# Algolzw/image-restoration-sde

Measured on AMD Instinct MI355X. Metric: restored images/sec at 256x256, 100-step IR-SDE reverse sampler, higher is better.
Workload: dtype f32; 1 GPU; IR-SDE deraining ConditionalUNet nf=64 depth=4, reverse_sde, batch=16/GPU 256x256, T=100 (BASELINE.json configs[1]); compute_dtype=fp32, global_batch=16

## Files before the change

### image_restoration_sde_amd/_lib.py

```python
import ctypes
import os
import subprocess
import threading

_HERE = os.path.dirname(os.path.abspath(__file__))
LIB_PATH = os.environ.get("IRSDE_LIB_PATH") or os.path.join(_HERE, "libirsde_hip.so")
CSRC = os.path.join(_HERE, "csrc")

MODE = {"sde": 0, "ode": 1, "posterior": 2, "dsde_sde": 3, "dsde_ode": 4}
COEF_STRIDE = 12
FLAG_KEEP_ACTIVATIONS = 1
FLAG_NAIVE_CONV = 2
FLAG_NO_WINOGRAD = 4
FLAG_NO_WINOGRAD_F43 = 8
FLAG_UNCOND_FULLATTN = 16
FLAG_BF16 = 32
FLAG_NAF_INTRO_SKIP = 64
FLAG_BF16_ACT = 128
FLAG_NO_FUSED_LN = 256
FLAG_NAF_LENS = 512
FLAG_FP16 = 1024
FLAG_NO_WINOGRAD_FUSED = 2048
FLAG_NO_FUSED_ATTN = 4096
FLAG_NO_NAF_CHAIN = 8192
FLAG_SPLIT_BF16X2 = 16384
FLAG_SPLIT_F16X2 = 32768
FLAG_NAF_STEREO = 65536
FLAG_NAF_UNCOND = 131072
FLAG_UNET_STEREO = 262144
FLAG_F16_ACT = 524288
FLAG_NO_WINO_POLY = 1048576
FLAG_SCAM_STREAM = 2097152
FLAG_NO_SPLIT3 = 4194304
SAMPLE_GRAPH = 1
SAMPLE_PROFILE = 2

SYMBOLS = [
    "irsde_last_error", "irsde_version", "irsde_create", "irsde_create_nafnet", "irsde_destroy", "irsde_num_weights",
    "irsde_weight_name", "irsde_weight_shape", "irsde_load_weight", "irsde_finalize_weights",
    "irsde_set_schedule", "irsde_unet_forward", "irsde_sample", "irsde_sde_step", "irsde_philox_normal",
    "irsde_get_profile", "irsde_debug_tap", "irsde_work_model", "irsde_debug_conv", "irsde_debug_conv_choice", "irsde_debug_conv_halo_choice", "irsde_debug_conv_features", "irsde_plan_describe", "irsde_bench_conv", "irsde_op_profile", "irsde_debug_split_gemm", "irsde_bench_naf_chain", "irsde_debug_force_subbatches", "irsde_debug_force_chain_groups", "irsde_debug_force_wino_poly", "irsde_debug_force_split3", "irsde_debug_force_split3_blocks", "irsde_debug_scam", "irsde_debug_scam_full",
    "irsde_debug_scam_stream", "irsde_debug_scam_full_stream", "irsde_debug_force_scam_stream",
    "irsde_debug_naf_gate_sca", "irsde_debug_tlsc", "irsde_debug_ln_film", "irsde_debug_naf_lnconv", "irsde_debug_naf_chain", "irsde_debug_naf_chain_split_order",
    "irsde_debug_full_attention16",
    "irsde_eval_metrics", "irsde_tensor2img", "irsde_upscale_bicubic", "irsde_mask_to", "irsde_imresize",
    "irsde_set_lens_info", "irsde_nafnet_set_local_pool", "irsde_create_latent_unet", "irsde_latent_shapes", "irsde_latent_encode", "irsde_latent_decode", "irsde_latent_hidden",
]


class IrsdeLibraryError(RuntimeError):
    pass


class IrsdeError(RuntimeError):
    pass


class Config(ctypes.Structure):
    _fields_ = [("in_nc", ctypes.c_int32), ("out_nc", ctypes.c_int32), ("nf", ctypes.c_int32),
                ("depth", ctypes.c_int32), ("device", ctypes.c_int32), ("flags", ctypes.c_int32)]


class NafConfig(ctypes.Structure):
    _fields_ = [("img_channel", ctypes.c_int32), ("width", ctypes.c_int32), ("middle_blk_num", ctypes.c_int32),
                ("n_enc", ctypes.c_int32), ("enc_blk_nums", ctypes.c_int32 * 8), ("n_dec", ctypes.c_int32),
                ("dec_blk_nums", ctypes.c_int32 * 8), ("device", ctypes.c_int32), ("flags", ctypes.c_int32)]


class LatentConfig(ctypes.Structure):
    _fields_ = [("in_ch", ctypes.c_int32), ("out_ch", ctypes.c_int32), ("ch", ctypes.c_int32), ("n_mult", ctypes.c_int32),
                ("ch_mult", ctypes.c_int32 * 8), ("embed_dim", ctypes.c_int32), ("device", ctypes.c_int32),
                ("flags", ctypes.c_int32)]


_lib = None
_lock = threading.Lock()


PROBES_LIB_PATH = os.path.join(_HERE, "libirsde_hip_probes.so")


def build_library(force=False, verbose=False, probes=True):
    if force:
        subprocess.run(["make", "-C", CSRC, "clean"], check=True, capture_output=not verbose)
    for extra in ([], ["PROBES=1"]) if probes else ([],):
        r = subprocess.run(["make", "-j8", "-C", CSRC] + extra, capture_output=True, text=True)
        if r.returncode != 0:
            raise IrsdeLibraryError("building libirsde_hip%s.so failed:\n" % ("_probes" if extra else "") + r.stdout + r.stderr)
        if verbose:
            print(r.stdout)
    return LIB_PATH


def _declare(lib):
    c = ctypes
    P = c.c_void_p
    lib.irsde_last_error.restype = c.c_char_p
    lib.irsde_last_error.argtypes = []
    lib.irsde_version.restype = c.c_int
    lib.irsde_create.argtypes = [c.POINTER(Config), c.POINTER(P)]
    lib.irsde_create_nafnet.argtypes = [c.POINTER(NafConfig), c.POINTER(P)]
    lib.irsde_destroy.argtypes = [P]
    lib.irsde_destroy.restype = None
    lib.irsde_num_weights.argtypes = [P]
    lib.irsde_weight_name.argtypes = [P, c.c_int]
    lib.irsde_weight_name.restype = c.c_char_p
    lib.irsde_weight_shape.argtypes = [P, c.c_int, c.POINTER(c.c_int64), c.POINTER(c.c_int)]
    lib.irsde_load_weight.argtypes = [P, c.c_char_p, P, c.POINTER(c.c_int64), c.c_int]
    lib.irsde_finalize_weights.argtypes = [P]
    lib.irsde_set_schedule.argtypes = [P, c.c_int, P]
    lib.irsde_unet_forward.argtypes = [P, P, P, c.POINTER(c.c_int64), c.c_int, c.c_int, c.c_int, c.c_int, P, P]
    lib.irsde_sample.argtypes = [P, c.c_int, P, P, P, c.c_uint64, c.c_uint64, c.c_int, c.c_int, c.c_int,
                                 c.c_int, c.c_int, P, P, c.c_int]
    lib.irsde_sde_step.argtypes = [c.c_int, c.c_int, P, P, P, P, P, c.c_uint64, c.c_uint64, c.c_int, c.c_int,
                                   c.c_int, c.c_int, P]
    lib.irsde_philox_normal.argtypes = [P, c.c_int, c.c_int, c.c_int, c.c_uint64, c.c_uint64, P]
    lib.irsde_get_profile.argtypes = [P, c.POINTER(c.c_double)]
    lib.irsde_debug_tap.argtypes = [P, c.c_char_p, P, c.POINTER(c.c_int64)]
    lib.irsde_work_model.argtypes = [P, c.c_int, c.c_int, c.c_int, c.POINTER(c.c_double)]
    lib.irsde_debug_conv.argtypes = [P, c.c_int, P, c.c_int, c.c_int, c.c_int, c.c_int, c.c_int, P, c.c_int, c.c_int,
                                     c.c_int, c.c_int, c.c_int, P, P, c.c_int, c.c_int, P, P, c.c_int, c.c_int, P]
    lib.irsde_debug_conv_choice.argtypes = [c.c_int] * 13 + [c.c_uint] + [c.c_int] * 4 + [c.POINTER(c.c_int), c.c_char_p, c.c_int]
    lib.irsde_debug_conv_halo_choice.argtypes = [c.c_int] * 13 + [c.c_uint] + [c.c_int] * 5 + [c.c_char_p, c.c_int]
    lib.irsde_debug_conv_features.argtypes = ([P, c.c_int, P, c.c_int] + [c.c_int] * 4 + [P] + [c.c_int] * 7 + [P] * 3 + [P, c.c_int, P, P, P, c.c_int] + [c.c_int] * 6 +
                                              [c.POINTER(c.c_int), P, c.c_char_p, c.c_int, P])
    lib.irsde_plan_describe.argtypes = [P, c.c_int, c.c_int, c.c_int, c.c_char_p, c.c_int]
    lib.irsde_op_profile.argtypes = [P, c.c_char_p, c.c_int]
    lib.irsde_bench_conv.argtypes = [c.c_int] * 11 + [c.POINTER(c.c_double)]
    lib.irsde_bench_naf_chain.argtypes = [c.c_int] * 4 + [c.POINTER(c.c_double)]
    lib.irsde_debug_force_subbatches.argtypes = [c.c_int]
    lib.irsde_debug_force_chain_groups.argtypes = [c.c_int]
    lib.irsde_debug_force_wino_poly.argtypes = [c.c_int]
    lib.irsde_debug_force_split3.argtypes = [c.c_int]
    lib.irsde_debug_force_split3_blocks.argtypes = [c.c_int]
    lib.irsde_debug_scam.argtypes = [P, c.c_int, c.c_int, c.c_int, c.c_int] + [P] * 12 + [P, P]
    lib.irsde_debug_scam_full.argtypes = [P, c.c_int, c.c_int, c.c_int, c.c_int] + [P] * 12 + [P, P]
    lib.irsde_debug_scam_stream.argtypes = [P, c.c_int, c.c_int, c.c_int, c.c_int] + [P] * 12 + [c.c_int, P, P]
    lib.irsde_debug_scam_full_stream.argtypes = [P, c.c_int, c.c_int, c.c_int, c.c_int] + [P] * 12 + [c.c_int, P, P]
    lib.irsde_debug_force_scam_stream.argtypes = [c.c_int]
    lib.irsde_debug_naf_gate_sca.argtypes = [P, c.c_int, c.c_int, c.c_int, c.c_int] + [P] * 8
    lib.irsde_debug_tlsc.argtypes = [P] + [c.c_int] * 6 + [P] * 4
    lib.irsde_debug_ln_film.argtypes = [P, c.c_int64, c.c_int, c.c_int64, P, P, P, c.c_int, P, P]
    lib.irsde_debug_naf_lnconv.argtypes = [c.c_int, P, c.c_int64, c.c_int, c.c_int, c.c_int64, P, P, P, c.c_int, P, P, P, c.c_int, P, P, P, P, P]
    lib.irsde_debug_naf_chain.argtypes = [P, P, c.c_int, c.c_int] + [P] * 16 + [P, c.c_int, c.c_int, P, c.c_int, c.c_int, c.c_int, P]
    lib.irsde_debug_naf_chain_split_order.argtypes = [c.c_int, c.c_int, c.POINTER(c.c_int), c.c_int64]
    lib.irsde_debug_full_attention16.argtypes = [P, c.c_int, c.c_int, P, P]
    lib.irsde_debug_split_gemm.argtypes = [P, P, P, c.c_int, c.c_int, c.c_int, c.c_int, c.c_int, P]
    lib.irsde_eval_metrics.argtypes = [P, P, c.c_int, c.c_int, c.c_int, c.c_int, c.c_int, c.POINTER(c.c_double), P]
    lib.irsde_tensor2img.argtypes = [P, P, c.c_int, c.c_int, c.c_int, c.c_int, P]
    lib.irsde_upscale_bicubic.argtypes = [P, P, c.c_int, c.c_int, c.c_int, c.c_int, c.c_int, P]
    lib.irsde_mask_to.argtypes = [P, P, c.c_int, c.c_int, c.c_int, c.c_int, P, c.c_int, c.c_int, c.c_int, c.c_int, P]
    lib.irsde_imresize.argtypes = [P, P] + [c.c_int] * 6 + [P, P, c.c_int, P, P, c.c_int, P]
    lib.irsde_set_lens_info.argtypes =[P, c.POINTER(c.c_float), c.c_int]
    lib.irsde_nafnet_set_local_pool.argtypes = [P, c.c_int, c.c_int, c.c_int, c.c_int]
    lib.irsde_create_latent_unet.argtypes = [c.POINTER(LatentConfig), c.POINTER(P)]
    lib.irsde_latent_shapes.argtypes = [P, c.c_int, c.c_int, c.POINTER(c.c_int64), c.POINTER(c.c_int64), c.POINTER(c.c_int)]
    lib.irsde_latent_encode.argtypes = [P, P, c.c_int, c.c_int, c.c_int, P, c.POINTER(P), P]
    lib.irsde_latent_decode.argtypes = [P, P, c.POINTER(P), c.c_int, c.c_int, c.c_int, P, P]
    lib.irsde_latent_hidden.argtypes = [P, c.c_int, c.c_int, c.c_int, c.c_int, P, P]
    for name in SYMBOLS:
        getattr(lib, name)
    return lib


def lib():
    global _lib
    with _lock:
        if _lib is None:
            if not os.path.exists(LIB_PATH):
                raise IrsdeLibraryError(
                    "libirsde_hip.so not found at %s — build it with `python -c 'import __graft_entry__ as g; "
                    "g.build()'` or `make -C %s`. There is no CPU/PyTorch fallback for this path." % (LIB_PATH, CSRC))
            try:
                _lib = _declare(ctypes.CDLL(LIB_PATH))
            except OSError as ex:
                raise IrsdeLibraryError("failed to load %s: %s" % (LIB_PATH, ex)) from ex
        return _lib


_probes = None


def probes_lib():
    global _probes
    with _lock:
        if _probes is None:
            if not os.path.exists(PROBES_LIB_PATH):
                raise IrsdeLibraryError("libirsde_hip_probes.so not found at %s — build it with `make -C %s PROBES=1`" % (PROBES_LIB_PATH, CSRC))
            try:
                _probes = _declare(ctypes.CDLL(PROBES_LIB_PATH))
            except OSError as ex:
                raise IrsdeLibraryError("failed to load %s: %s" % (PROBES_LIB_PATH, ex)) from ex
        return _probes


def check(rc, L=None):
    if rc != 0:
        msg = (L or lib()).irsde_last_error()
        raise IrsdeError("libirsde_hip error %d: %s" % (rc, msg.decode() if msg else "?"))


def stream_ptr(torch_stream=None):
    import torch
    s = torch_stream if torch_stream is not None else torch.cuda.current_stream()
    return ctypes.c_void_p(s.cuda_stream)
```

### image_restoration_sde_amd/csrc/common.h

```cpp
#pragma once
#include <hip/hip_runtime.h>
#include <cstdint>
#include <cstdio>
#include <cstdlib>
#include <stdexcept>
#include <string>
#include <vector>
#include "split3_layout.h"

namespace irsde {

struct HipError : std::runtime_error {
    using std::runtime_error::runtime_error;
};
struct HipOutOfMemory : HipError {
    using HipError::HipError;
};

inline int tuning_env_int(const char* name, int dflt) {
    static const bool on = [] { const char* t = getenv("IRSDE_TUNING"); return t && atoi(t) == 1; }();
    if (!on) return dflt;
    const char* v = getenv(name);
    return v ? atoi(v) : dflt;
}
// ... 185 lines not shown
    int tiles_x = 0, tiles_y = 0, nblk_n = 0;
    int n_slow = 0;
    unsigned grid = 0;
    int lds = 0;
    int instance = -1;
};
constexpr int kHaloInstances = 9;
struct ConvChoice {
    enum Family { PAIR, NARROW3, ZLOOP_BATCH, ZLOOP_1X1, HALO, IGEMM };
    enum Operand { OP_F32, OP_F32_BUF, OP_BF16, OP_F16 };
    enum Storage { ACT_F32, ACT_BF16, ACT_F16 };
    Family family = IGEMM;
    int BM = 0, BN = 0;
    Operand op = OP_F32;
    Storage act = ACT_F32;
    bool inscale = false;
    int zbatch = 0, zrows = 0;
    unsigned gx = 0, gy = 1, gz = 1;
    HaloChoice halo;
    int threads = 0, lds = 0;
    int row = -1;
    std::string name() const;
    long long blocks() const { return (long long)gx * gy * gz; }
};
int conv_base_bn(int Cout);
void conv_validate(const ConvParams& p);
ConvChoice conv_choose(const ConvParams& p, const ConvTune& t, const ConvKnobs& k, int cu_count);
int conv_instance_count();
void launch_conv(const ConvParams& p, hipStream_t s, const ConvTune& t = {}, const ConvKnobs* knobs = nullptr, ConvChoice* chosen = nullptr);
void conv_global_init();
void conv_halo_global_init();
bool conv_halo_eligible(const ConvParams& p);
HaloChoice conv_halo_choose(const ConvParams& p, const ConvTune& t, int halo2, int nslow);
bool conv_halo2_wanted(const ConvParams& p);
HaloChoice launch_conv_halo(const ConvParams& p, hipStream_t s, const ConvTune& t = {});
void launch_fill_random(float* p, size_t n, unsigned seed, float scale, hipStream_t s);
__device__ __forceinline__ float silu_hw(const float v) {
    return v * __builtin_amdgcn_rcpf(1.0f + __builtin_amdgcn_exp2f(v * -1.44269504088896341f));
}

void launch_f32_to_bf16(const float* in, unsigned short* out, size_t n, hipStream_t s);
void launch_f32_to_f16(const float* in, unsigned short* out, size_t n, hipStream_t s);
void launch_bf16_to_f32(const unsigned short* in, float* out, size_t n, hipStream_t s);
void launch_f16_to_f32(const unsigned short* in, float* out, size_t n, hipStream_t s);
void launch_conv_naive(const ConvParams& p, hipStream_t s);

void launch_layernorm(const float* x, const float* g, const float* res, float* out, int64_t M, int C,
                      float eps, hipStream_t s, bool bf16 = false);
void launch_layernorm_film(const float* x, const float* g, const float* scale, const float* shift, int film_bstride,
                           int64_t pixels_per_image, float* out, int64_t M, int C, float eps, hipStream_t s,
                           bool f16 = false);
int dwgate_tiles(int H, int W, int c);
bool naf_lnconv_ok(int c, int Cout, long long M);
void launch_naf_pwconv(const float* x, const float* in_scale, int64_t pixels_per_image, const unsigned short* w16, const float* bias, const float* ch_scale,
                       const float* res, float* out, int64_t M, int c, int Cout, hipStream_t s, bool f16 = false);
void naf_lnconv_global_init();
void launch_naf_lnconv(const float* x, const float* g, const float* fscale, const float* fshift, int film_bstride, int64_t pixels_per_image,
                       const unsigned short* w16, const float* bias, float* out, int64_t M, int c, int Cout, int gate, const float* gate_film,
                       int gate_film_bstride, hipStream_t s, bool f16 = false);
void launch_dwconv_gate(const float* u, const float* w, const float* bias, float* out, float* partial, int B, int H, int W,
                        int c, hipStream_t s, bool f16 = false);
void launch_sca(const float* partial, int ntiles, const float* W, const float* bias, float* mean, float* s_out, int B,
                int c, int HW, hipStream_t s);
void launch_sca_mean(const float* partial, int ntiles, float* mean, int B, int c, int HW, hipStream_t s);
void tlsc_check_shape(int B, int h, int w, int c, int k1, int k2);
void launch_tlsc_pool(const float* gated, float* rowsum, float* pooled, int B, int h, int w, int c, int k1, int k2, hipStream_t s);
void launch_tlsc_scale(float* gated, const float* scale, int B, int h, int w, int c, int k1, int k2, hipStream_t s);
void launch_row_gate(const float* in, float* out, int rows, int h, hipStream_t s);

struct AttnWorkspace {
    float* pmax = nullptr;
    float* pctx = nullptr;
    float* psum = nullptr;
    float* ctx = nullptr;
    int nch = 0;
};
int attn_num_chunks(int N, int B);
void launch_linear_attention(const float* qkv, float* out, int B, int N, const AttnWorkspace& ws, hipStream_t s,
                             bool bf16 = false);

void launch_attention_kv_context(const float* xn, const float* wkv, int B, int N, int C, const AttnWorkspace& ws, hipStream_t s,
                                 const float* ln_g = nullptr, float ln_eps = 1e-5f, const unsigned short* wkv_pair = nullptr,
                                 float w_inv_scale = 1.f, int op16 = 0, bool act_bf16 = false);
void launch_attention_q_out(const float* q, float* out, int B, int N, const AttnWorkspace& ws, hipStream_t s);
void launch_attention_q_out_fused(const float* xn, const float* x, const float* wq, const float* wout, const float* bias,
                                  const float* g2, float* y, int B, int N, int C, float eps, const AttnWorkspace& ws, hipStream_t s,
                                  const float* ln_g = nullptr, const unsigned short* wq_pair = nullptr, const unsigned short* wout_pair = nullptr,
                                  float wq_inv = 1.f, float wout_inv = 1.f, int op16 = 0, bool act_bf16 = false);

void scam_check_shape(int H, int W, int c, bool any_width = false);
void launch_scam_prologue(const float* x, const float* g_l, const float* g_r, float* xs2, int B, int H, int W, int c, hipStream_t s);
void launch_scam_core(const float* qv, float* F, int B, int H, int W, int c, hipStream_t s);
void launch_scam_epilogue(const float* x, const float* F, const float* beta, const float* gamma, float* out, int B, int H, int W, int c, hipStream_t s);
void scam_pack_proj(const float* w1, const float* b1, const float* w2, const float* b2, int c, std::vector<float>& w, std::vector<float>& bias);
constexpr int kScamFullMaxW = 1024;
constexpr int kScamFullMaxC = 2048;
void scam_full_check_shape(int H, int W, int c, bool any_width = false);
void launch_scam_full_prologue(const float* x, const float* g_l, const float* g_r, float* x2, int B, int H, int W, int c, hipStream_t s);
void launch_scam_full_core(const float* qv, float* F, int B, int H, int W, int c, hipStream_t s);
void launch_scam_full_epilogue(float* x, const float* F, const float* beta, const float* gamma, int B, int H, int W, int c, hipStream_t s);
constexpr int kScamMaxWs = 512;
constexpr int kScamStreamMaxBlockW = 512;
bool scam_stream_block_ok(int block_w);
void launch_scam_stream_core(const float* qv, float* F, int B, int Hs, int Ws, int c, int block_w, hipStream_t s);
void launch_stereo_prep(const float* xt, const float* cond, float* x0, int B, int ic, int P, int H, int W, int Hp, int Wp, hipStream_t s);
void launch_stereo_pack_pred(const float* in, float* out, int B, int ic, int Hp, int Wp, int in_stride, int out_stride, hipStream_t s);
void launch_stereo_unet_prep(const float* xt, const float* cond, float* x0, int B, int ic, int P, int H, int W, int Hp, int Wp, hipStream_t s);
void launch_stereo_unet_pack_pred(const float* in, const float* xt, float* out, int B, int ic, int H, int W, int Hp, int Wp, int in_stride, int out_stride,
                                  hipStream_t s);

void launch_full_attention(const float* qkv, float* out, int B, int N, hipStream_t s);
void launch_full_attention16(const unsigned short* qkv, unsigned short* out, int B, int N, hipStream_t s);

void launch_prep_input(const float* xt, const float* cond, float* x0, int B, int in_nc, int H, int W, int Hp, int Wp,
                       hipStream_t s, int reflect = 1);

enum Act { ACT_NONE = 0, ACT_SILU = 1, ACT_GELU = 2 };
void launch_sinusoid(const float* tvals, const float* freqs, float* out, int rows, int half, hipStream_t s);
void launch_row_linear(const float* in, int in_stride, const float* W, const float* b, float* out, int out_stride,
                       int rows, int in_dim, int out_dim, int act_in, int act_out, hipStream_t s);

struct StepState {
    int t;
    int t_next;
    int pad0, pad1;
    float coef[12];
};
void launch_step_begin(StepState* st, const float* film_table, int film_row, float* film_cur,
                       const float* coef_table, hipStream_t s);
void launch_set_step(StepState* st, int t_next, hipStream_t s);

struct SampleCtl {
    int mode;
    int pad;
    const float* noise;
    long long noise_tstride;
    unsigned long long seed;
    unsigned long long image_offset;
};
void launch_set_ctl(SampleCtl* ctl, int mode, const float* noise, long long noise_tstride, unsigned long long seed,
                    unsigned long long image_offset, hipStream_t s);

void launch_unpack_pred(const float* pred, float* out, int B, int C, int H, int W, int Hp, int Wp, int stride, hipStream_t s);
void launch_add(const float* a, const float* b, float* out, size_t n, hipStream_t s);
void launch_nchw_to_nhwc_pad(const float* in, float* out, int B, int C, int H, int W, int Hp, int Wp, int Cp, int reflect,
                             hipStream_t s);
void launch_nhwc_to_nchw(const float* in, float* out, int B, int C, int H, int W, hipStream_t s, bool bf16 = false, bool f16 = false);

struct UpdateParams {
    float* x;
    const float* mu;
    const float* pred;
    int64_t sb, sc, sy, sx;
    const float* noise;
    int64_t noise_tstride;
    const StepState* st;
    const SampleCtl* ctl;
    int t_imm;
    float coef_imm[12];
    int mode;
    int B, C, H, W;
    uint64_t seed;
    uint64_t image_offset;
    int batch0;
};
void launch_sde_update(const UpdateParams& p, hipStream_t s);
// ... 12 lines not shown
```

### image_restoration_sde_amd/csrc/engine.h

```cpp
#pragma once
#include <algorithm>
#include <cmath>
#include <cstring>
#include <functional>
#include <map>
#include <memory>
#include <mutex>
#include <string>
#include <vector>

#include "../../include/irsde_hip.h"
#include "common.h"

namespace irsde {

constexpr int kWinoFusedMaxCin = 256, kWinoFusedMaxCout = 256;
inline long long wino_fused_min_tiles() { return tuning_env_int("IRSDE_WINO_FUSED_MINT", 4096); }
inline bool wino_fused64_enabled() { return tuning_env_int("IRSDE_WINO_FUSED64", 1) != 0; }
inline bool wino_fused64_pair_enabled() { return tuning_env_int("IRSDE_WINO_FUSED64_PAIR", 1) != 0; }
inline int wino_fused64_max_cin() { return tuning_env_int("IRSDE_WINO_FUSED64_MAXCIN", 512); }
inline int wino_fused64_max_cout() { return tuning_env_int("IRSDE_WINO_FUSED64_MAXCOUT", 512); }
inline long long wino_fused64_min_tiles() { return tuning_env_int("IRSDE_WINO_FUSED64_MINT", 1024); }
inline int wino_fused64t_mode() { return tuning_env_int("IRSDE_WINO_FUSED64T", 1); }
inline bool naf_lnconv_enabled() { return tuning_env_int("IRSDE_NAF_LNCONV", 1) != 0; }
inline int naf_chain_split_mode() { return tuning_env_int("IRSDE_NAF_CHAIN_SPLIT", 0); }

int wino_poly_mode();
void set_force_wino_poly(int mode);
constexpr int kWinoPolyUpMinCin = 512;
inline bool wino_poly_wants_weights(int mode, bool up, int Cin) { return mode >= 2 || (mode == 1 && (!up || Cin >= kWinoPolyUpMinCin)); }

int split3_mode();
void set_force_split3(int mode);
constexpr int kSplit3WinoMinCin = 512;
inline int split3_wino_min_cin() { return tuning_env_int("IRSDE_SPLIT3_MINCIN", kSplit3WinoMinCin); }
inline bool split3_wino_wants_weights(int mode, int Cin, int Cout) { return mode >= 2 || Cin > 512 || (Cin >= split3_wino_min_cin() && Cout >= 512); }
inline long long split3_fused_min_tiles() { return tuning_env_int("IRSDE_SPLIT3_FUSED_MINT", 4096); }
constexpr int kSplit3NotExactF32 = IRSDE_FLAG_NO_WINOGRAD | IRSDE_FLAG_NAIVE_CONV | IRSDE_FLAG_BF16 | IRSDE_FLAG_BF16_ACT | IRSDE_FLAG_FP16 | IRSDE_FLAG_F16_ACT |
                                   IRSDE_FLAG_SPLIT_BF16X2 | IRSDE_FLAG_SPLIT_F16X2 | IRSDE_FLAG_NO_SPLIT3;
inline bool split3_wants_weights(int flags) { return !(flags & kSplit3NotExactF32) && split3_mode() > 0; }

inline int wino_min_c(int tile) {
    return tuning_env_int(tile == 4 ? "IRSDE_WINO4_MINC" : "IRSDE_WINO2_MINC", tile == 4 ? 64 : 256);
}

struct DeviceScope {
    int prev = -1;
    explicit DeviceScope(int dev) {
        if (hipGetDevice(&prev) != hipSuccess) prev = -1;
        if (prev != dev) IRSDE_HIP_CHECK(hipSetDevice(dev));
        else prev = -1;
    }
    ~DeviceScope() {
        if (prev >= 0) (void)hipSetDevice(prev);
    }
    DeviceScope(const DeviceScope&) = delete;
    DeviceScope& operator=(const DeviceScope&) = delete;
};

struct HostTensor {
    std::vector<int64_t> shape;
    std::vector<float> data;
    bool loaded = false;
};

struct ConvW {
    float* w = nullptr;
    float* bias = nullptr;
    int Cout = 0, Cin = 0, KH = 1, KW = 1;
    float* wino_u2 = nullptr;
    float* wino_u4 = nullptr;
    float* wino_uf = nullptr;
    float* wino_uf64 = nullptr;
    unsigned short* wino_uf64p = nullptr;
    float wino_uf64p_scale = 1.f;
    unsigned short* wino_up = nullptr;
    float wino_up_scale = 1.f;
    unsigned short* wino_u4t = nullptr;
    unsigned short* wino_polyt = nullptr;
    float* wino_poly = nullptr;
};
struct ResW {
    ConvW b1, b2, res;
    bool has_res = false;
    float* mlp_w = nullptr;
    float* mlp_b = nullptr;
    int film_off = 0;
    int Cout = 0;
};
struct ScamW {
    int c = 0;
    float *gl = nullptr, *gr = nullptr;
    ConvW l, r;
    float *beta = nullptr, *gamma = nullptr;
};
struct AttnW {
    float* g1 = nullptr;
    ConvW qkv, out;
    float* g2 = nullptr;
    int C = 0;
};

struct NafBlockW {
    int c = 0;
    float *g1 = nullptr, *g2 = nullptr;
    ConvW conv1, conv3, conv4, conv5;
    float *dw_w = nullptr, *dw_b = nullptr;
    float *sca_w = nullptr, *sca_b = nullptr;
    float *beta = nullptr, *gamma = nullptr;
    float *mlp_w = nullptr, *mlp_b = nullptr;
    int film_off = 0;
    float *cam_w = nullptr, *cam_b = nullptr;
    int cam_off = 0;
    ScamW fusion;
};

struct NafChainW {
    unsigned short* w = nullptr;
    float* vecs = nullptr;
    int nblocks = 0, film_off = 0, cam_off = 0;
    unsigned short* wsplit[5] = {nullptr, nullptr, nullptr, nullptr, nullptr};
};

// ... 226 lines not shown
    ScamW mid_scam;
    std::vector<ResW> up_res;
    std::vector<AttnW> up_attn;
    std::vector<ConvW> up_conv;
    ResW final_res;
    std::vector<ResW*> all_res;
    int film_row = 0;

    int arch = 0;
    int naf_ic = 0;
    std::vector<int> naf_enc_nums, naf_dec_nums;
    int naf_mid_num = 0;
    std::vector<std::vector<NafBlockW>> naf_enc, naf_dec;
    std::vector<NafBlockW> naf_mid;
    std::vector<ConvW> naf_downs, naf_ups;
    ConvW naf_intro, naf_ending;
    std::vector<NafBlockW*> naf_all;
    std::vector<NafChainW> naf_chain_enc, naf_chain_dec;
    NafChainW naf_chain_mid;
    float *cm_w1 = nullptr, *cm_b1 = nullptr, *cm_w3 = nullptr, *cm_b3 = nullptr;
    int cam_row = 0;
    float* cam_cur = nullptr;
    int cam_rows = 0;
    int cam_set = 0;

    int tlsc_base_h = 0, tlsc_base_w = 0, tlsc_train_h = 0, tlsc_train_w = 0;

    int lat_in = 0, lat_out = 0, lat_ch = 0, lat_embed = 0;
    std::vector<int> lat_mult;
    ConvW lat_init, lat_latent, lat_post, lat_final;
    std::vector<ResW> lat_enc_res, lat_dec_res;
    AttnW lat_enc_attn, lat_dec_attn;
    std::vector<ConvW> lat_down, lat_up;
    std::vector<std::unique_ptr<LatentPlan>> lat_plans;

    int T = 0;
    float* coef_table = nullptr;
    float* film_table = nullptr;
    float* film_cur = nullptr;
    int film_cur_rows = 0;
    StepState* step = nullptr;
    SampleCtl* ctl = nullptr;

    float* zeros = nullptr;
    hipStream_t stream = nullptr;
    hipEvent_t ev_in = nullptr, ev_out = nullptr;
    static constexpr int kMaxSub = 4;
    hipStream_t sub_stream[kMaxSub - 1] = {nullptr, nullptr, nullptr};
    hipEvent_t ev_fork = nullptr, ev_join[kMaxSub - 1] = {nullptr, nullptr, nullptr};
    std::vector<std::unique_ptr<Plan>> plans;
    uint64_t use_counter = 0;
    double profile[12] = {0};
    std::vector<double> op_ms;
    std::vector<std::string> op_desc;
    int op_steps = 0;
    int plan_parts = 1;
    int op_split = 1;
    std::vector<hipEvent_t> ev_pool;
    std::mutex mu;

    float* dmalloc(size_t n) {
        float* p = nullptr;
        IRSDE_HIP_CHECK(hipMalloc(&p, std::max<size_t>(n, 16) * sizeof(float)));
        dev_allocs.push_back(p);
        return p;
    }
    std::map<const float*, unsigned short*> bf16_copies;
    const unsigned short* bf16_copy(const float* w, size_t n) {
        auto it = bf16_copies.find(w);
        if (it != bf16_copies.end()) return it->second;
        unsigned short* d = nullptr;
        IRSDE_HIP_CHECK(hipMalloc(&d, n * sizeof(unsigned short)));
        if (cfg.flags & IRSDE_FLAG_FP16) launch_f32_to_f16(w, d, n, stream);
        else launch_f32_to_bf16(w, d, n, stream);
        IRSDE_HIP_CHECK(hipStreamSynchronize(stream));
        bf16_copies[w] = d;
        return d;
    }
    struct PairCopy { unsigned short* p; float inv_scale; };
    std::map<const float*, PairCopy> pair_copies;
    PairCopy pair_copy(const float* w, size_t n) {
        return make_pair_copy(pair_copies, w, n, [&](unsigned short* d, bool f16, float sc) { launch_split_planes(w, d, n, n, 2, stream, f16, sc); });
    }
    std::map<const float*, PairCopy> pair_copies_il;
    PairCopy pair_copy_il(const float* w, size_t rows, int K) {
        return make_pair_copy(pair_copies_il, w, rows * (size_t)K, [&](unsigned short* d, bool f16, float sc) { launch_split_pairs(w, d, rows, K, stream, f16, sc); });
    }
    template <class Split>
    PairCopy make_pair_copy(std::map<const float*, PairCopy>& cache, const float* w, size_t n, Split split) {
        auto it = cache.find(w);
        if (it != cache.end()) return it->second;
        const bool f16 = (cfg.flags & IRSDE_FLAG_SPLIT_F16X2) != 0;
        float sc = 1.f;
        if (f16) {
            std::vector<float> h(n);
            IRSDE_HIP_CHECK(hipMemcpy(h.data(), w, n * sizeof(float), hipMemcpyDeviceToHost));
            sc = pow2_scale_into_512(h.data(), n);
        }
        unsigned short* d = nullptr;
        IRSDE_HIP_CHECK(hipMalloc(&d, 2 * n * sizeof(unsigned short)));
        dev_allocs.push_back(reinterpret_cast<float*>(d));
        split(d, f16, sc);
        IRSDE_HIP_CHECK(hipStreamSynchronize(stream));
        const PairCopy pc{d, 1.0f / sc};
        cache[w] = pc;
        return pc;
    }
    float* upload(const std::vector<float>& v) {
        float* p = dmalloc(v.size());
        IRSDE_HIP_CHECK(hipMemcpy(p, v.data(), v.size() * sizeof(float), hipMemcpyHostToDevice));
        return p;
    }
};

namespace irsde {

inline bool naf_lens(const irsde_engine* e) { return (e->cfg.flags & IRSDE_FLAG_NAF_LENS) != 0; }
inline bool naf_stereo(const irsde_engine* e) { return e->arch == 1 && (e->cfg.flags & IRSDE_FLAG_NAF_STEREO) != 0; }
inline bool unet_stereo(const irsde_engine* e) { return e->arch == 0 && (e->cfg.flags & IRSDE_FLAG_UNET_STEREO) != 0; }
inline bool stereo_engine(const irsde_engine* e) { return naf_stereo(e) || unet_stereo(e); }
inline bool uncond_engine(const irsde_engine* e) {
    return (e->arch == 0 && (e->cfg.flags & IRSDE_FLAG_UNCOND_FULLATTN) != 0) || (e->arch == 1 && (e->cfg.flags & IRSDE_FLAG_NAF_UNCOND) != 0);
}
inline int rup32(int c) { return (c + 31) & ~31; }
inline bool tlsc_window(const irsde_engine* e, int level, int* K0, int* K1) {
    if (e->tlsc_train_h <= 0) return false;
    const int P = 1 << e->cfg.depth;
    const int Hp = (e->tlsc_train_h + P - 1) / P * P, Wp = (e->tlsc_train_w + P - 1) / P * P;
    *K0 = (int)((long long)(Hp >> level) * e->tlsc_base_h / e->tlsc_train_h);
    *K1 = (int)((long long)(Wp >> level) * e->tlsc_base_w / e->tlsc_train_w);
    return true;
}
inline StepState* step_of(const irsde_engine* e, const Plan* pl) { return pl->own_step ? pl->own_step : e->step; }
inline float* film_of(const irsde_engine* e, const Plan* pl) { return pl->own_film ? pl->own_film : e->film_cur; }

void build_inventory(irsde_engine* e);
void build_inventory_naf(irsde_engine* e);
void build_inventory_latent(irsde_engine* e);
void finalize(irsde_engine* e);
void compute_film_rows(irsde_engine* e, const float* tvals, int rows, float* dst, hipStream_t s);
void ensure_film_cur(irsde_engine* e, int rows);
void pack_conv_rows(const float* w_oihw, const float* bias, int O, int I, int KH, int KW, const std::vector<int>& perm, std::vector<float>& pw,
                    std::vector<float>& pb);
std::vector<int> naf_gate_perm(int c);
std::vector<int> naf_shuffle_perm(int Cout);
std::vector<float> pack_dwconv_taps(const float* w, int c2);
void pack_naf_chain_host(const std::vector<NafChainHostW>& blocks, std::vector<unsigned short>& w, std::vector<float>& vecs);

Plan* get_plan(irsde_engine* e, int B, int H, int W, bool per_sample_film, int slot = 0, int b0 = 0);
int naf_subbatches(const irsde_engine* e, int B, int H, int W);
void set_force_chain_groups(int g);
void set_force_scam_stream(int block_w);
int forced_chain_groups();
int forced_scam_stream();
void set_force_subbatches(int n);
LatentPlan* get_latent_plan(irsde_engine* e, int B, int H, int W, bool decode);

int guard(const std::function<void()>& f);

}
```

### image_restoration_sde_amd/csrc/engine_debug.hip

```cpp
#include "engine.h"
#include "../../include/irsde_hip_debug.h"

using namespace irsde;

namespace irsde {
namespace {

struct Scratch {
    hipStream_t s;
    std::vector<void*> bufs;
    explicit Scratch(hipStream_t s_) : s(s_) {}
    ~Scratch() {
        (void)hipStreamSynchronize(s);
        for (void* p : bufs) (void)hipFree(p);
    }
    Scratch(const Scratch&) = delete;
    Scratch& operator=(const Scratch&) = delete;
    template <class T> T* alloc(size_t n) {
        void* p = nullptr;
        IRSDE_HIP_CHECK(hipMalloc(&p, n * sizeof(T)));
        bufs.push_back(p);
        return static_cast<T*>(p);
    }
    float* upload(const float* host, size_t n) {
// ... 838 lines not shown
        const bool f16 = operand == 2;
        unsigned short *w16 = nullptr, *a0 = nullptr, *a1 = nullptr, *ar = nullptr, *ao = nullptr;
        float wsc = 1.f;
        if (pair) {
            wsc = f16 ? pow2_scale_into_512(pk.data(), pk.size()) : 1.f;
            w16 = mem.alloc<unsigned short>(2 * pk.size());
            p.w_pair = w16; p.pair_scale = 1.0f / wsc;
        } else if (operand) {
            w16 = mem.alloc<unsigned short>(pk.size());
            p.w_bf = w16;
        }
        p.f16 = f16 ? 1 : 0;
        if (storage) {
            a0 = mem.alloc<unsigned short>(npix_in * C0);
            p.in0 = reinterpret_cast<const float*>(a0);
            if (in1) { a1 = mem.alloc<unsigned short>(npix_in * C1); p.in1 = reinterpret_cast<const float*>(a1); }
            if (res) { ar = mem.alloc<unsigned short>(nout); p.res = reinterpret_cast<const float*>(ar); }
            ao = mem.alloc<unsigned short>(nout);
            p.out = reinterpret_cast<float*>(ao);
            p.in_bf16 = p.out_bf16 = storage == 1;
            p.in_f16 = p.out_f16 = storage == 2;
        }
        ConvKnobs k;
        static_assert(sizeof(ConvKnobs) == 11 * sizeof(int), "the hook's knob array is ConvKnobs, field by field");
        if (knobs) memcpy(&k, knobs, sizeof k);
        conv_validate(p);
        auto narrow = [&](const float* src, unsigned short* dst, size_t n) {
            if (storage == 2) launch_f32_to_f16(src, dst, n, s);
            else launch_f32_to_bf16(src, dst, n, s);
        };
        if (pair) launch_split_pairs(dw, w16, (size_t)Cout * nz, K * K * Cin, s, f16, wsc);
        else if (operand == 2) launch_f32_to_f16(dw, w16, pk.size(), s);
        else if (operand == 1) launch_f32_to_bf16(dw, w16, pk.size(), s);
        if (storage) {
            narrow(in0, a0, npix_in * C0);
            if (in1) narrow(in1, a1, npix_in * C1);
            if (res) narrow(res, ar, nout);
            IRSDE_HIP_CHECK(hipMemsetAsync(ao, 0xFF, nout * 2, s));
        }
        ConvChoice c;
        launch_conv(p, s, conv_tune_from_code(tune), knobs ? &k : nullptr, &c);
        if (storage == 2) launch_f16_to_f32(ao, out, nout, s);
        else if (storage == 1) launch_bf16_to_f32(ao, out, nout, s);
        IRSDE_HIP_CHECK(hipStreamSynchronize(s));
        write_choice_line(c, choice, choice_len);
        if (c.family == ConvChoice::HALO) {
            const size_t n = strlen(choice);
            if (n + 2 < (size_t)choice_len) {
                choice[n] = ' ';
                write_halo_line(c.halo, choice + n + 1, choice_len - (int)n - 1);
            }
        }
    });
}

int irsde_debug_split_gemm(const float* A, const float* Bm, float* C, int M, int N, int K, int ncomp, int nplanes, void* stream) {
    return guard([&] {
        const int twin3 = nplanes == 43 ? 0 : nplanes == 45 ? 1 : nplanes == 47 ? 2 : -1;
        if (twin3 < 0 && nplanes != 42 && nplanes != 44) throw HipError("debug_split_gemm: nplanes must be 42, 43, 44, 45 or 47");
        hipStream_t s = reinterpret_cast<hipStream_t>(stream);
        conv_global_init();
        Scratch mem(s);
        if (twin3 >= 0) {
            if (!gemm_split_triples_fits(M, N, K, N)) throw HipError("debug_split_gemm: shape not eligible for the three-piece GEMM");
            launch_gemm_split_triples(split_triples(mem, A, Bm, C, M, N, K, ncomp, s), ncomp, s, split3_launch_twin(twin3));
        } else {
            const bool f16 = nplanes == 44;
            launch_gemm_split_pairs(split_pairs(mem, A, Bm, C, M, N, K, ncomp, s, f16, f16 ? 1.0f / 16.0f : 1.f, f16 ? 64.0f : 1.f), ncomp, s, 0, f16);
        }
        IRSDE_HIP_CHECK(hipStreamSynchronize(s));
    });
}

int irsde_debug_force_chain_groups(int g) {
    set_force_chain_groups(g == 1 || g == 2 || g == 4 ? g : 0);
    return IRSDE_OK;
}

int irsde_debug_force_split3(int mode) {
    set_force_split3(mode >= 0 && mode <= 2 ? mode : -1);
    return IRSDE_OK;
}

int irsde_debug_force_split3_blocks(int n) {
    if (n >= 0 && n < 8) return guard([&] { throw HipError("debug_force_split3_blocks: n must be at least 8 (one block per XCD), or negative for the default"); });
    set_force_split3_blocks(n);
    return IRSDE_OK;
}

int irsde_debug_force_wino_poly(int mode) {
    set_force_wino_poly(mode >= 0 && mode <= 2 ? mode : -1);
    return IRSDE_OK;
}

int irsde_debug_force_subbatches(int n) {
    set_force_subbatches(n < 0 ? 0 : n);
    return IRSDE_OK;
}

int irsde_bench_naf_chain(int variant, int nblocks, int B, int iters, double* ms_out) {
    return guard([&] {
        if (!ms_out || nblocks < 1 || nblocks > 64 || B < 1 || iters < 1) throw HipError("bench_naf_chain: bad argument");
        const int G = variant == 22 ? 2 : (variant == 24 || variant == 25 || variant == 26) ? 4 : 1;
#ifdef IRSDE_PROBES
        if (variant != 0 && variant != 1 && variant != 11 && G == 1) throw HipError("bench_naf_chain: bad variant");
#else
        if (variant != 0 && variant != 1 && G == 1) throw HipError("bench_naf_chain: variant 11 is a measurement twin (make PROBES=1)");
#endif
        conv_global_init();
        OwnedStream stream(hipStreamDefault);
        hipStream_t s = stream.s;
        Scratch mem(s);
        const size_t nx = (size_t)B * 64 * 512, nw = naf_chain_weight_halves(nblocks), nv = naf_chain_vec_floats(nblocks);
        float *dx = mem.alloc<float>(nx), *dout = mem.alloc<float>(nx), *dvec = mem.alloc<float>(nv), *dfilm = mem.alloc<float>((size_t)nblocks * 2048);
        unsigned short* dw = mem.alloc<unsigned short>(nw);
        const size_t chunk = (size_t)64 << 20;
        float* dwf = mem.alloc<float>(chunk);
        launch_fill_random(dx, nx, 1, 1.0f, s);
        launch_fill_random(dvec, nv, 2, 0.1f, s);
        launch_fill_random(dfilm, (size_t)nblocks * 2048, 3, 0.1f, s);
        for (size_t o = 0; o < nw; o += chunk) {
            const size_t n = std::min(chunk, nw - o);
            launch_fill_random(dwf, n, 4 + (unsigned)(o / chunk), 0.04f, s);
            launch_f32_to_f16(dwf, dw + o, n, s);
        }
        unsigned short* dwg = nullptr;
        void* dscratch = nullptr;
        if (G > 1) {
            IRSDE_HIP_CHECK(hipStreamSynchronize(s));
            dwg = mem.alloc<unsigned short>(nw);
            naf_chain_build_split_weights(dw, dwg, nblocks, G, s);
            dscratch = mem.alloc<char>(naf_chain_split_scratch_bytes(B));
            IRSDE_HIP_CHECK(hipMemset(dscratch, 0, naf_chain_split_scratch_bytes(B)));
        }
        auto run = [&]() {
            if (G > 1) launch_naf_chain_split(dx, dout, dwg, dvec, nblocks, B, dfilm, 0, 0, nullptr, 0, 0, G, dscratch, s);
            else launch_naf_chain(dx, dout, dw, dvec, nblocks, B, dfilm, 0, 0, nullptr, 0, 0, s, variant == 11 ? 1 : variant);
        };
        if (variant == 26) {
#ifdef IRSDE_PROBES
            naf_chain_set_sabotage(1);
#else
            throw HipError("bench_naf_chain: variant 26 is a PROBES-build test");
#endif
        }
        struct SabotageOff { ~SabotageOff() { naf_chain_set_sabotage(0); } } sabotage_off;
        run();
        if (variant == 25) {
#ifdef IRSDE_PROBES
            const int ng = naf_chain_split_groups(B, 4);
            unsigned long long* dd = mem.alloc<unsigned long long>((size_t)ng * 8 * 16);
            IRSDE_HIP_CHECK(hipMemsetAsync(dd, 0, (size_t)ng * 8 * 16 * 8, s));
            naf_chain_set_debug(dd);
            run();
            IRSDE_HIP_CHECK(hipStreamSynchronize(s));
            naf_chain_set_debug(nullptr);
            std::vector<unsigned long long> hd((size_t)ng * 8 * 16);
            IRSDE_HIP_CHECK(hipMemcpy(hd.data(), dd, hd.size() * 8, hipMemcpyDeviceToHost));
            double acc[16] = {0};
            double nwv = 0;
            for (size_t w = 0; w < (size_t)ng * 8; ++w) {
                if (!hd[w * 16 + 15]) continue;
                for (int k = 0; k < 16; ++k) acc[k] += (double)hd[w * 16 + k];
                nwv += 1;
            }
            static const char* names[12] = {"norm1 (incl. residual-stream fetch)", "conv1 GEMM passes", "depthwise 3x3 + gate + pool", "gated fetch behind barrier (pool)", "sca.1 GEMM", "conv3 GEMM + residual", "norm2 (incl. residual-stream fetch)", "conv4 GEMM + gate", "conv5 GEMM + residual", "scale-vector / gated fetch (sca, conv4)", "group barriers (6 per block)", "publishing (gated slice, residual slice)"};
// ... 244 lines not shown
```

### image_restoration_sde_amd/csrc/engine_plan.hip

```cpp
#include "engine.h"
#include <atomic>

using namespace irsde;

namespace irsde {

struct Builder {
    irsde_engine* e;
    Plan* pl;
    bool reuse;
    bool naive;
    int film_bstride;
    int b0 = 0;
    const float* film_base() const { return film_of(e, pl) + (size_t)b0 * film_bstride; }
    const float* cam_base() const { return e->cam_cur + (size_t)b0 * e->cam_row; }
    const float* fused_ln_g = nullptr;

    bool act_bf16() const { return (e->cfg.flags & IRSDE_FLAG_BF16_ACT) != 0; }
    bool act_f16() const { return (e->cfg.flags & IRSDE_FLAG_F16_ACT) != 0; }
    Tensor talloc(int B, int H, int W, int C, int force_f32 = 0) {
        Tensor t;
        t.B = B; t.H = H; t.W = W; t.C = C;
        t.bf16 = act_bf16() && !force_f32;
        t.f16 = act_f16() && !force_f32;
// ... 96 lines not shown
            if (w.wino_uf64p && push_wino_fused(p, reinterpret_cast<const float*>(w.wino_uf64p), true, w.wino_uf64p_scale)) return out;
            if (w.wino_uf64 && push_wino_fused(p, w.wino_uf64, true)) return out;
            if (w.wino_uf && push_wino_fused(p, w.wino_uf, false)) return out;
            if (w.wino_u4 && wino_shape_ok(p, 4) && push_wino(p, w.wino_u4, 4, nullptr, 1.f, w.wino_u4t)) return out;
            if (w.wino_u2 && wino_shape_ok(p, 2) && push_wino(p, w.wino_u2, 2)) return out;
        }
        push_conv(p);
        return out;
    }

    bool push_wino_fused(const ConvParams& d, const float* Uf, bool k64, float pair_uscale = 0.f) {
        ConvParams dd = d;
        dd.zeros = e->zeros;
        if (pair_uscale != 0.f) dd.pair_scale = 1.0f / (kWinoFused64PairVScale * pair_uscale);
        auto eligible = [&](const ConvParams& q) { return k64 ? wino_fused64_eligible(q) : wino_fused_eligible(q); };
        int parts = 1;
        if (!eligible(dd)) {
            for (parts = 2; parts <= 4; parts *= 2) {
                if (d.B % parts) continue;
                ConvParams q = dd;
                q.B = d.B / parts;
                if (eligible(q)) break;
            }
            if (parts > 4) return false;
            dd.B = d.B / parts;
        }
        const int Ctot = d.C0 + d.C1;
        const long long T = (long long)dd.B * (d.Ho / 4) * (d.Wo / 4);
        const long long blocks = k64 ? wino_fused64_num_blocks(dd) : (long long)dd.B * ((d.Ho / 4 + 3) / 4) * ((d.Wo / 4 + 7) / 8) * (d.Cout / 32);
        if (T < (k64 ? wino_fused64_min_tiles() : wino_fused_min_tiles()) || blocks < 256) return false;
        bool use_t = false;
        if (k64 && pair_uscale == 0.f && wino_fused64t_mode() && wino_fused64t_eligible(dd)) {
            const double per_block = (double)wino_fused64t_num_items(dd) / std::max(1, device_cu_count());
            const double work = per_block * (Ctot / 16);
            use_t = wino_fused64t_mode() >= 2 || (!d.in_shift && (work >= 64.0 || (work >= 32.0 && per_block >= 8.0 && !d.res)));
        }
        Op op;
        op.kind = OP_CONV;
        op.flops = conv_flops(d);
        op.exec_flops = 36 * 2.0 * (double)T * parts * Ctot * d.Cout;
        op.bytes = 4.0 * (double)d.B * d.Hin * d.Win * Ctot + 4.0 * (double)d.B * d.Ho * d.Wo * d.Cout + 4.0 * 9.0 * (double)d.Cout * Ctot;
        char buf[256];
        const bool pair = pair_uscale != 0.f;
        snprintf(buf, sizeof buf, "conv(%swinograd F4 fused) %s T=%lld Cout=%d Cin=%d up=%d blocks=%lld flops=%.4g exec=%.4g%s", pair ? "split f16x2 " : "",
                 use_t ? "32x64" : k64 ? "16x64" : "32x32", T * parts, d.Cout, Ctot, d.in_shift, blocks * parts, op.flops, op.exec_flops,
                 parts > 1 ? (parts == 2 ? " (2 batch slices)" : " (4 batch slices)") : "");
        op.desc = buf;
        std::vector<ConvParams> slices;
        for (int i = 0; i < parts; ++i) {
            ConvParams q = dd;
            const size_t b0 = (size_t)i * dd.B;
            q.in0 = dd.in0 + b0 * dd.Hin * dd.Win * dd.pix0;
            if (dd.in1) q.in1 = dd.in1 + b0 * dd.Hin * dd.Win * dd.pix1;
            q.out = dd.out + b0 * dd.Ho * dd.Wo * dd.out_stride;
            if (dd.res) q.res = dd.res + b0 * dd.Ho * dd.Wo * dd.res_stride;
            if (dd.film && dd.film_bstride) q.film = dd.film + b0 * dd.film_bstride;
            slices.push_back(q);
        }
        if (use_t)
            op.fn = [slices, Uf](hipStream_t s) { for (const auto& q : slices) launch_wino_fused64t(q, Uf, s, 0); };
        else if (k64)
            op.fn = [slices, Uf, pair](hipStream_t s) { for (const auto& q : slices) launch_wino_fused64(q, Uf, s, pair ? 4 : 0); };
        else
            op.fn = [slices, Uf](hipStream_t s) { for (const auto& q : slices) launch_wino_fused(q, Uf, s); };
        push_op(std::move(op));
        return true;
    }

    static constexpr long long kSplit3MinRows = 256;
    static constexpr int kSplit3MinCout = 512, kSplit3MinCoutPoly = 256;
    static constexpr double kSplit3MinFlop = 9e9;
    bool split3_rule(long long T, int K, int Cout, int ncomp, int min_cout = kSplit3MinCout) const {
        return T >= kSplit3MinRows && Cout >= min_cout && ncomp * 2.0 * (double)T * K * Cout >= kSplit3MinFlop;
    }
    bool split3_adopts(const unsigned short* Ut, long long T, int K, int Cout, int ncomp, int min_cout = kSplit3MinCout) const {
        const int mode = split3_mode();
        if (!Ut || mode <= 0 || naive || (e->cfg.flags & kSplit3NotExactF32) || !gemm_split_triples_fits(T, Cout, K, Cout)) return false;
        return mode >= 2 || split3_rule(T, K, Cout, ncomp, min_cout);
    }
    bool split3_over_fused(const ConvW& w, const ConvParams& p) const {
        if (!w.wino_u4t || p.C0 + p.C1 > 512 || !wino_shape_ok(p, 4)) return false;
        const long long T = (long long)p.B * (p.Ho / 4) * (p.Wo / 4);
        return T >= split3_fused_min_tiles() && split3_rule(T, p.C0 + p.C1, p.Cout, 36) && split3_adopts(w.wino_u4t, T, p.C0 + p.C1, p.Cout, 36);
    }
    float* alloc_triples(int ncomp, long long rows, int K) { return pl->alloc(((size_t)ncomp * split3_comp_elems((size_t)rows, (size_t)K) + 1) / 2, true); }

    bool push_wino_poly(const ConvParams& d, const float* U, const unsigned short* Ut = nullptr) {
        const int mode = wino_poly_mode();
        if (mode <= 0 || !wino_poly_eligible(d)) return false;
        ConvParams dd = d;
        dd.zeros = e->zeros;
        WinoPolyPlan wp = make_wino_poly(dd, U, nullptr, nullptr);
        const long long T = wp.T;
        const long long gemm_blocks = wp.ncomp * ((T + 127) / 128) * ((d.Cout + 127) / 128);
        const double exec_flops = wp.ncomp * 2.0 * (double)T * wp.K * d.Cout;
        if (mode == 1 && (gemm_blocks < 2ll * device_cu_count() || exec_flops < 2e10)) return false;
        if ((unsigned long long)T * std::max(wp.K, d.Cout) * 4ull >= 0x7fffffffull) return false;
        static const int poly_min_cout = tuning_env_int("IRSDE_SPLIT3_POLY_MINCOUT", kSplit3MinCoutPoly);
        const bool tri = split3_adopts(Ut, T, wp.K, d.Cout, wp.ncomp, poly_min_cout);
        float* V = tri ? alloc_triples(wp.ncomp, T, wp.K) : pl->alloc((size_t)wp.ncomp * T * wp.K, true);
        float* Mb = pl->alloc((size_t)wp.ncomp * T * d.Cout, true);
        wp = make_wino_poly(dd, U, V, Mb);
        SplitGemmArgs sg;
        if (tri) sg = make_wino_poly_triples(wp, d.Cout, Ut, reinterpret_cast<unsigned short*>(V), Mb);
        const char* what = wp.in.up ? "up" : "down";
        {
            Op op;
            op.kind = OP_WINO;
            op.desc = std::string("wino_poly_input(") + what + ") T=" + std::to_string(T) + " C=" + std::to_string(d.C0);
            const WinoPolyParams ip = wp.in;
            op.fn = [ip](hipStream_t s) { launch_wino_poly_input(ip, s); };
            pl->net_ops.push_back(std::move(op));
        }
        {
            Op op;
            op.kind = OP_CONV;
            op.flops = conv_flops(d);
            op.exec_flops = exec_flops;
            op.bytes = 4.0 * (double)d.B * d.Hin * d.Win * d.C0 + 4.0 * (double)d.B * d.Ho * d.Wo * d.Cout + 4.0 * (double)d.KH * d.KW * d.Cout * d.C0;
            char buf[256];
            snprintf(buf, sizeof buf, "conv(winograd F4x2 poly %s gemm x%d) T=%lld Cout=%d Cin=%d K=%d flops=%.4g exec=%.4g%s", what, wp.ncomp, T, d.Cout, d.C0, wp.K,
                     op.flops, op.exec_flops, tri ? " bf16x3" : "");
            op.desc = buf;
            const ConvParams g = wp.gemm;
            const int ncomp = wp.ncomp;
            if (tri) op.fn = [sg, ncomp](hipStream_t s) { launch_gemm_split_triples(sg, ncomp, s); };
            else op.fn = [g](hipStream_t s) { launch_conv(g, s); };
            push_op(std::move(op));
        }
        {
            Op op;
            op.kind = OP_WINO;
            op.desc = std::string("wino_poly_output(") + what + ") T=" + std::to_string(T) + " Cout=" + std::to_string(d.Cout);
            const WinoPolyParams oparm = wp.out;
            op.fn = [oparm](hipStream_t s) { launch_wino_poly_output(oparm, s); };
            pl->net_ops.push_back(std::move(op));
        }
        pl->release(V);
        pl->release(Mb);
        return true;
    }

    bool push_wino(const ConvParams& d, const float* U, int tile, const unsigned short* Up = nullptr, float up_scale = 1.f, const unsigned short* Ut = nullptr) {
        const int Ctot = d.C0 + d.C1;
        const int ncomp = (tile + 2) * (tile + 2);
        const long long T = (long long)d.B * (d.Ho / tile) * (d.Wo / tile);
        const long long gemm_blocks = ncomp * ((T + 127) / 128) * ((d.Cout + 127) / 128);
        if (gemm_blocks < 256) return false;
        ConvParams dd = d;
        dd.zeros = e->zeros;
        if (Up && (T < 256 || d.Cout < 256 || (unsigned long long)T * Ctot * 4ull >= 0xffffffffull)) return false;
        const bool tri = !Up && tile == 4 && split3_adopts(Ut, T, Ctot, d.Cout, ncomp);
        float* V = tri ? alloc_triples(ncomp, T, Ctot) : pl->alloc((size_t)ncomp * T * Ctot, true);
        float* Mb = pl->alloc((size_t)ncomp * T * d.Cout, true);
        WinoPlan wp = make_wino(dd, U, V, Mb, tile);
        WinoSplitPlan sp;
        if (Up) {
            sp = make_wino_pairs(dd, Up, reinterpret_cast<unsigned short*>(V), Mb, (e->cfg.flags & IRSDE_FLAG_SPLIT_F16X2) != 0, up_scale);
            wp.in = sp.in;
        } else if (tri) {
            sp = make_wino_triples(dd, Ut, reinterpret_cast<unsigned short*>(V), Mb);
            wp.in = sp.in;
        }
        const double direct = conv_flops(d);
        {
            Op op;
// ... 380 lines not shown
            pl->net_ops.back().desc = buf;
        }
        Tensor out = x;
        if (!reuse) {
            out = talloc(x.B, H, W, c);
            const float* src = x.p;
            float* dst = out.p;
            const size_t bytes = x.numel() * sizeof(float);
            push_other(OP_OTHER, [=](hipStream_t s) { IRSDE_HIP_CHECK(hipMemcpyAsync(dst, src, bytes, hipMemcpyDeviceToDevice, s)); });
            name("copy(kept activations)");
        }
        {
            const float *be = w.beta, *ga = w.gamma;
            float* op = out.p;
            push_other(OP_OTHER, [=](hipStream_t s) { launch_scam_full_epilogue(op, F, be, ga, Bp, H, W, c, s); });
            name("epilogue(scale + residual, in place)");
        }
        return out;
    }

    Tensor resblock(const ResW& w, const Tensor& in0, const Tensor* in1) {
        Tensor R;
        if (w.has_res)
            R = conv(w.res, in0, in1, 1, 0, 0, nullptr, 0, nullptr);
        else
            R = in0;
        Tensor h1 = conv(w.b1, in0, in1, 1, 1, 0, w.mlp_w ? film_base() + w.film_off : nullptr, 1, nullptr);
        Tensor out = conv(w.b2, h1, nullptr, 1, 1, 0, nullptr, 1, &R);
        tfree(h1);
        if (w.has_res) tfree(R);
        return out;
    }

    AttnWorkspace attn_workspace(int B, int N) {
        AttnWorkspace ws;
        ws.nch = attn_num_chunks(N, B);
        ws.pmax = pl->alloc((size_t)B * ws.nch * 128, false);
        ws.pctx = pl->alloc((size_t)B * 4 * ws.nch * 1024, false);
        ws.psum = pl->alloc((size_t)B * 4 * ws.nch * 32, false);
        ws.ctx = pl->alloc((size_t)B * 4 * 1024, false);
        return ws;
    }

    Tensor attn(const AttnW& w, const Tensor& x) {
        const int64_t M = (int64_t)x.B * x.H * x.W;
        const int N = x.H * x.W;
        const bool fused_kv = w.g2 && !naive && !x.bf16 && !(e->cfg.flags & (IRSDE_FLAG_BF16 | IRSDE_FLAG_NO_FUSED_ATTN)) &&
                              x.C % 32 == 0 && x.C <= 256;
        const bool fused_all = fused_kv && (x.C == 64 || x.C == 128 || x.C == 256) && !(e->cfg.flags & IRSDE_FLAG_NO_FUSED_LN);
        const bool fused_16 = w.g2 && !naive && (e->cfg.flags & IRSDE_FLAG_BF16) && !(e->cfg.flags & (IRSDE_FLAG_NO_FUSED_ATTN | IRSDE_FLAG_NO_FUSED_LN)) &&
                              (x.C == 64 || x.C == 128 || x.C == 256) && x.bf16 == act_bf16();
        if (fused_16) {
            const AttnWorkspace ws = attn_workspace(x.B, N);
            Tensor y = talloc(x.B, x.H, x.W, x.C);
            if (y.bf16 != x.bf16) throw HipError("attention: mixed activation storage types");
            const float *xp = x.p, *wqkv = w.qkv.w, *wo = w.out.w, *bo = w.out.bias, *g1 = w.g1, *g2 = w.g2;
            float* yp = y.p;
            const int B = x.B, C = x.C;
            if (!bo) throw HipError("attention: to_out.0.bias missing");
            const unsigned short* wqkv16 = e->bf16_copy(wqkv, (size_t)384 * C);
            const unsigned short* wo16 = e->bf16_copy(wo, (size_t)C * 128);
            const unsigned short* wkv16 = wqkv16 + (size_t)128 * C;
            const int op16 = (e->cfg.flags & IRSDE_FLAG_FP16) ? 3 : 2;
            const bool abf = x.bf16;
            const char* tag = op16 == 3 ? " (fp16 operands)" : abf ? " (bf16 operands + storage)" : " (bf16 operands)";
            push_other(OP_ATTN, [=](hipStream_t s) {
                launch_attention_kv_context(xp, wqkv + (size_t)128 * C, B, N, C, ws, s, g1, 1e-5f, wkv16, 1.f, op16, abf);
            });
            pl->net_ops.back().desc = std::string("linear_attention LayerNorm + k,v projection") + tag + " + context (fused) C=" + std::to_string(C);
            push_other(OP_ATTN, [=](hipStream_t s) {
                launch_attention_q_out_fused(xp, xp, wqkv, wo, bo, g2, yp, B, N, C, 1e-5f, ws, s, g1, wqkv16, wo16, 1.f, 1.f, op16, abf);
            });
            pl->net_ops.back().desc = std::string("linear_attention LayerNorm + q projection") + tag +
                                      " + softmax + context + to_out + LayerNorm + residual (fused) C=" + std::to_string(C);
            return y;
        }
        if (fused_all) {
            const AttnWorkspace ws = attn_workspace(x.B, N);
            Tensor y = talloc(x.B, x.H, x.W, x.C);
            const float *xp = x.p, *wq = w.qkv.w, *wkv = w.qkv.w + (size_t)128 * x.C, *wo = w.out.w, *bo = w.out.bias, *g1 = w.g1, *g2 = w.g2;
            float* yp = y.p;
            const int B = x.B, C = x.C;
            if (!bo) throw HipError("attention: to_out.0.bias missing");
            const unsigned short* wkv_pair = nullptr;
            float kv_inv = 1.f;
            if (e->cfg.flags & IRSDE_FLAG_SPLIT_F16X2) {
                const auto pc = e->pair_copy(wkv, (size_t)256 * C);
                wkv_pair = pc.p; kv_inv = pc.inv_scale;
            }
            push_other(OP_ATTN, [=](hipStream_t s) { launch_attention_kv_context(xp, wkv, B, N, C, ws, s, g1, 1e-5f, wkv_pair, kv_inv); });
            pl->net_ops.back().desc = std::string("linear_attention LayerNorm + k,v projection") + (wkv_pair ? " (split f16x2)" : "") + " + context (fused) C=" + std::to_string(C);
            const unsigned short *wq_pair = nullptr, *wo_pair = nullptr;
            float wq_inv = 1.f, wo_inv = 1.f;
            if (e->cfg.flags & IRSDE_FLAG_SPLIT_F16X2) {
                const auto pq = e->pair_copy(wq, (size_t)128 * C), po = e->pair_copy(wo, (size_t)C * 128);
                wq_pair = pq.p; wq_inv = pq.inv_scale; wo_pair = po.p; wo_inv = po.inv_scale;
            }
            push_other(OP_ATTN, [=](hipStream_t s) {
                launch_attention_q_out_fused(xp, xp, wq, wo, bo, g2, yp, B, N, C, 1e-5f, ws, s, g1, wq_pair, wo_pair, wq_inv, wo_inv);
            });
            pl->net_ops.back().desc = std::string("linear_attention LayerNorm + q projection") + (wq_pair ? " (split f16x2)" : "") +
                                      " + softmax + context + to_out + LayerNorm + residual (fused) C=" + std::to_string(C);
            return y;
        }
        Tensor xn = talloc(x.B, x.H, x.W, x.C);
        {
            const float *xp = x.p, *g = w.g1;
            float* o = xn.p;
            const int C = x.C;
            const bool bf = x.bf16;
            push_other(OP_LN, [=](hipStream_t s) { launch_layernorm(xp, g, nullptr, o, M, C, 1e-5f, s, bf); });
        }
        Tensor a = talloc(x.B, x.H, x.W, 128);
        if (fused_kv) {
            const AttnWorkspace ws = attn_workspace(x.B, N);
            {
                const float *xp = xn.p, *wkv = w.qkv.w + (size_t)128 * x.C;
                const int B = x.B, C = x.C;
                push_other(OP_ATTN, [=](hipStream_t s) { launch_attention_kv_context(xp, wkv, B, N, C, ws, s); });
                pl->net_ops.back().desc = "linear_attention k,v projection + context (fused) C=" + std::to_string(C);
            }
            ConvW wq = w.qkv;
            wq.Cout = 128;
            Tensor q = conv(wq, xn, nullptr, 1, 0, 0, nullptr, 0, nullptr);
            tfree(xn);
            {
                const float* qp = q.p;
                float* o = a.p;
                const int B = x.B;
                push_other(OP_ATTN, [=](hipStream_t s) { launch_attention_q_out(qp, o, B, N, ws, s); });
                pl->net_ops.back().desc = "linear_attention softmax(q) . context";
            }
            tfree(q);
            return attn_tail(w, x, a, M);
        }
        Tensor qkv = conv(w.qkv, xn, nullptr, 1, 0, 0, nullptr, 0, nullptr);
        tfree(xn);
        if (!w.g2) {
            const float* q = qkv.p;
            float* o = a.p;
            const int B = x.B;
            if (x.bf16) {
                if (!qkv.bf16 || !a.bf16) throw HipError("attention: mixed activation storage types");
                push_other(OP_ATTN, [=](hipStream_t s) {
                    launch_full_attention16(reinterpret_cast<const unsigned short*>(q), reinterpret_cast<unsigned short*>(o), B, N, s);
                });
                pl->net_ops.back().desc = "full_attention (bf16 operands + storage)";
            } else {
                push_other(OP_ATTN, [=](hipStream_t s) { launch_full_attention(q, o, B, N, s); });
            }
            tfree(qkv);
            Tensor y = conv(w.out, a, nullptr, 1, 0, 0, nullptr, 0, &x);
            tfree(a);
            return y;
        }
        {
            const AttnWorkspace ws = attn_workspace(x.B, N);
            const float* q = qkv.p;
            float* o = a.p;
            const int B = x.B;
            const bool bf = x.bf16;
            push_other(OP_ATTN, [=](hipStream_t s) { launch_linear_attention(q, o, B, N, ws, s, bf); });
        }
        tfree(qkv);
        return attn_tail(w, x, a, M);
    }
// ... 52 lines not shown
        x = b.talloc(B, pl->Hp, pl->Wp, p.Cout);
        p.out = x.p; p.out_stride = p.Cout; p.out_f16 = x.f16;
        b.push_conv(p);
        const double real = 2.0 * (double)B * pl->Hp * pl->Wp * p.Cout * 9.0 * ((uncond_engine(e) ? 1.0 : 2.0) * e->naf_ic);
        pl->conv_flops += real - pl->net_ops.back().flops;
        pl->net_ops.back().flops = real;
    }
    b.tap("intro", x);
    const bool intro_skip = (e->cfg.flags & IRSDE_FLAG_NAF_INTRO_SKIP) != 0;
    const Tensor intro = x;
    auto run_level = [&](NafChainW& chain, const std::vector<NafBlockW>& blks, const std::string& path, int level) {
        auto advance = [&](const Tensor& y) {
            if (!(intro_skip && x.p == intro.p)) b.tfree(x);
            x = y;
        };
        if (!b.tlsc_local(x, level) && b.naf_chain_ok(chain, x))
            advance(b.nafchain(chain, x));
        else
            for (size_t j = 0; j < blks.size(); ++j) advance(block(blks[j], x, path + std::to_string(j), level));
    };
    std::vector<Tensor> encs;
    for (size_t i = 0; i < e->naf_enc.size(); ++i) {
        run_level(e->naf_chain_enc[i], e->naf_enc[i], "encoders." + std::to_string(i) + ".", (int)i);
        b.tap("encoders." + std::to_string(i), x);
        encs.push_back(x);
        Builder::ConvOpts od;
        od.stride = 2;
        x = b.conv_naf(e->naf_downs[i], x, od);
        b.tap("downs." + std::to_string(i), x);
    }
    const int nlev = (int)e->naf_enc.size();
    run_level(e->naf_chain_mid, e->naf_mid, "middle_blks.", nlev);
    b.tap("middle", x);
    for (size_t i = 0; i < e->naf_dec.size(); ++i) {
        Tensor skip = encs[encs.size() - 1 - i];
        Builder::ConvOpts ou;
        ou.shuffle = 1; ou.res = &skip;
        Tensor y = b.conv_naf(e->naf_ups[i], x, ou);
        b.tfree(x);
        b.tfree(skip);
        x = y;
        b.tap("ups." + std::to_string(i), x);
        run_level(e->naf_chain_dec[i], e->naf_dec[i], "decoders." + std::to_string(i) + ".", nlev - 1 - (int)i);
        b.tap("decoders." + std::to_string(i), x);
    }
    if (intro_skip) {
        Tensor y = b.talloc(x.B, x.H, x.W, x.C);
        const float *xa = x.p, *xb = intro.p;
        float* yo = y.p;
        const size_t n = x.numel();
        b.push_other(OP_OTHER, [=](hipStream_t s) { launch_add(xa, xb, yo, n, s); });
        b.tfree(x);
        b.tfree(intro);
        x = y;
    }
    Builder::ConvOpts oe;
    oe.pad = 1; oe.out_stride = stereo ? (e->naf_ic + 3) & ~3 : pl->pred_stride;
    Tensor pr = b.conv_naf(e->naf_ending, x, oe);
    b.tfree(x);
    if (stereo) {
        float* pred = pl->alloc((size_t)pl->B * pl->Hp * pl->Wp * pl->pred_stride, false);
        const float* src = pr.p;
        const int Bp = pl->B, ic = e->naf_ic, Hp = pl->Hp, Wp = pl->Wp, is = oe.out_stride, os = pl->pred_stride;
        b.push_other(OP_OTHER, [=](hipStream_t s) { launch_stereo_pack_pred(src, pred, Bp, ic, Hp, Wp, is, os, s); });
        pl->net_ops.back().desc = "stereo_pack_pred";
        pl->pred = pred;
        return;
    }
    pl->pred = pr.p;
}

static std::atomic<int> g_force_chain_groups{0};
void set_force_chain_groups(int g) { g_force_chain_groups.store(g, std::memory_order_relaxed); }
int forced_chain_groups() { return g_force_chain_groups.load(std::memory_order_relaxed); }
static std::atomic<int> g_force_scam_stream{0};
void set_force_scam_stream(int block_w) { g_force_scam_stream.store(block_w, std::memory_order_relaxed); }
int forced_scam_stream() { return g_force_scam_stream.load(std::memory_order_relaxed); }
static std::atomic<int> g_force_split3{-1};
void set_force_split3(int mode) { g_force_split3.store(mode, std::memory_order_relaxed); }
int split3_mode() {
    const int f = g_force_split3.load(std::memory_order_relaxed);
    return f >= 0 ? f : tuning_env_int("IRSDE_SPLIT3", 1);
}
static std::atomic<int> g_force_wino_poly{-1};
void set_force_wino_poly(int mode) { g_force_wino_poly.store(mode, std::memory_order_relaxed); }
int wino_poly_mode() {
    const int f = g_force_wino_poly.load(std::memory_order_relaxed);
    return f >= 0 ? f : tuning_env_int("IRSDE_WINO_POLY", 1);
}
static std::atomic<int> g_force_subbatches{0};
void set_force_subbatches(int n) { g_force_subbatches.store(n, std::memory_order_relaxed); }
int naf_subbatches(const irsde_engine* e, int B, int H, int W) {
    if (e->arch == 2 || stereo_engine(e) || (e->cfg.flags & (IRSDE_FLAG_NAIVE_CONV | IRSDE_FLAG_KEEP_ACTIVATIONS))) return 1;
    int n = g_force_subbatches.load(std::memory_order_relaxed);
    if (n <= 0) {
        static const int env = tuning_env_int("IRSDE_SUBBATCHES", 0);
        n = env;
    }
    if (n <= 0 && e->arch != 1) n = 1;
    if (n <= 0) {
        bool chain = false;
        const int nlev = (int)e->naf_enc.size(), ps = 1 << nlev;
        const int Hp = (H + ps - 1) / ps * ps, Wp = (W + ps - 1) / ps * ps;
        if ((e->cfg.flags & IRSDE_FLAG_FP16) && !(e->cfg.flags & (IRSDE_FLAG_NO_NAF_CHAIN | IRSDE_FLAG_F16_ACT)))
            for (int i = 0; i < nlev; ++i)
                if (e->naf_chain_enc[i].nblocks > 0 && naf_chain_shape_ok(Hp >> i, Wp >> i, e->naf_intro.Cout << i)) {
                    int K0 = 0, K1 = 0;
                    if (!tlsc_window(e, i, &K0, &K1) || (K0 >= (Hp >> i) && K1 >= (Wp >> i))) chain = true;
                }
        n = chain && B >= 8 ? 2 : 1;
    }
    n = std::min(n, (int)irsde_engine::kMaxSub);
    while (n > 1 && B % n) --n;
    return std::max(n, 1);
}

static bool evict_lru_plan(irsde_engine* e) {
    if (e->plans.empty()) return false;
    size_t lru = 0;
    for (size_t i = 1; i < e->plans.size(); ++i)
        if (e->plans[i]->last_use < e->plans[lru]->last_use) lru = i;
    IRSDE_HIP_CHECK(hipDeviceSynchronize());
    const int vb = e->plans[lru]->B, vh = e->plans[lru]->H, vw = e->plans[lru]->W;
    const bool split = e->plans[lru]->slot > 0;
    for (size_t i = e->plans.size(); i-- > 0;)
        if (i == lru || (split && e->plans[i]->slot > 0 && e->plans[i]->B == vb && e->plans[i]->H == vh && e->plans[i]->W == vw))
            e->plans.erase(e->plans.begin() + i);
    return true;
}

static Plan* build_plan(irsde_engine* e, int B, int H, int W, bool per_sample_film, int slot, int b0);

static void init_plan_geometry(irsde_engine* e, Plan* pl, int B, int H, int W, int sdiv) {
    pl->B = B; pl->H = H; pl->W = W;
    pl->Hp = (H + sdiv - 1) / sdiv * sdiv;
    pl->Wp = (W + sdiv - 1) / sdiv * sdiv;
    pl->last_use = ++e->use_counter;
    if (e->arch != 1 && (pl->Hp - H >= H || pl->Wp - W >= W)) throw HipError("image too small for reflect padding");
}

Plan* get_plan(irsde_engine* e, int B, int H, int W, bool per_sample_film, int slot, int b0) {
    for (auto& p : e->plans)
        if (p->B == B && p->H == H && p->W == W && p->per_sample_film == per_sample_film && p->slot == slot && p->b0 == b0) {
            p->last_use = ++e->use_counter;
            return p.get();
        }
    if (e->plans.size() >= 8) evict_lru_plan(e);
    for (;;) {
        try {
            return build_plan(e, B, H, W, per_sample_film, slot, b0);
        } catch (const HipOutOfMemory&) {
            if (!evict_lru_plan(e)) throw;
        }
    }
}

static Plan* build_plan(irsde_engine* e, int B, int H, int W, bool per_sample_film, int slot, int b0) {
    const bool stereo = stereo_engine(e), ustereo = unet_stereo(e);
    if (stereo && slot > 0) throw HipError("internal: a stereo batch is never split into sub-batches");
    ensure_film_cur(e, per_sample_film ? (stereo ? 2 : 1) * (b0 + B) : 1);
    if (naf_lens(e)) {
        if (e->cam_set < b0 + B) throw HipError("latent-bokeh ConditionalNAFNet: irsde_set_lens_info must cover the batch first");
        if (e->cam_rows < b0 + B) throw HipError("internal: lens table smaller than the batch");
    }

    const int depth = e->cfg.depth, nf = e->cfg.nf, in_nc = e->cfg.in_nc;
// ... 236 lines not shown
```

### image_restoration_sde_amd/csrc/gemm_split.hip

```cpp
#include "common.h"
#include <algorithm>
#include <atomic>
#include <type_traits>

namespace irsde {

typedef float floatx16 __attribute__((ext_vector_type(16)));
typedef __bf16 bf16x8 __attribute__((ext_vector_type(8)));
typedef _Float16 f16x8 __attribute__((ext_vector_type(8)));
typedef unsigned uintx4 __attribute__((ext_vector_type(4)));

namespace {

constexpr int SG_BK = 32;

#define IRSDE_GLDS16(GPTR, LPTR) \
    __builtin_amdgcn_global_load_lds((const __attribute__((address_space(1))) void*)(GPTR), (__attribute__((address_space(3))) void*)(LPTR), 16, 0, 0)

template <int ABL = 0, bool F16 = false>
__global__ __launch_bounds__(512, 2) void gemm_split2i_kernel(const SplitGemmArgs g) {
    using frag_t = typename std::conditional<F16, f16x8, bf16x8>::type;
    constexpr int TM = 4, TN = 2, WN = 4, BM = 256, BN = 256;
    constexpr int A_STAGE = BM * 128, STAGE = (BM + BN) * 128;
    extern __shared__ __attribute__((aligned(16))) char lds[];
// ... 323 lines not shown
                    for (int r = 0; r < 16; ++r) {
                        const float v = acc[i][j][r];
                        const unsigned voff = (unsigned)((i * 32 + (r & 3) + 8 * (r >> 2) + 4 * h) * g.ldc + colu + l31) * 4u;
                        __builtin_amdgcn_raw_buffer_store_b32(__builtin_bit_cast(unsigned, v), ro, (int)voff, 0, 0);
                    }
                }
            }
        if (!next) break;
#pragma unroll
        for (int i = 0; i < TM; ++i)
#pragma unroll
            for (int j = 0; j < TN; ++j)
#pragma unroll
                for (int r = 0; r < 16; ++r) acc[i][j][r] = 0.f;
    }
}
#undef IRSDE_PHASE_BARRIER
#undef IRSDE_WAIT_VM
#undef IRSDE_GLDS16

__global__ __launch_bounds__(256) void split_triples_kernel(const float* __restrict__ in, unsigned short* __restrict__ out, const size_t n, const size_t rows,
                                                            const int K) {
    const size_t i = (size_t)blockIdx.x * blockDim.x + threadIdx.x;
    if (i >= n) return;
    const size_t rk = rows * (size_t)K;
    const size_t z = i / rk, rem = i - z * rk;
    const size_t row = rem / K;
    const int k = (int)(rem - row * K);
    float r = in[i];
    unsigned short* o = out + z * split3_comp_elems(rows, K);
#pragma unroll
    for (int p = 0; p < 3; ++p) {
        const __bf16 hb = (__bf16)r;
        o[split3_index(row, k, p, K / 32)] = __builtin_bit_cast(unsigned short, hb);
        r -= (float)hb;
    }
}

template <bool F16>
__global__ __launch_bounds__(256) void split_pairs_kernel(const float* __restrict__ in, unsigned short* __restrict__ out, const size_t n, const int K,
                                                          const float scale) {
    const size_t i = (size_t)blockIdx.x * blockDim.x + threadIdx.x;
    if (i >= n) return;
    const size_t row = i / K;
    const int k = (int)(i - row * K);
    float r = in[i];
    const size_t base = (row * (size_t)(K / 32) + k / 32) * 64 + (k & 31);
    if constexpr (F16) {
        r *= scale;
        const _Float16 hb = (_Float16)r;
        out[base] = __builtin_bit_cast(unsigned short, hb);
        r -= (float)hb;
        const _Float16 lb = (_Float16)r;
        out[base + 32] = __builtin_bit_cast(unsigned short, lb);
    } else {
        const __bf16 hb = (__bf16)r;
        out[base] = __builtin_bit_cast(unsigned short, hb);
        r -= (float)hb;
        const __bf16 lb = (__bf16)r;
        out[base + 32] = __builtin_bit_cast(unsigned short, lb);
    }
}

template <int NPL, bool F16 = false>
__global__ __launch_bounds__(256) void split_planes_kernel(const float* __restrict__ in, unsigned short* __restrict__ out, const size_t n,
                                                           const size_t plane, const float scale) {
    const size_t i = (size_t)blockIdx.x * blockDim.x + threadIdx.x;
    if (i >= n) return;
    float r = F16 ? in[i] * scale : in[i];
#pragma unroll
    for (int p = 0; p < NPL; ++p) {
        if constexpr (F16) {
            const _Float16 hb = (_Float16)r;
            out[p * plane + i] = __builtin_bit_cast(unsigned short, hb);
            r -= (float)hb;
        } else {
            const __bf16 hb = (__bf16)r;
            out[p * plane + i] = __builtin_bit_cast(unsigned short, hb);
            r -= (float)hb;
        }
    }
}

}

void gemm_split_global_init() {
    IRSDE_HIP_CHECK(hipFuncSetAttribute(reinterpret_cast<const void*>(gemm_split2i_kernel<0>), hipFuncAttributeMaxDynamicSharedMemorySize, 160 * 1024));
    IRSDE_HIP_CHECK(hipFuncSetAttribute(reinterpret_cast<const void*>(gemm_split2i_kernel<0, true>), hipFuncAttributeMaxDynamicSharedMemorySize, 160 * 1024));
    IRSDE_HIP_CHECK(hipFuncSetAttribute(reinterpret_cast<const void*>(gemm_split2i_kernel<5, true>), hipFuncAttributeMaxDynamicSharedMemorySize, 160 * 1024));
    IRSDE_HIP_CHECK(hipFuncSetAttribute(reinterpret_cast<const void*>(gemm_split2i_kernel<1>), hipFuncAttributeMaxDynamicSharedMemorySize, 160 * 1024));
    IRSDE_HIP_CHECK(hipFuncSetAttribute(reinterpret_cast<const void*>(gemm_split2i_kernel<3>), hipFuncAttributeMaxDynamicSharedMemorySize, 160 * 1024));
    IRSDE_HIP_CHECK(hipFuncSetAttribute(reinterpret_cast<const void*>(gemm_split2i_kernel<4>), hipFuncAttributeMaxDynamicSharedMemorySize, 160 * 1024));
    IRSDE_HIP_CHECK(hipFuncSetAttribute(reinterpret_cast<const void*>(gemm_split3i_kernel<0, true>), hipFuncAttributeMaxDynamicSharedMemorySize, 160 * 1024));
    IRSDE_HIP_CHECK(hipFuncSetAttribute(reinterpret_cast<const void*>(gemm_split3i_kernel<0, false>), hipFuncAttributeMaxDynamicSharedMemorySize, 160 * 1024));
    IRSDE_HIP_CHECK(hipFuncSetAttribute(reinterpret_cast<const void*>(gemm_split3i_kernel<0, true, true>), hipFuncAttributeMaxDynamicSharedMemorySize, 160 * 1024));
#ifdef IRSDE_PROBES
    IRSDE_HIP_CHECK(hipFuncSetAttribute(reinterpret_cast<const void*>(gemm_split3i_kernel<1, true>), hipFuncAttributeMaxDynamicSharedMemorySize, 160 * 1024));
    IRSDE_HIP_CHECK(hipFuncSetAttribute(reinterpret_cast<const void*>(gemm_split3i_kernel<3, true>), hipFuncAttributeMaxDynamicSharedMemorySize, 160 * 1024));
    IRSDE_HIP_CHECK(hipFuncSetAttribute(reinterpret_cast<const void*>(gemm_split3i_kernel<4, true>), hipFuncAttributeMaxDynamicSharedMemorySize, 160 * 1024));
    IRSDE_HIP_CHECK(hipFuncSetAttribute(reinterpret_cast<const void*>(gemm_split3i_kernel<1, false>), hipFuncAttributeMaxDynamicSharedMemorySize, 160 * 1024));
    IRSDE_HIP_CHECK(hipFuncSetAttribute(reinterpret_cast<const void*>(gemm_split3i_kernel<3, false>), hipFuncAttributeMaxDynamicSharedMemorySize, 160 * 1024));
    IRSDE_HIP_CHECK(hipFuncSetAttribute(reinterpret_cast<const void*>(gemm_split3i_kernel<4, false>), hipFuncAttributeMaxDynamicSharedMemorySize, 160 * 1024));
    IRSDE_HIP_CHECK(hipFuncSetAttribute(reinterpret_cast<const void*>(gemm_split3i_kernel<1, true, true>), hipFuncAttributeMaxDynamicSharedMemorySize, 160 * 1024));
    IRSDE_HIP_CHECK(hipFuncSetAttribute(reinterpret_cast<const void*>(gemm_split3i_kernel<3, true, true>), hipFuncAttributeMaxDynamicSharedMemorySize, 160 * 1024));
    IRSDE_HIP_CHECK(hipFuncSetAttribute(reinterpret_cast<const void*>(gemm_split3i_kernel<4, true, true>), hipFuncAttributeMaxDynamicSharedMemorySize, 160 * 1024));
#endif
}

void launch_gemm_split_pairs(const SplitGemmArgs& a, int ncomp, hipStream_t s, int abl, bool f16) {
    if (a.K % SG_BK) throw HipError("gemm_split_pairs: K must be a multiple of 32");
    if ((unsigned long long)a.M * a.K * 4ull >= 0xffffffffull || (unsigned long long)a.N * a.K * 4ull >= 0xffffffffull ||
        (size_t)a.M * a.ldc * 4 >= 0xffffffffull)
        throw HipError("gemm_split_pairs: a component exceeds the 32-bit offset range");
    SplitGemmArgs g = a;
    g.nblk_n = (a.N + 255) / 256;
    g.n_inner = ncomp;
    const int units = ((a.M + 255) / 256) * ncomp;
    int per_xcd = 0;
    for (int x = 0; x < 8; ++x) per_xcd = std::max(per_xcd, (int)((long long)(x + 1) * units / 8) - (int)((long long)x * units / 8));
    const dim3 grid((unsigned)(8 * per_xcd * g.nblk_n));
    const size_t lds = (size_t)2 * 512 * 128;
    if (f16) {
        if (abl != 0) throw HipError("gemm_split_pairs: the ablation twins exist for the bf16 kernel only");
        static const bool nt = tuning_env_int("IRSDE_SPLIT_NT", 0) != 0;
        if (nt) hipLaunchKernelGGL((gemm_split2i_kernel<5, true>), grid, dim3(512), lds, s, g);
        else hipLaunchKernelGGL((gemm_split2i_kernel<0, true>), grid, dim3(512), lds, s, g);
        IRSDE_HIP_CHECK(hipGetLastError());
        return;
    }
    switch (abl) {
        case 0: hipLaunchKernelGGL(gemm_split2i_kernel<0>, grid, dim3(512), lds, s, g); break;
        case 1: hipLaunchKernelGGL(gemm_split2i_kernel<1>, grid, dim3(512), lds, s, g); break;
        case 3: hipLaunchKernelGGL(gemm_split2i_kernel<3>, grid, dim3(512), lds, s, g); break;
        case 4: hipLaunchKernelGGL(gemm_split2i_kernel<4>, grid, dim3(512), lds, s, g); break;
        default: throw HipError("gemm_split_pairs: bad ablation variant");
    }
    IRSDE_HIP_CHECK(hipGetLastError());
}

bool gemm_split_triples_fits(long long M, long long N, long long K, long long ldc) {
    if (M < 1 || N < 1 || K < 32 || K % SG_BK) return false;
    return (unsigned long long)split3_comp_elems((size_t)M, (size_t)K) * 2ull < 0xffffffffull && (unsigned long long)split3_comp_elems((size_t)N, (size_t)K) * 2ull < 0xffffffffull &&
           (unsigned long long)M * ldc * 4ull < 0xffffffffull;
}

static std::atomic<int> g_force_split3_blocks{-1};
void set_force_split3_blocks(int n) { g_force_split3_blocks.store(n >= 8 ? n : -1, std::memory_order_relaxed); }

template <int ABL>
static void launch_split3_abl(bool walk, bool drain, dim3 grid, size_t lds, hipStream_t s, const SplitGemmArgs& g) {
    if (drain) hipLaunchKernelGGL((gemm_split3i_kernel<ABL, true, true>), grid, dim3(512), lds, s, g);
    else if (walk) hipLaunchKernelGGL((gemm_split3i_kernel<ABL, true>), grid, dim3(512), lds, s, g);
    else hipLaunchKernelGGL((gemm_split3i_kernel<ABL, false>), grid, dim3(512), lds, s, g);
}
void launch_gemm_split_triples(const SplitGemmArgs& a, int ncomp, hipStream_t s, const Split3Launch& o) {
    if (a.K % SG_BK) throw HipError("gemm_split_triples: K must be a multiple of 32");
    if (!gemm_split_triples_fits(a.M, a.N, a.K, a.ldc)) throw HipError("gemm_split_triples: a component exceeds the 32-bit offset range");
    if (ncomp < 1 || a.ldc < a.N) throw HipError("gemm_split_triples: bad component count or output stride");
    static const bool walk_knob = tuning_env_int("IRSDE_SPLIT3_WALK", 1) != 0, drain_knob = tuning_env_int("IRSDE_SPLIT3_DRAIN", 0) != 0;
    const bool walk = o.walk == Split3Launch::RULE ? walk_knob : o.walk == Split3Launch::ON;
    const bool drain = o.drain == Split3Launch::RULE ? drain_knob : o.drain == Split3Launch::ON;
    if (drain && !walk) throw HipError("gemm_split_triples: the drain twin exists on the walk only");
    SplitGemmArgs g = a;
    g.nblk_n = (a.N + 127) / 128;
    g.n_inner = ncomp;
    const long long units = (long long)((a.M + 255) / 256) * ncomp;
// ... 48 lines not shown
```

### image_restoration_sde_amd/csrc/kernels_misc.hip

```cpp
#include "common.h"
#include <algorithm>
#include <type_traits>

namespace irsde {

typedef float floatx16 __attribute__((ext_vector_type(16)));
typedef float floatx4 __attribute__((ext_vector_type(4)));
typedef __bf16 bf16_t;
typedef _Float16 f16_t;
typedef __bf16 bf16x4 __attribute__((ext_vector_type(4)));
typedef _Float16 f16x4 __attribute__((ext_vector_type(4)));
typedef _Float16 f16x8 __attribute__((ext_vector_type(8)));
typedef __bf16 bf16x8 __attribute__((ext_vector_type(8)));
typedef float floatx8 __attribute__((ext_vector_type(8)));

namespace {

template <bool F16OP>
struct Mf16 {
    using x8 = bf16x8;
    using x4 = bf16x4;
    static __device__ __forceinline__ floatx16 mfma(x8 a, x8 b, floatx16 c) { return __builtin_amdgcn_mfma_f32_32x32x16_bf16(a, b, c, 0, 0, 0); }
};
template <>
// ... 205 lines not shown
    ssum += __shfl_xor(ssum, 32, 64);
    if (h == 0) red[wave][1024 + 32 + l31] = mrun;
    __syncthreads();
    float mblk = fmaxf(fmaxf(red[0][1024 + 32 + l31], red[1][1024 + 32 + l31]),
                       fmaxf(red[2][1024 + 32 + l31], red[3][1024 + 32 + l31]));
    const float wscale = mrun == -INFINITY ? 0.f : expf(mrun - mblk);
#pragma unroll
    for (int r = 0; r < 16; ++r) {
        const int d = (r & 3) + 8 * (r >> 2) + 4 * h;
        red[wave][d * 32 + l31] = acc[r] * __shfl(wscale, d, 64);
    }
    if (h == 0) red[wave][1024 + l31] = ssum * wscale;
    __syncthreads();
    float* oc = pctx + ((size_t)bh * nch + ch) * 1024;
    for (int i = threadIdx.x; i < 1024; i += 256) oc[i] = (red[0][i] + red[1][i]) + (red[2][i] + red[3][i]);
    if (threadIdx.x < 32) {
        const int i = 1024 + threadIdx.x;
        psum[((size_t)bh * nch + ch) * 32 + threadIdx.x] = (red[0][i] + red[1][i]) + (red[2][i] + red[3][i]);
        pmax[((size_t)b * nch + ch) * kHid + head * kDh + threadIdx.x] = mblk;
    }
}

struct SwapPair { float a, b; };
__device__ __forceinline__ SwapPair swap16(const float v) {
    SwapPair r{v, v};
    asm volatile("s_nop 1\n\tv_permlane16_swap_b32 %0, %1" : "+v"(r.a), "+v"(r.b));
    return r;
}
__device__ __forceinline__ SwapPair swap32(const float v) {
    SwapPair r{v, v};
    asm volatile("s_nop 1\n\tv_permlane32_swap_b32 %0, %1" : "+v"(r.a), "+v"(r.b));
    return r;
}
template <int W>
__device__ __forceinline__ float group_sum(float v) {
    static_assert(W >= 1 && W <= 64 && (W & (W - 1)) == 0, "group width must be a power of two <= 64");
    if constexpr (W >= 2) v += __builtin_bit_cast(float, __builtin_amdgcn_mov_dpp(__builtin_bit_cast(int, v), 0xB1, 0xF, 0xF, true));
    if constexpr (W >= 4) v += __builtin_bit_cast(float, __builtin_amdgcn_mov_dpp(__builtin_bit_cast(int, v), 0x4E, 0xF, 0xF, true));
    if constexpr (W >= 8) v += __builtin_bit_cast(float, __builtin_amdgcn_mov_dpp(__builtin_bit_cast(int, v), 0x141, 0xF, 0xF, true));
    if constexpr (W >= 16) v += __builtin_bit_cast(float, __builtin_amdgcn_mov_dpp(__builtin_bit_cast(int, v), 0x140, 0xF, 0xF, true));
    if constexpr (W >= 32) {
        const SwapPair r = swap16(v);
        v = r.a + r.b;
    }
    if constexpr (W >= 64) {
        const SwapPair r = swap32(v);
        v = r.a + r.b;
    }
    return v;
}

__device__ __forceinline__ float half_sum(const float v) {
    const SwapPair r = swap32(v);
    return r.a + r.b;
}
__device__ __forceinline__ float half_max(const float v) {
    const SwapPair r = swap32(v);
    return fmaxf(r.a, r.b);
}

template <int C4>
__device__ __forceinline__ floatx4 ln_piece(floatx4 v, const floatx4 g, const float eps) {
    const float s = group_sum<C4>((v.x + v.y) + (v.z + v.w));
    const float mean = s * (1.0f / (float)(4 * C4));
    v -= mean;
    const float q = group_sum<C4>((v.x * v.x + v.y * v.y) + (v.z * v.z + v.w * v.w));
    const float rstd = __builtin_amdgcn_rsqf(q * (1.0f / (float)(4 * C4)) + eps);
    return v * rstd * g;
}

template <int C8>
__device__ __forceinline__ floatx8 ln_piece8(floatx8 v, const float* __restrict__ g8, const float eps) {
    const float s = group_sum<C8>(((v[0] + v[1]) + (v[2] + v[3])) + ((v[4] + v[5]) + (v[6] + v[7])));
    const float mean = s * (1.0f / (float)(8 * C8));
    v -= mean;
    const float q = group_sum<C8>(((v[0] * v[0] + v[1] * v[1]) + (v[2] * v[2] + v[3] * v[3])) + ((v[4] * v[4] + v[5] * v[5]) + (v[6] * v[6] + v[7] * v[7])));
    const float rstd = __builtin_amdgcn_rsqf(q * (1.0f / (float)(8 * C8)) + eps);
    const floatx4 ga = *reinterpret_cast<const floatx4*>(g8), gb = *reinterpret_cast<const floatx4*>(g8 + 4);
    const floatx8 g = {ga.x, ga.y, ga.z, ga.w, gb.x, gb.y, gb.z, gb.w};
    return v * rstd * g;
}

constexpr int kKvTile = 128;
template <int C, int MODE = 0, bool ABF = false>
__global__ __launch_bounds__(256, 2) void attn_kv_ctx_kernel(const float* __restrict__ xn, const float* __restrict__ wkv,
                                                             float* __restrict__ pmax, float* __restrict__ pctx,
                                                             float* __restrict__ psum, const int N, const int chunk_len,
                                                             const int nch, const float* __restrict__ ln_g, const float ln_eps,
                                                             const unsigned short* __restrict__ wkv_pair = nullptr, const float w_inv_scale = 1.f) {
    extern __shared__ __attribute__((aligned(16))) float kv_smem[];
    constexpr bool PAIR = MODE == 1, P16 = MODE != 0;
    using M16 = Mf16<MODE == 1 || MODE == 3>;
    static_assert(!ABF || MODE == 2, "bf16 activation storage goes with the bf16 operand mode");
    constexpr int RB = 2 * C + 16;
    const int ch = blockIdx.x, b = blockIdx.y;
    const int tid = threadIdx.x, lane = tid & 63, head = tid >> 6;
    const int l31 = lane & 31, h = lane >> 5;
    constexpr int LDA = C + 4;
    const int n0 = ch * chunk_len;
    const int n1 = min(N, n0 + chunk_len);
    const float* wk = wkv + (size_t)(head * kDh + l31) * C + 4 * h;
    const float* wv = wkv + (size_t)(kHid + head * kDh + l31) * C + 4 * h;
    constexpr int c4n = C >> 2;
    floatx16 ctx;
#pragma unroll
    for (int r = 0; r < 16; ++r) ctx[r] = 0.f;
    float ssum = 0.f, mrun = -INFINITY;
    for (int t0 = n0; t0 < n1; t0 += kKvTile) {
        auto stage_tile = [&](auto full_tag) {
            constexpr bool FULL = decltype(full_tag)::value;
            const float* tile = xn + ((size_t)b * N + t0) * C;
            constexpr int NP = kKvTile * c4n / 256;
            constexpr int NB = NP % 8 == 0 ? 8 : 4;
#pragma unroll
            for (int j0 = 0; j0 < NP; j0 += NB) {
                floatx4 st[NB];
#pragma unroll
                for (int j = 0; j < NB; ++j) {
                    int i = tid + 256 * (j0 + j), row, c4;
                    if constexpr (256 % c4n == 0) { row = tid / c4n + (256 / c4n) * (j0 + j); c4 = tid % c4n; }
                    else { row = i / c4n; c4 = i - row * c4n; }
                    if constexpr (FULL) st[j] = *reinterpret_cast<const floatx4*>(tile + 4 * i);
                    else st[j] = *reinterpret_cast<const floatx4*>(xn + ((size_t)b * N + min(t0 + row, n1 - 1)) * C + 4 * c4);
                }
#pragma unroll
                for (int j = 0; j < NB; ++j) {
                    int i = tid + 256 * (j0 + j), row, c4;
                    if constexpr (256 % c4n == 0) { row = tid / c4n + (256 / c4n) * (j0 + j); c4 = tid % c4n; }
                    else { row = i / c4n; c4 = i - row * c4n; }
                    if constexpr ((c4n & (c4n - 1)) == 0)
                        if (ln_g) st[j] = ln_piece<c4n>(st[j], *reinterpret_cast<const floatx4*>(ln_g + 4 * c4), ln_eps);
                    if constexpr (PAIR) {
                        const f16x4 hi = __builtin_convertvector(st[j], f16x4);
                        const f16x4 lo = __builtin_convertvector(st[j] - __builtin_convertvector(hi, floatx4), f16x4);
                        char* dst = reinterpret_cast<char*>(kv_smem) + row * RB + 8 * c4;
                        *reinterpret_cast<f16x4*>(dst) = hi;
                        *reinterpret_cast<f16x4*>(dst + kKvTile * RB) = lo;
                    } else if constexpr (P16) {
                        *reinterpret_cast<typename M16::x4*>(reinterpret_cast<char*>(kv_smem) + row * RB + 8 * c4) = __builtin_convertvector(st[j], typename M16::x4);
                    } else {
                        *reinterpret_cast<floatx4*>(kv_smem + row * LDA + 4 * c4) = st[j];
                    }
                }
            }
        };
        auto stage_tile_bf = [&](auto full_tag) {
            constexpr bool FULL = decltype(full_tag)::value;
            constexpr int c8n = C >> 3;
            const char* xb = reinterpret_cast<const char*>(xn);
            const char* tile = xb + ((size_t)b * N + t0) * C * 2;
            constexpr int NP = kKvTile * c8n / 256;
            constexpr int NB = NP % 8 == 0 ? 8 : 4;
            static_assert(256 % c8n == 0 && NP % NB == 0, "piece / thread mapping");
#pragma unroll
            for (int j0 = 0; j0 < NP; j0 += NB) {
                bf16x8 st[NB];
#pragma unroll
                for (int j = 0; j < NB; ++j) {
                    const int i = tid + 256 * (j0 + j), row = tid / c8n + (256 / c8n) * (j0 + j), c8 = tid % c8n;
                    if constexpr (FULL) st[j] = *reinterpret_cast<const bf16x8*>(tile + 16 * (size_t)i);
                    else st[j] = *reinterpret_cast<const bf16x8*>(xb + (((size_t)b * N + min(t0 + row, n1 - 1)) * C + 8 * c8) * 2);
                }
#pragma unroll
                for (int j = 0; j < NB; ++j) {
                    const int row = tid / c8n + (256 / c8n) * (j0 + j), c8 = tid % c8n;
                    if (ln_g) st[j] = __builtin_convertvector(ln_piece8<c8n>(__builtin_convertvector(st[j], floatx8), ln_g + 8 * c8, ln_eps), bf16x8);
                    *reinterpret_cast<bf16x8*>(reinterpret_cast<char*>(kv_smem) + row * RB + 16 * c8) = st[j];
                }
            }
        };
        if constexpr (ABF) {
            if (t0 + kKvTile <= n1) stage_tile_bf(std::true_type{}); else stage_tile_bf(std::false_type{});
        } else {
            if (t0 + kKvTile <= n1) stage_tile(std::true_type{}); else stage_tile(std::false_type{});
        }
        __syncthreads();
        floatx16 ak[4], av[4];
#pragma unroll
        for (int rt = 0; rt < 4; ++rt)
#pragma unroll
            for (int r = 0; r < 16; ++r) { ak[rt][r] = 0.f; av[rt][r] = 0.f; }
        if constexpr (PAIR) {
            const char* arow = reinterpret_cast<const char*>(kv_smem) + l31 * RB + 16 * h;
            const char* wkp = reinterpret_cast<const char*>(wkv_pair) + ((size_t)(head * kDh + l31) * C + 8 * h) * 2;
            const char* wvp = reinterpret_cast<const char*>(wkv_pair) + ((size_t)(kHid + head * kDh + l31) * C + 8 * h) * 2;
            constexpr size_t WPL = (size_t)2 * kHid * C * 2;
            constexpr int NK16 = C / 16;
            f16x8 wk2[2][2], wv2[2][2];
            wk2[0][0] = *reinterpret_cast<const f16x8*>(wkp);
            wk2[0][1] = *reinterpret_cast<const f16x8*>(wkp + WPL);
            wv2[0][0] = *reinterpret_cast<const f16x8*>(wvp);
            wv2[0][1] = *reinterpret_cast<const f16x8*>(wvp + WPL);
            auto kstep = [&](const int ks) {
                const int cur = ks & 1, nxt = cur ^ 1;
                const int kp = (ks + 1 < NK16 ? ks + 1 : ks) * 32;
                wk2[nxt][0] = *reinterpret_cast<const f16x8*>(wkp + kp);
                wk2[nxt][1] = *reinterpret_cast<const f16x8*>(wkp + WPL + kp);
                wv2[nxt][0] = *reinterpret_cast<const f16x8*>(wvp + kp);
                wv2[nxt][1] = *reinterpret_cast<const f16x8*>(wvp + WPL + kp);
#pragma unroll
                for (int rt = 0; rt < 4; ++rt) {
                    const f16x8 ah = *reinterpret_cast<const f16x8*>(arow + rt * 32 * RB + 32 * ks);
                    const f16x8 al = *reinterpret_cast<const f16x8*>(arow + kKvTile * RB + rt * 32 * RB + 32 * ks);
                    ak[rt] = __builtin_amdgcn_mfma_f32_32x32x16_f16(ah, wk2[cur][1], ak[rt], 0, 0, 0);
                    av[rt] = __builtin_amdgcn_mfma_f32_32x32x16_f16(ah, wv2[cur][1], av[rt], 0, 0, 0);
                    ak[rt] = __builtin_amdgcn_mfma_f32_32x32x16_f16(al, wk2[cur][0], ak[rt], 0, 0, 0);
                    av[rt] = __builtin_amdgcn_mfma_f32_32x32x16_f16(al, wv2[cur][0], av[rt], 0, 0, 0);
                    ak[rt] = __builtin_amdgcn_mfma_f32_32x32x16_f16(ah, wk2[cur][0], ak[rt], 0, 0, 0);
                    av[rt] = __builtin_amdgcn_mfma_f32_32x32x16_f16(ah, wv2[cur][0], av[rt], 0, 0, 0);
                }
            };
            if constexpr (C > 64) {
#pragma unroll 2
                for (int ks = 0; ks < NK16; ++ks) kstep(ks);
            } else {
#pragma unroll
                for (int ks = 0; ks < NK16; ++ks) kstep(ks);
            }
#pragma unroll
            for (int rt = 0; rt < 4; ++rt)
#pragma unroll
                for (int r = 0; r < 16; ++r) { ak[rt][r] *= w_inv_scale; av[rt][r] *= w_inv_scale; }
        } else if constexpr (P16) {
            using x8 = typename M16::x8;
            const char* arow = reinterpret_cast<const char*>(kv_smem) + l31 * RB + 16 * h;
            const char* wkp = reinterpret_cast<const char*>(wkv_pair) + ((size_t)(head * kDh + l31) * C + 8 * h) * 2;
            const char* wvp = reinterpret_cast<const char*>(wkv_pair) + ((size_t)(kHid + head * kDh + l31) * C + 8 * h) * 2;
            constexpr int NK16 = C / 16;
            x8 wk1[2], wv1[2];
            wk1[0] = *reinterpret_cast<const x8*>(wkp);
            wv1[0] = *reinterpret_cast<const x8*>(wvp);
#pragma unroll
            for (int ks = 0; ks < NK16; ++ks) {
                const int cur = ks & 1, nxt = cur ^ 1;
                const int kp = (ks + 1 < NK16 ? ks + 1 : ks) * 32;
                wk1[nxt] = *reinterpret_cast<const x8*>(wkp + kp);
                wv1[nxt] = *reinterpret_cast<const x8*>(wvp + kp);
#pragma unroll
                for (int rt = 0; rt < 4; ++rt) {
                    const x8 a = *reinterpret_cast<const x8*>(arow + rt * 32 * RB + 32 * ks);
                    ak[rt] = M16::mfma(a, wk1[cur], ak[rt]);
                    av[rt] = M16::mfma(a, wv1[cur], av[rt]);
                }
            }
        } else {
            const float* arow = kv_smem + l31 * LDA + 4 * h;
            constexpr int NK = C / 8;
            static_assert(NK % 2 == 0, "C must be a multiple of 16");
            floatx4 wkr[2], wvr[2];
            wkr[0] = *reinterpret_cast<const floatx4*>(wk);
            wvr[0] = *reinterpret_cast<const floatx4*>(wv);
#pragma unroll 1
            for (int ks0 = 0; ks0 < NK; ks0 += 2)
#pragma unroll
            for (int u = 0; u < 2; ++u) {
                const int ks = ks0 + u;
                const int k8 = 8 * ks;
                {
                    const int kp = ks + 1 < NK ? k8 + 8 : k8;
                    wkr[u ^ 1] = *reinterpret_cast<const floatx4*>(wk + kp);
                    wvr[u ^ 1] = *reinterpret_cast<const floatx4*>(wv + kp);
                }
                __builtin_amdgcn_sched_barrier(0);
                const floatx4 bk = wkr[u], bv = wvr[u];
#pragma unroll
                for (int rt = 0; rt < 4; ++rt) {
                    const floatx4 a = *reinterpret_cast<const floatx4*>(arow + rt * 32 * LDA + k8);
                    ak[rt] = __builtin_amdgcn_mfma_f32_32x32x2f32(a.x, bk.x, ak[rt], 0, 0, 0);
                    av[rt] = __builtin_amdgcn_mfma_f32_32x32x2f32(a.x, bv.x, av[rt], 0, 0, 0);
                    ak[rt] = __builtin_amdgcn_mfma_f32_32x32x2f32(a.y, bk.y, ak[rt], 0, 0, 0);
                    av[rt] = __builtin_amdgcn_mfma_f32_32x32x2f32(a.y, bv.y, av[rt], 0, 0, 0);
                    ak[rt] = __builtin_amdgcn_mfma_f32_32x32x2f32(a.z, bk.z, ak[rt], 0, 0, 0);
                    av[rt] = __builtin_amdgcn_mfma_f32_32x32x2f32(a.z, bv.z, av[rt], 0, 0, 0);
                    ak[rt] = __builtin_amdgcn_mfma_f32_32x32x2f32(a.w, bk.w, ak[rt], 0, 0, 0);
                    av[rt] = __builtin_amdgcn_mfma_f32_32x32x2f32(a.w, bv.w, av[rt], 0, 0, 0);
                }
            }
        }
        float mit = -INFINITY;
        if (t0 + kKvTile > n1) {
#pragma unroll
            for (int rt = 0; rt < 4; ++rt)
#pragma unroll
                for (int r = 0; r < 16; ++r) {
                    const int n = t0 + 32 * rt + (r & 3) + 8 * (r >> 2) + 4 * h;
                    if (n >= n1) { ak[rt][r] = -INFINITY; av[rt][r] = 0.f; }
                }
        }
#pragma unroll
        for (int rt = 0; rt < 4; ++rt)
#pragma unroll
            for (int r = 0; r < 16; ++r) mit = fmaxf(mit, ak[rt][r]);
        mit = half_max(mit);
        if (__any(mit > mrun)) {
            const float mnew = fmaxf(mrun, mit);
            const float alpha = expf(mrun - mnew);
            mrun = mnew;
            ssum *= alpha;
#pragma unroll
            for (int r = 0; r < 16; ++r) ctx[r] *= __shfl(alpha, (r & 3) + 8 * (r >> 2) + 4 * h, 64);
        }
        {
            const float ml = mrun * 1.44269504088896341f;
#pragma unroll
            for (int rt = 0; rt < 4; ++rt)
#pragma unroll
                for (int r = 0; r < 16; ++r) {
                    ak[rt][r] = __builtin_amdgcn_exp2f(__builtin_fmaf(ak[rt][r], 1.44269504088896341f, -ml));
                    ssum += ak[rt][r];
                }
        }
        __builtin_amdgcn_sched_barrier(0);
        if constexpr (MODE >= 2) {
            using x8 = typename M16::x8;
#pragma unroll
            for (int rt = 0; rt < 4; ++rt)
#pragma unroll
                for (int sh = 0; sh < 2; ++sh) {
                    const floatx8 ka = {ak[rt][8 * sh], ak[rt][8 * sh + 1], ak[rt][8 * sh + 2], ak[rt][8 * sh + 3],
                                        ak[rt][8 * sh + 4], ak[rt][8 * sh + 5], ak[rt][8 * sh + 6], ak[rt][8 * sh + 7]};
                    const floatx8 va = {av[rt][8 * sh], av[rt][8 * sh + 1], av[rt][8 * sh + 2], av[rt][8 * sh + 3],
                                        av[rt][8 * sh + 4], av[rt][8 * sh + 5], av[rt][8 * sh + 6], av[rt][8 * sh + 7]};
                    ctx = M16::mfma(__builtin_convertvector(ka, x8), __builtin_convertvector(va, x8), ctx);
                }
        } else {
#pragma unroll
            for (int rt = 0; rt < 4; ++rt)
#pragma unroll
                for (int r = 0; r < 16; ++r) ctx = __builtin_amdgcn_mfma_f32_32x32x2f32(ak[rt][r], av[rt][r], ctx, 0, 0, 0);
        }
        __syncthreads();
    }
    ssum = half_sum(ssum);
    const int bh = b * kHeads + head;
    float* oc = pctx + ((size_t)bh * nch + ch) * 1024;
#pragma unroll
    for (int r = 0; r < 16; ++r) oc[((r & 3) + 8 * (r >> 2) + 4 * h) * 32 + l31] = ctx[r];
    if (h == 0) {
        psum[((size_t)bh * nch + ch) * 32 + l31] = ssum;
        pmax[((size_t)b * nch + ch) * kHid + head * kDh + l31] = mrun;
    }
}

__global__ __launch_bounds__(1024) void attn_ctx_finalize_kernel(const float* __restrict__ pctx,
                                                                 const float* __restrict__ psum,
                                                                 const float* __restrict__ pmax,
                                                                 float* __restrict__ ctx, const int nch,
                                                                 const float inv_n, const float scale) {
    __shared__ float sm[4][8];
    __shared__ float ss[4][256];
    __shared__ float sz[4][8];
    const int bh = blockIdx.x, dq = blockIdx.y;
    const int b = bh >> 2, head = bh & 3;
    const int el = threadIdx.x & 255, sl = threadIdx.x >> 8;
    const int dl = el >> 5, e = el & 31, d = 8 * dq + dl;
    const float* pm = pmax + (size_t)b * nch * kHid + head * kDh + d;
    float mx = -INFINITY;
    for (int c = sl; c < nch; c += 4) mx = fmaxf(mx, pm[(size_t)c * kHid]);
    if (e == 0) sm[sl][dl] = mx;
    __syncthreads();
    mx = fmaxf(fmaxf(sm[0][dl], sm[1][dl]), fmaxf(sm[2][dl], sm[3][dl]));
    const float* pc = pctx + (size_t)bh * nch * 1024 + d * 32 + e;
    const float* ps = psum + (size_t)bh * nch * 32 + d;
    float s = 0.f, z = 0.f;
#pragma unroll 4
    for (int c = sl; c < nch; c += 4) {
        const float w = expf(pm[(size_t)c * kHid] - mx);
        s += pc[(size_t)c * 1024] * w;
        z += ps[(size_t)c * 32] * w;
    }
    ss[sl][el] = s;
    if (e == 0) sz[sl][dl] = z;
    __syncthreads();
    if (sl == 0) {
        const float st = (ss[0][el] + ss[1][el]) + (ss[2][el] + ss[3][el]);
        const float zt = (sz[0][dl] + sz[1][dl]) + (sz[2][dl] + sz[3][dl]);
        ctx[(size_t)bh * 1024 + d * 32 + e] = st / zt * inv_n * scale;
    }
}

constexpr int kOutTilesPerBlock = 8;

template <typename T>
__global__ __launch_bounds__(256) void attn_out_kernel(const T* __restrict__ qkv, const float* __restrict__ ctx,
                                                       T* __restrict__ out, const int N, const int qstride) {
    const int b = blockIdx.y;
    const int lane = threadIdx.x & 63, head = threadIdx.x >> 6;
    const int l31 = lane & 31, h = lane >> 5;
    float cb[16];
    const float* cp = ctx + ((size_t)(b * kHeads + head)) * 1024 + (16 * h) * 32 + l31;
#pragma unroll
    for (int s = 0; s < 16; ++s) cb[s] = cp[s * 32];

    auto load_q = [&](int t, float* dst) {
        const int nb = (blockIdx.x * kOutTilesPerBlock + t) * 32;
        const int nn = nb + l31;
        const T* qp = qkv + ((size_t)b * N + (nn < N ? nn : (nb < N ? nb : 0))) * qstride + head * kDh + 16 * h;
#pragma unroll
        for (int v = 0; v < 4; ++v) {
            const float4 t4 = ld4(qp + 4 * v);
            dst[4 * v + 0] = t4.x; dst[4 * v + 1] = t4.y; dst[4 * v + 2] = t4.z; dst[4 * v + 3] = t4.w;
        }
    };
    float qn[16];
    load_q(0, qn);
    for (int t = 0; t < kOutTilesPerBlock; ++t) {
        const int nbase = (blockIdx.x * kOutTilesPerBlock + t) * 32;
        if (nbase >= N) break;
        float q[16];
#pragma unroll
        for (int s = 0; s < 16; ++s) q[s] = qn[s];
        if (t + 1 < kOutTilesPerBlock) load_q(t + 1, qn);
        float m = q[0];
#pragma unroll
        for (int s = 1; s < 16; ++s) m = fmaxf(m, q[s]);
        m = fmaxf(m, __shfl_xor(m, 32, 64));
        float z = 0.f;
#pragma unroll
        for (int s = 0; s < 16; ++s) {
            q[s] = expf(q[s] - m);
            z += q[s];
        }
        z += __shfl_xor(z, 32, 64);
        const float iz = 1.0f / z;
        floatx16 acc;
#pragma unroll
        for (int r = 0; r < 16; ++r) acc[r] = 0.f;
#pragma unroll
        for (int s = 0; s < 16; ++s) acc = __builtin_amdgcn_mfma_f32_32x32x2f32(q[s] * iz, cb[s], acc, 0, 0, 0);
#pragma unroll
        for (int r = 0; r < 16; ++r) {
            const int row = (r & 3) + 8 * (r >> 2) + 4 * h;
            const int nn = nbase + row;
            if (nn < N) st1(out + ((size_t)b * N + nn) * kHid + head * kDh + l31, acc[r]);
        }
    }
}

template <int C, int MODE = 0, bool ABF = false>
__global__ __launch_bounds__(256, 2) void attn_q_out_fused_kernel(const float* __restrict__ xn, const float* __restrict__ xres,
                                                               const float* __restrict__ wq, const float* __restrict__ ctx,
                                                               const float* __restrict__ wout, const float* __restrict__ bias,
                                                               const float* __restrict__ g2, float* __restrict__ y, const int N,
                                                               const float eps, const float* __restrict__ ln_g,
                                                               const unsigned short* __restrict__ wq_pair = nullptr,
                                                               const unsigned short* __restrict__ wout_pair = nullptr, const float wq_inv = 1.f,
                                                               const float wout_inv = 1.f) {
    constexpr int TP = 128, LDA = C + 4, LDO = kHid + 4, RT = C / 32;
    constexpr bool PAIR = MODE == 1, P16 = MODE != 0;
    using M16 = Mf16<MODE == 1 || MODE == 3>;
    static_assert(!ABF || MODE == 2, "bf16 activation storage goes with the bf16 operand mode");
    constexpr int RBX = 2 * C + 16, RBO = 2 * kHid + 16;
    constexpr int LDY = C > kHid ? C + 4 : LDO;
    extern __shared__ __attribute__((aligned(16))) float qo_smem[];
    float* Xs = qo_smem;
    float* Os = qo_smem;
    const int b = blockIdx.y, t0 = blockIdx.x * TP;
    const int tid = threadIdx.x, lane = tid & 63, wave = tid >> 6;
    const int l31 = lane & 31, h = lane >> 5;
    const size_t img = (size_t)b * N;

    constexpr int C4 = C / 4;
    const bool full_tile = t0 + TP <= N;
    constexpr int NQ = 32 * C4 / 64;
    constexpr bool KEEP = !PAIR && !ABF && C <= 128;
    floatx4 xkeep[KEEP ? NQ : 1];
    constexpr int C8 = C / 8, NQ8 = 32 * C8 / 64;
    constexpr bool KEEP8 = ABF && C <= 128;
    const bool keep_res = (KEEP || KEEP8) && full_tile && xres == xn;
    bf16x8 xkeep8[KEEP8 ? NQ8 : 1];
    auto stage_tile = [&](auto full_tag) {
        constexpr bool FULL = decltype(full_tag)::value;
        const float* slab_in = xn + (img + t0 + wave * 32) * C;
#pragma unroll
        for (int j0 = 0; j0 < NQ; j0 += 8) {
            floatx4 st[8];
#pragma unroll
            for (int j = 0; j < 8; ++j) {
                const int i = lane + 64 * (j0 + j), row = wave * 32 + lane / C4 + (64 / C4) * (j0 + j), c4 = lane % C4;
                if constexpr (FULL) st[j] = *reinterpret_cast<const floatx4*>(slab_in + 4 * i);
                else st[j] = *reinterpret_cast<const floatx4*>(xn + (img + min(t0 + row, N - 1)) * C + 4 * c4);
                if constexpr (FULL && KEEP) xkeep[j0 + j] = st[j];
            }
#pragma unroll
            for (int j = 0; j < 8; ++j) {
                const int row = wave * 32 + lane / C4 + (64 / C4) * (j0 + j), c4 = lane % C4;
                if (ln_g) st[j] = ln_piece<C4>(st[j], *reinterpret_cast<const floatx4*>(ln_g + 4 * c4), eps);
                if constexpr (PAIR) {
                    const f16x4 hi = __builtin_convertvector(st[j], f16x4);
                    const f16x4 lo = __builtin_convertvector(st[j] - __builtin_convertvector(hi, floatx4), f16x4);
                    char* dst = reinterpret_cast<char*>(qo_smem) + row * RBX + 8 * c4;
                    *reinterpret_cast<f16x4*>(dst) = hi;
                    *reinterpret_cast<f16x4*>(dst + TP * RBX) = lo;
                } else if constexpr (P16) {
                    *reinterpret_cast<typename M16::x4*>(reinterpret_cast<char*>(qo_smem) + row * RBX + 8 * c4) = __builtin_convertvector(st[j], typename M16::x4);
                } else {
                    *reinterpret_cast<floatx4*>(Xs + row * LDA + 4 * c4) = st[j];
                }
            }
        }
    };
    auto stage_tile_bf = [&](auto full_tag) {
        constexpr bool FULL = decltype(full_tag)::value;
        const char* xb = reinterpret_cast<const char*>(xn);
        const char* slab_in = xb + (img + t0 + wave * 32) * C * 2;
        constexpr int NB = NQ8 < 8 ? NQ8 : 8;
#pragma unroll
        for (int j0 = 0; j0 < NQ8; j0 += NB) {
            bf16x8 st[NB];
#pragma unroll
            for (int j = 0; j < NB; ++j) {
                const int i = lane + 64 * (j0 + j), row = wave * 32 + lane / C8 + (64 / C8) * (j0 + j), c8 = lane % C8;
                if constexpr (FULL) st[j] = *reinterpret_cast<const bf16x8*>(slab_in + 16 * (size_t)i);
                else st[j] = *reinterpret_cast<const bf16x8*>(xb + ((img + min(t0 + row, N - 1)) * C + 8 * c8) * 2);
                if constexpr (FULL && KEEP8) xkeep8[j0 + j] = st[j];
            }
#pragma unroll
            for (int j = 0; j < NB; ++j) {
                const int row = wave * 32 + lane / C8 + (64 / C8) * (j0 + j), c8 = lane % C8;
                if (ln_g) st[j] = __builtin_convertvector(ln_piece8<C8>(__builtin_convertvector(st[j], floatx8), ln_g + 8 * c8, eps), bf16x8);
                *reinterpret_cast<bf16x8*>(reinterpret_cast<char*>(qo_smem) + row * RBX + 16 * c8) = st[j];
            }
        }
    };
    if constexpr (ABF) {
        if (full_tile) stage_tile_bf(std::true_type{}); else stage_tile_bf(std::false_type{});
    } else {
        if (full_tile) stage_tile(std::true_type{}); else stage_tile(std::false_type{});
    }
    float cb[16];
    {
        const float* cp = ctx + ((size_t)(b * kHeads + wave)) * 1024 + l31;
#pragma unroll
        for (int s2 = 0; s2 < 16; ++s2) cb[s2] = cp[((s2 & 3) + 8 * (s2 >> 2) + 4 * h) * 32];
    }
    float ctx_up = 1.f;
    if constexpr (MODE == 3) {
        ctx_up = exp2f(ceilf(log2f((float)N)));
#pragma unroll
        for (int s2 = 0; s2 < 16; ++s2) cb[s2] *= ctx_up;
    }
    __syncthreads();

    floatx16 q[4];
#pragma unroll
    for (int ct = 0; ct < 4; ++ct)
#pragma unroll
        for (int r = 0; r < 16; ++r) q[ct][r] = 0.f;
    if constexpr (PAIR) {
        const char* wrow = reinterpret_cast<const char*>(wq_pair) + ((size_t)(wave * kDh + l31) * C + 8 * h) * 2;
        constexpr size_t WPL = (size_t)kHid * C * 2;
        const char* brow = reinterpret_cast<const char*>(qo_smem) + l31 * RBX + 16 * h;
        constexpr int NK16 = C / 16;
        f16x8 wa2[2][2];
        wa2[0][0] = *reinterpret_cast<const f16x8*>(wrow);
        wa2[0][1] = *reinterpret_cast<const f16x8*>(wrow + WPL);
#pragma unroll
        for (int ks = 0; ks < NK16; ++ks) {
            const int cur = ks & 1, nxt = cur ^ 1;
            const int kp = (ks + 1 < NK16 ? ks + 1 : ks) * 32;
            wa2[nxt][0] = *reinterpret_cast<const f16x8*>(wrow + kp);
            wa2[nxt][1] = *reinterpret_cast<const f16x8*>(wrow + WPL + kp);
#pragma unroll
            for (int ct = 0; ct < 4; ++ct) {
                const f16x8 bh = *reinterpret_cast<const f16x8*>(brow + ct * 32 * RBX + 32 * ks);
                const f16x8 bl = *reinterpret_cast<const f16x8*>(brow + TP * RBX + ct * 32 * RBX + 32 * ks);
                q[ct] = __builtin_amdgcn_mfma_f32_32x32x16_f16(wa2[cur][0], bl, q[ct], 0, 0, 0);
                q[ct] = __builtin_amdgcn_mfma_f32_32x32x16_f16(wa2[cur][1], bh, q[ct], 0, 0, 0);
                q[ct] = __builtin_amdgcn_mfma_f32_32x32x16_f16(wa2[cur][0], bh, q[ct], 0, 0, 0);
            }
        }
#pragma unroll
        for (int ct = 0; ct < 4; ++ct)
#pragma unroll
            for (int r = 0; r < 16; ++r) q[ct][r] *= wq_inv;
    } else if constexpr (P16) {
        using x8 = typename M16::x8;
        const char* wrow = reinterpret_cast<const char*>(wq_pair) + ((size_t)(wave * kDh + l31) * C + 8 * h) * 2;
        const char* brow = reinterpret_cast<const char*>(qo_smem) + l31 * RBX + 16 * h;
        constexpr int NK16 = C / 16;
        x8 wa1[2];
        wa1[0] = *reinterpret_cast<const x8*>(wrow);
#pragma unroll
        for (int ks = 0; ks < NK16; ++ks) {
            const int cur = ks & 1, nxt = cur ^ 1;
            wa1[nxt] = *reinterpret_cast<const x8*>(wrow + (ks + 1 < NK16 ? ks + 1 : ks) * 32);
#pragma unroll
            for (int ct = 0; ct < 4; ++ct)
                q[ct] = M16::mfma(wa1[cur], *reinterpret_cast<const x8*>(brow + ct * 32 * RBX + 32 * ks), q[ct]);
        }
    } else
    {
        const float* wrow = wq + (size_t)(wave * kDh + l31) * C + 4 * h;
        const float* brow = Xs + l31 * LDA + 4 * h;
        constexpr int NK = C / 8;
        floatx4 wa[3];
        wa[0] = *reinterpret_cast<const floatx4*>(wrow);
        wa[1] = *reinterpret_cast<const floatx4*>(wrow + 8);
#pragma unroll
        for (int ks = 0; ks < NK; ++ks) {
            if (ks + 2 < NK) wa[(ks + 2) % 3] = *reinterpret_cast<const floatx4*>(wrow + 8 * (ks + 2));
            __builtin_amdgcn_sched_barrier(0);
            const floatx4 a = wa[ks % 3];
#pragma unroll
            for (int ct = 0; ct < 4; ++ct) {
                const floatx4 bb = *reinterpret_cast<const floatx4*>(brow + ct * 32 * LDA + 8 * ks);
                q[ct] = __builtin_amdgcn_mfma_f32_32x32x2f32(a.x, bb.x, q[ct], 0, 0, 0);
                q[ct] = __builtin_amdgcn_mfma_f32_32x32x2f32(a.y, bb.y, q[ct], 0, 0, 0);
                q[ct] = __builtin_amdgcn_mfma_f32_32x32x2f32(a.z, bb.z, q[ct], 0, 0, 0);
                q[ct] = __builtin_amdgcn_mfma_f32_32x32x2f32(a.w, bb.w, q[ct], 0, 0, 0);
            }
        }
    }
    __syncthreads();
#pragma unroll
    for (int ct = 0; ct < 4; ++ct) {
        float m = q[ct][0];
#pragma unroll
        for (int r = 1; r < 16; ++r) m = fmaxf(m, q[ct][r]);
        m = half_max(m);
        float z = 0.f;
        const float ml = m * 1.44269504088896341f;
#pragma unroll
        for (int r = 0; r < 16; ++r) {
            q[ct][r] = __builtin_amdgcn_exp2f(__builtin_fmaf(q[ct][r], 1.44269504088896341f, -ml));
            z += q[ct][r];
        }
        z = half_sum(z);
        const float iz = __builtin_amdgcn_rcpf(z);
        floatx16 o;
#pragma unroll
        for (int r = 0; r < 16; ++r) o[r] = 0.f;
        if constexpr (MODE >= 2) {
            using x8 = typename M16::x8;
#pragma unroll
            for (int sh = 0; sh < 2; ++sh) {
                const floatx8 ca = {cb[8 * sh], cb[8 * sh + 1], cb[8 * sh + 2], cb[8 * sh + 3], cb[8 * sh + 4], cb[8 * sh + 5], cb[8 * sh + 6], cb[8 * sh + 7]};
                const floatx8 qa = {q[ct][8 * sh], q[ct][8 * sh + 1], q[ct][8 * sh + 2], q[ct][8 * sh + 3],
                                    q[ct][8 * sh + 4], q[ct][8 * sh + 5], q[ct][8 * sh + 6], q[ct][8 * sh + 7]};
                o = M16::mfma(__builtin_convertvector(ca, x8), __builtin_convertvector(qa * iz, x8), o);
            }
        } else {
#pragma unroll
            for (int s2 = 0; s2 < 16; ++s2) o = __builtin_amdgcn_mfma_f32_32x32x2f32(cb[s2], q[ct][s2] * iz, o, 0, 0, 0);
        }
        if constexpr (PAIR) {
            char* orow = reinterpret_cast<char*>(qo_smem) + (ct * 32 + l31) * RBO + (wave * kDh + 4 * h) * 2;
#pragma unroll
            for (int gq = 0; gq < 4; ++gq) {
                const floatx4 v = floatx4{o[4 * gq], o[4 * gq + 1], o[4 * gq + 2], o[4 * gq + 3]};
                const f16x4 hi = __builtin_convertvector(v, f16x4);
                const f16x4 lo = __builtin_convertvector(v - __builtin_convertvector(hi, floatx4), f16x4);
                *reinterpret_cast<f16x4*>(orow + 16 * gq) = hi;
                *reinterpret_cast<f16x4*>(orow + TP * RBO + 16 * gq) = lo;
            }
        } else if constexpr (P16) {
            char* orow = reinterpret_cast<char*>(qo_smem) + (ct * 32 + l31) * RBO + (wave * kDh + 4 * h) * 2;
#pragma unroll
            for (int gq = 0; gq < 4; ++gq)
                *reinterpret_cast<typename M16::x4*>(orow + 16 * gq) =
                    __builtin_convertvector(floatx4{o[4 * gq], o[4 * gq + 1], o[4 * gq + 2], o[4 * gq + 3]}, typename M16::x4);
        } else {
            float* orow = Os + (ct * 32 + l31) * LDO + wave * kDh + 4 * h;
#pragma unroll
            for (int gq = 0; gq < 4; ++gq)
                *reinterpret_cast<floatx4*>(orow + 8 * gq) = floatx4{o[4 * gq], o[4 * gq + 1], o[4 * gq + 2], o[4 * gq + 3]};
        }
    }
    __syncthreads();

    floatx16 yv[RT];
#pragma unroll
    for (int rt = 0; rt < RT; ++rt)
#pragma unroll
        for (int r = 0; r < 16; ++r) yv[rt][r] = 0.f;
    if constexpr (PAIR) {
        const char* wrow = reinterpret_cast<const char*>(wout_pair) + ((size_t)l31 * kHid + 8 * h) * 2;
        constexpr size_t WPL = (size_t)C * kHid * 2;
        const char* brow = reinterpret_cast<const char*>(qo_smem) + (wave * 32 + l31) * RBO + 16 * h;
        constexpr int NK16 = kHid / 16;
        constexpr int RH = RT > 4 ? RT / 4 : RT;
#pragma unroll
        for (int r0 = 0; r0 < RT; r0 += RH) {
            f16x8 wa2[2][2][RH];
#pragma unroll
            for (int rt = 0; rt < RH; ++rt) {
                wa2[0][0][rt] = *reinterpret_cast<const f16x8*>(wrow + (size_t)(r0 + rt) * 32 * kHid * 2);
                wa2[0][1][rt] = *reinterpret_cast<const f16x8*>(wrow + WPL + (size_t)(r0 + rt) * 32 * kHid * 2);
            }
#pragma unroll
            for (int ks = 0; ks < NK16; ++ks) {
                const int cur = ks & 1, nxt = cur ^ 1;
                const int kp = (ks + 1 < NK16 ? ks + 1 : ks) * 32;
#pragma unroll
                for (int rt = 0; rt < RH; ++rt) {
                    wa2[nxt][0][rt] = *reinterpret_cast<const f16x8*>(wrow + (size_t)(r0 + rt) * 32 * kHid * 2 + kp);
                    wa2[nxt][1][rt] = *reinterpret_cast<const f16x8*>(wrow + WPL + (size_t)(r0 + rt) * 32 * kHid * 2 + kp);
                }
                const f16x8 bh = *reinterpret_cast<const f16x8*>(brow + 32 * ks);
                const f16x8 bl = *reinterpret_cast<const f16x8*>(brow + TP * RBO + 32 * ks);
#pragma unroll
                for (int rt = 0; rt < RH; ++rt) yv[r0 + rt] = __builtin_amdgcn_mfma_f32_32x32x16_f16(wa2[cur][0][rt], bl, yv[r0 + rt], 0, 0, 0);
#pragma unroll
                for (int rt = 0; rt < RH; ++rt) yv[r0 + rt] = __builtin_amdgcn_mfma_f32_32x32x16_f16(wa2[cur][1][rt], bh, yv[r0 + rt], 0, 0, 0);
#pragma unroll
                for (int rt = 0; rt < RH; ++rt) yv[r0 + rt] = __builtin_amdgcn_mfma_f32_32x32x16_f16(wa2[cur][0][rt], bh, yv[r0 + rt], 0, 0, 0);
            }
        }
#pragma unroll
        for (int rt = 0; rt < RT; ++rt)
#pragma unroll
            for (int r = 0; r < 16; ++r) yv[rt][r] *= wout_inv;
    } else if constexpr (P16) {
        using x8 = typename M16::x8;
        const char* wrow = reinterpret_cast<const char*>(wout_pair) + ((size_t)l31 * kHid + 8 * h) * 2;
        const char* brow = reinterpret_cast<const char*>(qo_smem) + (wave * 32 + l31) * RBO + 16 * h;
        constexpr int NK16 = kHid / 16;
        x8 wa1[2][RT];
#pragma unroll
        for (int rt = 0; rt < RT; ++rt) wa1[0][rt] = *reinterpret_cast<const x8*>(wrow + (size_t)rt * 32 * kHid * 2);
#pragma unroll
        for (int ks = 0; ks < NK16; ++ks) {
            const int cur = ks & 1, nxt = cur ^ 1;
            const int kp = (ks + 1 < NK16 ? ks + 1 : ks) * 32;
#pragma unroll
            for (int rt = 0; rt < RT; ++rt) wa1[nxt][rt] = *reinterpret_cast<const x8*>(wrow + (size_t)rt * 32 * kHid * 2 + kp);
            const x8 bb = *reinterpret_cast<const x8*>(brow + 32 * ks);
#pragma unroll
            for (int rt = 0; rt < RT; ++rt) yv[rt] = M16::mfma(wa1[cur][rt], bb, yv[rt]);
        }
        if constexpr (MODE == 3) {
            const float dn = 1.0f / ctx_up;
#pragma unroll
            for (int rt = 0; rt < RT; ++rt)
#pragma unroll
                for (int r = 0; r < 16; ++r) yv[rt][r] *= dn;
        }
    } else
    {
        const float* wrow = wout + (size_t)l31 * kHid + 4 * h;
        const float* brow = Os + (wave * 32 + l31) * LDO + 4 * h;
        constexpr int NK = kHid / 8;
        constexpr int PF = RT > 4 ? 1 : 2, RING = PF + 1;
        floatx4 wa[RING][RT];
#pragma unroll
        for (int pf = 0; pf < PF; ++pf)
#pragma unroll
            for (int rt = 0; rt < RT; ++rt) wa[pf][rt] = *reinterpret_cast<const floatx4*>(wrow + (size_t)rt * 32 * kHid + 8 * pf);
#pragma unroll
        for (int ks = 0; ks < NK; ++ks) {
            if (ks + PF < NK) {
#pragma unroll
                for (int rt = 0; rt < RT; ++rt)
                    wa[(ks + PF) % RING][rt] = *reinterpret_cast<const floatx4*>(wrow + (size_t)rt * 32 * kHid + 8 * (ks + PF));
            }
            __builtin_amdgcn_sched_barrier(0);
            const floatx4 bb = *reinterpret_cast<const floatx4*>(brow + 8 * ks);
#pragma unroll
            for (int rt = 0; rt < RT; ++rt) {
                const floatx4 a = wa[ks % RING][rt];
                yv[rt] = __builtin_amdgcn_mfma_f32_32x32x2f32(a.x, bb.x, yv[rt], 0, 0, 0);
                yv[rt] = __builtin_amdgcn_mfma_f32_32x32x2f32(a.y, bb.y, yv[rt], 0, 0, 0);
                yv[rt] = __builtin_amdgcn_mfma_f32_32x32x2f32(a.z, bb.z, yv[rt], 0, 0, 0);
                yv[rt] = __builtin_amdgcn_mfma_f32_32x32x2f32(a.w, bb.w, yv[rt], 0, 0, 0);
            }
        }
    }
    float sum = 0.f;
#pragma unroll
    for (int rt = 0; rt < RT; ++rt)
#pragma unroll
        for (int r = 0; r < 16; ++r) {
            yv[rt][r] += bias[32 * rt + (r & 3) + 8 * (r >> 2) + 4 * h];
            sum += yv[rt][r];
        }
    sum = half_sum(sum);
    const float mean = sum * (1.0f / (float)C);
    float sq = 0.f;
#pragma unroll
    for (int rt = 0; rt < RT; ++rt)
#pragma unroll
        for (int r = 0; r < 16; ++r) {
            yv[rt][r] -= mean;
            sq += yv[rt][r] * yv[rt][r];
        }
    sq = half_sum(sq);
    const float rstd = __builtin_amdgcn_rsqf(sq * (1.0f / (float)C) + eps);
    if constexpr (C > kHid || P16) __syncthreads();
    float* yrow = Os + (wave * 32 + l31) * LDY + 4 * h;
#pragma unroll
    for (int rt = 0; rt < RT; ++rt)
#pragma unroll
        for (int gq = 0; gq < 4; ++gq) {
            const floatx4 g4 = *reinterpret_cast<const floatx4*>(g2 + 32 * rt + 8 * gq + 4 * h);
            *reinterpret_cast<floatx4*>(yrow + 32 * rt + 8 * gq) =
                floatx4{yv[rt][4 * gq] * rstd * g4.x, yv[rt][4 * gq + 1] * rstd * g4.y, yv[rt][4 * gq + 2] * rstd * g4.z,
                        yv[rt][4 * gq + 3] * rstd * g4.w};
        }
    __builtin_amdgcn_s_waitcnt(0xc07f);
    auto residual_store = [&](auto full_tag) {
        constexpr bool FULL = decltype(full_tag)::value;
        const size_t slab = (img + t0 + wave * 32) * C;
        floatx4 xr[NQ];
        if (FULL && KEEP && keep_res) {
#pragma unroll
            for (int j = 0; j < NQ; ++j) xr[j] = xkeep[KEEP ? j : 0];
        } else {
#pragma unroll
            for (int j = 0; j < NQ; ++j) {
                const int i = lane + 64 * j, row = lane / C4 + (64 / C4) * j, c4 = lane % C4;
                if constexpr (FULL) xr[j] = *reinterpret_cast<const floatx4*>(xres + slab + 4 * i);
                else xr[j] = *reinterpret_cast<const floatx4*>(xres + (img + min(t0 + wave * 32 + row, N - 1)) * C + 4 * c4);
            }
        }
#pragma unroll
        for (int j = 0; j < NQ; ++j) {
            const int i = lane + 64 * j, row = lane / C4 + (64 / C4) * j, c4 = lane % C4;
            const int n = t0 + wave * 32 + row;
            const floatx4 v = *reinterpret_cast<const floatx4*>(Os + (wave * 32 + row) * LDY + 4 * c4);
            if constexpr (FULL) *reinterpret_cast<floatx4*>(y + slab + 4 * i) = v + xr[j];
            else if (n < N) *reinterpret_cast<floatx4*>(y + (img + n) * C + 4 * c4) = v + xr[j];
        }
    };
    auto residual_store_bf = [&](auto full_tag) {
        constexpr bool FULL = decltype(full_tag)::value;
        const char* rb = reinterpret_cast<const char*>(xres);
        char* yb = reinterpret_cast<char*>(y);
        const size_t slab = (img + t0 + wave * 32) * C * 2;
        bf16x8 xr[NQ8];
        if (FULL && KEEP8 && keep_res) {
#pragma unroll
            for (int j = 0; j < NQ8; ++j) xr[j] = xkeep8[KEEP8 ? j : 0];
        } else {
#pragma unroll
            for (int j = 0; j < NQ8; ++j) {
                const int i = lane + 64 * j, row = lane / C8 + (64 / C8) * j, c8 = lane % C8;
                if constexpr (FULL) xr[j] = *reinterpret_cast<const bf16x8*>(rb + slab + 16 * (size_t)i);
                else xr[j] = *reinterpret_cast<const bf16x8*>(rb + ((img + min(t0 + wave * 32 + row, N - 1)) * C + 8 * c8) * 2);
            }
        }
#pragma unroll
        for (int j = 0; j < NQ8; ++j) {
            const int i = lane + 64 * j, row = lane / C8 + (64 / C8) * j, c8 = lane % C8;
            const int n = t0 + wave * 32 + row;
            const float* yr = Os + (wave * 32 + row) * LDY + 8 * c8;
            const floatx4 va = *reinterpret_cast<const floatx4*>(yr), vb = *reinterpret_cast<const floatx4*>(yr + 4);
            const floatx8 v = floatx8{va.x, va.y, va.z, va.w, vb.x, vb.y, vb.z, vb.w} + __builtin_convertvector(xr[j], floatx8);
            const bf16x8 o = __builtin_convertvector(v, bf16x8);
            if constexpr (FULL) *reinterpret_cast<bf16x8*>(yb + slab + 16 * (size_t)i) = o;
            else if (n < N) *reinterpret_cast<bf16x8*>(yb + ((img + n) * C + 8 * c8) * 2) = o;
        }
    };
    if constexpr (ABF) {
        if (full_tile) residual_store_bf(std::true_type{}); else residual_store_bf(std::false_type{});
    } else {
        if (full_tile) residual_store(std::true_type{}); else residual_store(std::false_type{});
    }
}

__global__ __launch_bounds__(256) void full_attn_kernel(const float* __restrict__ qkv, float* __restrict__ out, const int N,
                                                        const float scale) {
    const int lane = threadIdx.x & 63, wave = threadIdx.x >> 6;
    const int l31 = lane & 31, h = lane >> 5;
    const int bh = blockIdx.y, b = bh >> 2, head = bh & 3;
    const int q0 = (blockIdx.x * 4 + wave) * 32;
    if (q0 >= N) return;
    const float* base = qkv + (size_t)b * N * kQkv + head * kDh;
    const int q = q0 + l31;
    float qreg[16];
    {
        const float4* qp = reinterpret_cast<const float4*>(base + (size_t)(q < N ? q : q0) * kQkv + 16 * h);
#pragma unroll
        for (int v = 0; v < 4; ++v) {
            const float4 t4 = qp[v];
            qreg[4 * v + 0] = t4.x * scale; qreg[4 * v + 1] = t4.y * scale;
            qreg[4 * v + 2] = t4.z * scale; qreg[4 * v + 3] = t4.w * scale;
        }
    }
    float m = -INFINITY, l = 0.f;
    floatx16 o;
#pragma unroll
    for (int r = 0; r < 16; ++r) o[r] = 0.f;
    for (int j0 = 0; j0 < N; j0 += 32) {
        const int j = j0 + l31;
        float kreg[16];
        {
            const float4* kp = reinterpret_cast<const float4*>(base + (size_t)(j < N ? j : 0) * kQkv + kHid + 16 * h);
#pragma unroll
            for (int v = 0; v < 4; ++v) {
                const float4 t4 = kp[v];
                kreg[4 * v + 0] = t4.x; kreg[4 * v + 1] = t4.y; kreg[4 * v + 2] = t4.z; kreg[4 * v + 3] = t4.w;
            }
        }
        float vreg[16];
#pragma unroll
        for (int s2 = 0; s2 < 16; ++s2) {
            const int jj = j0 + (s2 & 3) + 8 * (s2 >> 2) + 4 * h;
            vreg[s2] = jj < N ? base[(size_t)jj * kQkv + 2 * kHid + l31] : 0.f;
        }
        floatx16 st;
#pragma unroll
        for (int r = 0; r < 16; ++r) st[r] = 0.f;
// ... 667 lines not shown
    } else {
        if (c == 64) IRSDE_PW(64, float); else if (c == 128) IRSDE_PW(128, float); else IRSDE_PW(256, float);
    }
#undef IRSDE_PW
    IRSDE_HIP_CHECK(hipGetLastError());
}

void launch_dwconv_gate(const float* u, const float* w, const float* bias, float* out, float* partial, int B, int H, int W,
                        int c, hipStream_t s, bool f16) {
    if (c % 4) throw HipError("dwconv_gate: channel count must be a multiple of 4");
    const DwGeom g = dw_geom(H, W, c);
    const int nt = g.tiles_x * g.tiles_y;
    if (f16)
        hipLaunchKernelGGL(dwconv_gate_kernel<f16_t>, dim3(nt, B), dim3(256), 0, s, reinterpret_cast<const f16_t*>(u), w, bias, reinterpret_cast<f16_t*>(out), partial,
                           H, W, c, g.tiles_x, nt, g.run);
    else
        hipLaunchKernelGGL(dwconv_gate_kernel<float>, dim3(nt, B), dim3(256), 0, s, u, w, bias, out, partial, H, W, c, g.tiles_x, nt, g.run);
    IRSDE_HIP_CHECK(hipGetLastError());
}

void launch_sca(const float* partial, int ntiles, const float* W, const float* bias, float* mean, float* s_out, int B,
                int c, int HW, hipStream_t s) {
    if ((long long)ntiles * c <= 65536 && c <= 4096) {
        hipLaunchKernelGGL(sca_fused_kernel, dim3((c + 3) / 4, B), dim3(256), (size_t)c * 4, s, partial, ntiles, W, bias, s_out, c, 1.0f / (float)HW);
    } else {
        launch_sca_mean(partial, ntiles, mean, B, c, HW, s);
        hipLaunchKernelGGL(sca_kernel, dim3((c + 3) / 4, B), dim3(256), 0, s, mean, W, bias, s_out, c);
    }
    IRSDE_HIP_CHECK(hipGetLastError());
}

void launch_sca_mean(const float* partial, int ntiles, float* mean, int B, int c, int HW, hipStream_t s) {
    hipLaunchKernelGGL(sca_mean_kernel, dim3((c + 63) / 64, B), dim3(256), 0, s, partial, ntiles, mean, c, 1.0f / (float)HW);
    IRSDE_HIP_CHECK(hipGetLastError());
}

void launch_row_gate(const float* in, float* out, int rows, int h, hipStream_t s) {
    const int total = rows * h;
    hipLaunchKernelGGL(row_gate_kernel, dim3((total + 255) / 256), dim3(256), 0, s, in, out, rows, h);
    IRSDE_HIP_CHECK(hipGetLastError());
}

static int attn_chunk_len(int N, int B) {
    const int want = std::max(32, (512 + B - 1) / std::max(B, 1));
    int len = (N + want - 1) / want;
    if (len < 128) len = 128;
    return (len + 7) & ~7;
}
int attn_num_chunks(int N, int B) {
    const int len = attn_chunk_len(N, B);
    return (N + len - 1) / len;
}

template <typename T>
static void linear_attention_t(const T* qkv, T* out, int B, int N, const AttnWorkspace& ws, hipStream_t s) {
    const int len = attn_chunk_len(N, B);
    const int nch = attn_num_chunks(N, B);
    if (nch != ws.nch) throw HipError("attention workspace chunk mismatch");
    hipLaunchKernelGGL(attn_ctx_partial_kernel<T>, dim3(nch, B * kHeads), dim3(256), 0, s, qkv, ws.pmax, ws.pctx, ws.psum,
                       N, len, nch);
    hipLaunchKernelGGL(attn_ctx_finalize_kernel, dim3(B * kHeads, 4), dim3(1024), 0, s, ws.pctx, ws.psum, ws.pmax, ws.ctx, nch,
                       1.0f / (float)N, 1.0f / sqrtf((float)kDh));
    const int tiles = (N + 31) / 32;
    hipLaunchKernelGGL(attn_out_kernel<T>, dim3((tiles + kOutTilesPerBlock - 1) / kOutTilesPerBlock, B), dim3(256), 0, s,
                       qkv, ws.ctx, out, N, kQkv);
    IRSDE_HIP_CHECK(hipGetLastError());
}
void attention_global_init() {
#define IRSDE_KV_ATTR(CC) IRSDE_HIP_CHECK(hipFuncSetAttribute(reinterpret_cast<const void*>(attn_kv_ctx_kernel<CC>), hipFuncAttributeMaxDynamicSharedMemorySize, 160 * 1024))
    IRSDE_KV_ATTR(32); IRSDE_KV_ATTR(64); IRSDE_KV_ATTR(96); IRSDE_KV_ATTR(128); IRSDE_KV_ATTR(160); IRSDE_KV_ATTR(192); IRSDE_KV_ATTR(224); IRSDE_KV_ATTR(256);
#undef IRSDE_KV_ATTR
    IRSDE_HIP_CHECK(hipFuncSetAttribute(reinterpret_cast<const void*>(attn_q_out_fused_kernel<64, true>), hipFuncAttributeMaxDynamicSharedMemorySize, 160 * 1024));
    IRSDE_HIP_CHECK(hipFuncSetAttribute(reinterpret_cast<const void*>(attn_q_out_fused_kernel<128, true>), hipFuncAttributeMaxDynamicSharedMemorySize, 160 * 1024));
    IRSDE_HIP_CHECK(hipFuncSetAttribute(reinterpret_cast<const void*>(attn_q_out_fused_kernel<256, true>), hipFuncAttributeMaxDynamicSharedMemorySize, 160 * 1024));
    IRSDE_HIP_CHECK(hipFuncSetAttribute(reinterpret_cast<const void*>(attn_kv_ctx_kernel<64, true>), hipFuncAttributeMaxDynamicSharedMemorySize, 160 * 1024));
    IRSDE_HIP_CHECK(hipFuncSetAttribute(reinterpret_cast<const void*>(attn_kv_ctx_kernel<128, true>), hipFuncAttributeMaxDynamicSharedMemorySize, 160 * 1024));
    IRSDE_HIP_CHECK(hipFuncSetAttribute(reinterpret_cast<const void*>(attn_kv_ctx_kernel<256, true>), hipFuncAttributeMaxDynamicSharedMemorySize, 160 * 1024));
#define IRSDE_A16_ATTR(CC, MM, AA)                                                                                                                  \
    IRSDE_HIP_CHECK(hipFuncSetAttribute(reinterpret_cast<const void*>(attn_kv_ctx_kernel<CC, MM, AA>), hipFuncAttributeMaxDynamicSharedMemorySize, 160 * 1024)); \
    IRSDE_HIP_CHECK(hipFuncSetAttribute(reinterpret_cast<const void*>(attn_q_out_fused_kernel<CC, MM, AA>), hipFuncAttributeMaxDynamicSharedMemorySize, 160 * 1024))
    IRSDE_A16_ATTR(64, 2, false); IRSDE_A16_ATTR(128, 2, false); IRSDE_A16_ATTR(256, 2, false);
    IRSDE_A16_ATTR(64, 2, true); IRSDE_A16_ATTR(128, 2, true); IRSDE_A16_ATTR(256, 2, true);
    IRSDE_A16_ATTR(64, 3, false); IRSDE_A16_ATTR(128, 3, false); IRSDE_A16_ATTR(256, 3, false);
#undef IRSDE_A16_ATTR
    IRSDE_HIP_CHECK(hipFuncSetAttribute(reinterpret_cast<const void*>(attn_q_out_fused_kernel<64>),
                                        hipFuncAttributeMaxDynamicSharedMemorySize, 160 * 1024));
    IRSDE_HIP_CHECK(hipFuncSetAttribute(reinterpret_cast<const void*>(attn_q_out_fused_kernel<128>),
                                        hipFuncAttributeMaxDynamicSharedMemorySize, 160 * 1024));
    IRSDE_HIP_CHECK(hipFuncSetAttribute(reinterpret_cast<const void*>(attn_q_out_fused_kernel<256>),
                                        hipFuncAttributeMaxDynamicSharedMemorySize, 160 * 1024));
}
void launch_attention_kv_context(const float* xn, const float* wkv, int B, int N, int C, const AttnWorkspace& ws, hipStream_t s,
                                 const float* ln_g, float ln_eps, const unsigned short* wkv_pair, float w_inv_scale, int op16, bool act_bf16) {
    if (ln_g && (C & (C - 1))) throw HipError("attention_kv_context: the fused LayerNorm needs a power-of-two channel count");
    if (C % 32 || C > 256 || C < 32) throw HipError("attention_kv_context: C must be a multiple of 32, <= 256");
    const int len = attn_chunk_len(N, B);
    const int nch = attn_num_chunks(N, B);
    if (nch != ws.nch) throw HipError("attention workspace chunk mismatch");
    if (op16) {
        if (!wkv_pair || (op16 != 2 && op16 != 3) || (act_bf16 && op16 != 2) || (C != 64 && C != 128 && C != 256))
            throw HipError("attention_kv_context: the 16-bit operand modes need their weight plane, C = 64 / 128 / 256; bf16 storage goes with bf16 operands");
        const size_t lds1 = (size_t)kKvTile * (2 * C + 16);
#define IRSDE_KV16_LAUNCH(CC, MM, AA) hipLaunchKernelGGL((attn_kv_ctx_kernel<CC, MM, AA>), dim3(nch, B), dim3(256), lds1, s, xn, wkv, ws.pmax, ws.pctx, ws.psum, N, len, nch, ln_g, ln_eps, wkv_pair, 1.f)
#define IRSDE_KV16_C(CC) { if (act_bf16) IRSDE_KV16_LAUNCH(CC, 2, true); else if (op16 == 2) IRSDE_KV16_LAUNCH(CC, 2, false); else IRSDE_KV16_LAUNCH(CC, 3, false); }
        if (C == 64) IRSDE_KV16_C(64) else if (C == 128) IRSDE_KV16_C(128) else IRSDE_KV16_C(256)
#undef IRSDE_KV16_C
#undef IRSDE_KV16_LAUNCH
        hipLaunchKernelGGL(attn_ctx_finalize_kernel, dim3(B * kHeads, 4), dim3(1024), 0, s, ws.pctx, ws.psum, ws.pmax, ws.ctx, nch,
                           1.0f / (float)N, 1.0f / sqrtf((float)kDh));
        IRSDE_HIP_CHECK(hipGetLastError());
        return;
    }
    if (wkv_pair) {
        const size_t ldsp = (size_t)2 * kKvTile * (2 * C + 16);
#define IRSDE_KVP_LAUNCH(CC) hipLaunchKernelGGL((attn_kv_ctx_kernel<CC, true>), dim3(nch, B), dim3(256), ldsp, s, xn, wkv, ws.pmax, ws.pctx, ws.psum, N, len, nch, ln_g, ln_eps, wkv_pair, w_inv_scale)
        switch (C) {
            case 64: IRSDE_KVP_LAUNCH(64); break;
            case 128: IRSDE_KVP_LAUNCH(128); break;
            case 256: IRSDE_KVP_LAUNCH(256); break;
            default: throw HipError("attention_kv_context: the fp16-pair projection exists for C = 64, 128, 256");
        }
#undef IRSDE_KVP_LAUNCH
        hipLaunchKernelGGL(attn_ctx_finalize_kernel, dim3(B * kHeads, 4), dim3(1024), 0, s, ws.pctx, ws.psum, ws.pmax, ws.ctx, nch,
                           1.0f / (float)N, 1.0f / sqrtf((float)kDh));
        IRSDE_HIP_CHECK(hipGetLastError());
        return;
    }
    const size_t lds = (size_t)kKvTile * (C + 4) * sizeof(float);
#define IRSDE_KV_LAUNCH(CC) hipLaunchKernelGGL(attn_kv_ctx_kernel<CC>, dim3(nch, B), dim3(256), lds, s, xn, wkv, ws.pmax, ws.pctx, ws.psum, N, len, nch, ln_g, ln_eps)
    switch (C) {
        case 32: IRSDE_KV_LAUNCH(32); break;
        case 64: IRSDE_KV_LAUNCH(64); break;
        case 96: IRSDE_KV_LAUNCH(96); break;
        case 128: IRSDE_KV_LAUNCH(128); break;
        case 160: IRSDE_KV_LAUNCH(160); break;
        case 192: IRSDE_KV_LAUNCH(192); break;
        case 224: IRSDE_KV_LAUNCH(224); break;
        case 256: IRSDE_KV_LAUNCH(256); break;
        default: throw HipError("attention_kv_context: unsupported channel count");
    }
#undef IRSDE_KV_LAUNCH
    hipLaunchKernelGGL(attn_ctx_finalize_kernel, dim3(B * kHeads, 4), dim3(1024), 0, s, ws.pctx, ws.psum, ws.pmax, ws.ctx, nch,
                       1.0f / (float)N, 1.0f / sqrtf((float)kDh));
    IRSDE_HIP_CHECK(hipGetLastError());
}
void launch_attention_q_out(const float* q, float* out, int B, int N, const AttnWorkspace& ws, hipStream_t s) {
    const int tiles = (N + 31) / 32;
    hipLaunchKernelGGL(attn_out_kernel<float>, dim3((tiles + kOutTilesPerBlock - 1) / kOutTilesPerBlock, B), dim3(256), 0, s, q, ws.ctx,
                       out, N, kHid);
    IRSDE_HIP_CHECK(hipGetLastError());
}

void launch_attention_q_out_fused(const float* xn, const float* x, const float* wq, const float* wout, const float* bias,
                                  const float* g2, float* y, int B, int N, int C, float eps, const AttnWorkspace& ws, hipStream_t s,
                                  const float* ln_g, const unsigned short* wq_pair, const unsigned short* wout_pair, float wq_inv,
                                  float wout_inv, int op16, bool act_bf16) {
    if (C != 64 && C != 128 && C != 256) throw HipError("attention_q_out_fused: C must be 64, 128 or 256");
    if (op16) {
        if (!wq_pair || !wout_pair || (op16 != 2 && op16 != 3) || (act_bf16 && op16 != 2))
            throw HipError("attention_q_out_fused: the 16-bit operand modes need their weight planes; bf16 storage goes with bf16 operands");
        const size_t plane_x = (size_t)128 * (2 * C + 16), plane_o = (size_t)128 * (2 * kHid + 16);
        const size_t ys = (size_t)128 * ((C > kHid ? C : kHid) + 4) * sizeof(float);
        const size_t lds1 = std::max(std::max(plane_x, plane_o), ys);
        const dim3 grid1((N + 127) / 128, B);
#define IRSDE_QO16_LAUNCH(CC, MM, AA) hipLaunchKernelGGL((attn_q_out_fused_kernel<CC, MM, AA>), grid1, dim3(256), lds1, s, xn, x, wq, ws.ctx, wout, bias, g2, y, N, eps, ln_g, wq_pair, wout_pair, 1.f, 1.f)
#define IRSDE_QO16_C(CC) { if (act_bf16) IRSDE_QO16_LAUNCH(CC, 2, true); else if (op16 == 2) IRSDE_QO16_LAUNCH(CC, 2, false); else IRSDE_QO16_LAUNCH(CC, 3, false); }
        if (C == 64) IRSDE_QO16_C(64) else if (C == 128) IRSDE_QO16_C(128) else IRSDE_QO16_C(256)
#undef IRSDE_QO16_C
#undef IRSDE_QO16_LAUNCH
        IRSDE_HIP_CHECK(hipGetLastError());
        return;
    }
    if (wq_pair && wout_pair) {
        const size_t planes_x = (size_t)2 * 128 * (2 * C + 16), planes_o = (size_t)2 * 128 * (2 * kHid + 16);
        const size_t ys = (size_t)128 * ((C > kHid ? C : kHid) + 4) * sizeof(float);
        const size_t ldsp = std::max(std::max(planes_x, planes_o), ys);
        const dim3 gridp((N + 127) / 128, B);
        if (C == 64)
            hipLaunchKernelGGL((attn_q_out_fused_kernel<64, true>), gridp, dim3(256), ldsp, s, xn, x, wq, ws.ctx, wout, bias, g2, y, N, eps, ln_g,
                               wq_pair, wout_pair, wq_inv, wout_inv);
        else if (C == 128)
            hipLaunchKernelGGL((attn_q_out_fused_kernel<128, true>), gridp, dim3(256), ldsp, s, xn, x, wq, ws.ctx, wout, bias, g2, y, N, eps, ln_g,
                               wq_pair, wout_pair, wq_inv, wout_inv);
        else
            hipLaunchKernelGGL((attn_q_out_fused_kernel<256, true>), gridp, dim3(256), ldsp, s, xn, x, wq, ws.ctx, wout, bias, g2, y, N, eps, ln_g,
                               wq_pair, wout_pair, wq_inv, wout_inv);
        IRSDE_HIP_CHECK(hipGetLastError());
        return;
    }
    const size_t lds = (size_t)128 * ((C > kHid ? C : kHid) + 4) * sizeof(float);
    const dim3 grid((N + 127) / 128, B);
    if (C == 64)
        hipLaunchKernelGGL(attn_q_out_fused_kernel<64>, grid, dim3(256), lds, s, xn, x, wq, ws.ctx, wout, bias, g2, y, N, eps, ln_g);
    else if (C == 128)
        hipLaunchKernelGGL(attn_q_out_fused_kernel<128>, grid, dim3(256), lds, s, xn, x, wq, ws.ctx, wout, bias, g2, y, N, eps, ln_g);
    else
        hipLaunchKernelGGL(attn_q_out_fused_kernel<256>, grid, dim3(256), lds, s, xn, x, wq, ws.ctx, wout, bias, g2, y, N, eps, ln_g);
    IRSDE_HIP_CHECK(hipGetLastError());
}

void launch_linear_attention(const float* qkv, float* out, int B, int N, const AttnWorkspace& ws, hipStream_t s, bool bf16) {
    if (bf16)
        linear_attention_t(reinterpret_cast<const bf16_t*>(qkv), reinterpret_cast<bf16_t*>(out), B, N, ws, s);
    else
        linear_attention_t(qkv, out, B, N, ws, s);
}

void launch_full_attention(const float* qkv, float* out, int B, int N, hipStream_t s) {
    const int qtiles = (N + 31) / 32;
    hipLaunchKernelGGL(full_attn_kernel, dim3((qtiles + 3) / 4, B * kHeads), dim3(256), 0, s, qkv, out, N,
                       1.0f / sqrtf((float)kDh));
    IRSDE_HIP_CHECK(hipGetLastError());
}

void launch_prep_input(const float* xt, const float* cond, float* x0, int B, int in_nc, int H, int W, int Hp, int Wp,
                       hipStream_t s, int reflect) {
    const int P = ((cond ? 2 : 1) * in_nc + 3) & ~3;
    if (P > 16) throw HipError("prep_input: more than 8 (conditional) / 16 (unconditional) input channels unsupported");
    const size_t total = (size_t)B * (Hp + 6) * (Wp + 6);
    hipLaunchKernelGGL(prep_input_kernel, dim3((unsigned)((total + 255) / 256)), dim3(256), 0, s, xt, cond, x0, B,
                       in_nc, P, H, W, Hp, Wp, reflect);
    IRSDE_HIP_CHECK(hipGetLastError());
}

void launch_sinusoid(const float* tvals, const float* freqs, float* out, int rows, int half, hipStream_t s) {
    const int total = rows * half;
    hipLaunchKernelGGL(sinusoid_kernel, dim3((total + 255) / 256), dim3(256), 0, s, tvals, freqs, out, rows, half);
    IRSDE_HIP_CHECK(hipGetLastError());
}

void launch_row_linear(const float* in, int in_stride, const float* W, const float* b, float* out, int out_stride,
                       int rows, int in_dim, int out_dim, int act_in, int act_out, hipStream_t s) {
    hipLaunchKernelGGL(row_linear_kernel, dim3((out_dim + 3) / 4), dim3(256), 0, s, in, in_stride, W, b, out,
                       out_stride, rows, in_dim, out_dim, act_in, act_out);
    IRSDE_HIP_CHECK(hipGetLastError());
}

void launch_step_begin(StepState* st, const float* film_table, int film_row, float* film_cur, const float* coef_table,
                       hipStream_t s) {
    hipLaunchKernelGGL(step_begin_kernel, dim3(1), dim3(1024), 0, s, st, film_table, film_row, film_cur, coef_table);
// ... 134 lines not shown
```

### include/irsde_hip_debug.h

```cpp
#ifndef IRSDE_HIP_DEBUG_H
#define IRSDE_HIP_DEBUG_H

#include "irsde_hip.h"

#ifdef __cplusplus
extern "C" {
#endif

int irsde_debug_conv(const float* in0, int C0, const float* in1, int C1, int B, int Hin, int Win, int in_shift,
                     const float* w_oihw, int Cout, int KH, int KW, int stride, int pad, const float* bias,
                     const float* film, int film_bstride, int silu, const float* res, float* out, int naive,
                     int splits, void* stream);

int irsde_debug_conv_choice(int B, int Hin, int Win, int C0, int C1, int Cout, int K, int stride, int pad, int in_shift, int operand, int storage, int pair,
                            unsigned features, int splits, int nz, int tune, int cu_count, const int* knobs, char* out, int out_len);

int irsde_debug_conv_halo_choice(int B, int Hin, int Win, int C0, int C1, int Cout, int K, int stride, int pad, int in_shift, int operand, int storage, int pair,
                                 unsigned features, int splits, int nz, int tune, int halo2, int nslow, char* out, int out_len);

int irsde_debug_conv_features(const float* in0, int C0, const float* in1, int C1, int B, int Hin, int Win, int in_shift, const float* w_oihw, int Cout, int K,
                              int stride, int pad, int operand, int storage, int pair, const float* bias, const float* ch_scale, const float* ln_g,
                              const float* film, int film_bstride, const float* res, const float* in_scale, const float* gate_film, int gate_film_bstride,
                              int silu, int gate, int shuffle, int nz, int splits, int tune, const int* knobs, float* out, char* choice, int choice_len,
                              void* stream);

int irsde_debug_split_gemm(const float* A, const float* B, float* C, int M, int N, int K, int ncomp, int nplanes, void* stream);

int irsde_bench_conv(int variant, int B, int H, int W, int Cin, int Cout, int K, int stride, int up, int epi, int iters,
                     double* ms_out);
int irsde_bench_naf_chain(int variant, int nblocks, int B, int iters, double* ms_out);
int irsde_debug_force_subbatches(int n);
int irsde_debug_force_chain_groups(int g);
int irsde_debug_force_wino_poly(int mode);
int irsde_debug_force_split3(int mode);
int irsde_debug_force_split3_blocks(int n);

int irsde_debug_scam(const float* x, int B_pairs, int H, int W, int C, const float* norm_l_g, const float* norm_r_g, const float* l_proj1_w,
                     const float* l_proj1_b, const float* r_proj1_w, const float* r_proj1_b, const float* l_proj2_w, const float* l_proj2_b,
                     const float* r_proj2_w, const float* r_proj2_b, const float* beta, const float* gamma, float* out, void* stream);

int irsde_debug_naf_gate_sca(const float* u, int B, int H, int W, int c, const float* conv2_w, const float* conv2_b, const float* sca_w, const float* sca_b,
                             float* gated_out, float* mean_out, float* s_out, void* stream);
int irsde_debug_tlsc(const float* g, int B, int h, int w, int c, int k1, int k2, float* pooled_out, const float* scale_map, float* scaled_out, void* stream);
int irsde_debug_ln_film(const float* x, long long M, int C, long long ppi, const float* g, const float* fscale, const float* fshift, int film_bstride,
                        float* out, void* stream);
int irsde_debug_naf_lnconv(int mode, const float* x, long long M, int c, int Cout, long long ppi, const float* g, const float* fscale, const float* fshift,
                           int film_bstride, const float* w, const float* bias, const float* gate_film, int gate_film_bstride, const float* in_scale,
                           const float* ch_scale, const float* res, float* out, void* stream);

int irsde_debug_naf_chain(const float* x, float* out, int B, int nblocks, const float* norm1_g, const float* conv1_w, const float* conv1_b, const float* conv2_w,
                          const float* conv2_b, const float* sca_w, const float* sca_b, const float* conv3_w, const float* conv3_b, const float* beta,
                          const float* norm2_g, const float* conv4_w, const float* conv4_b, const float* conv5_w, const float* conv5_b, const float* gamma,
                          const float* film, int film_bstride, int film_off, const float* cam, int cam_bstride, int cam_off, int groups, void* stream);
int irsde_debug_naf_chain_split_order(int nblocks, int groups, int* order_out, long long n);

int irsde_debug_full_attention16(const void* qkv_bf16, int B, int N, void* out_bf16, void* stream);

int irsde_debug_scam_full(const float* x, int B_pairs, int H, int W, int C, const float* norm_l_g, const float* norm_r_g, const float* l_proj1_w,
                          const float* l_proj1_b, const float* r_proj1_w, const float* r_proj1_b, const float* l_proj2_w, const float* l_proj2_b,
                          const float* r_proj2_w, const float* r_proj2_b, const float* beta, const float* gamma, float* out, void* stream);

int irsde_debug_scam_stream(const float* x, int B_pairs, int H, int W, int C, const float* norm_l_g, const float* norm_r_g, const float* l_proj1_w,
                            const float* l_proj1_b, const float* r_proj1_w, const float* r_proj1_b, const float* l_proj2_w, const float* l_proj2_b,
                            const float* r_proj2_w, const float* r_proj2_b, const float* beta, const float* gamma, int block_w, float* out, void* stream);
int irsde_debug_scam_full_stream(const float* x, int B_pairs, int H, int W, int C, const float* norm_l_g, const float* norm_r_g, const float* l_proj1_w,
                                 const float* l_proj1_b, const float* r_proj1_w, const float* r_proj1_b, const float* l_proj2_w, const float* l_proj2_b,
                                 const float* r_proj2_w, const float* r_proj2_b, const float* beta, const float* gamma, int block_w, float* out,
                                 void* stream);
int irsde_debug_force_scam_stream(int block_w);

#ifdef __cplusplus
}
#endif
#endif
```

Baseline: 4.771 images/s.

## Run linear-attention projections on bf16x3 split MFMA instead of fp32 path

Adds a three-piece bf16 split mode for the fused linear-attention kernels (k/v projection + context, and q projection + output + LayerNorm). Weights are pre-split once into fragment-ordered bf16 planes and activations are split in LDS, so the projections run on bf16 matrix instructions and emulate fp32 accuracy with six products. The mode is on by default for C=64/128/256. It adds more MFMA work per tile, smaller tiles, extra LDS and extra syncs for the cross-wave LayerNorm reduction.

```diff
diff --git a/image_restoration_sde_amd/_lib.py b/image_restoration_sde_amd/_lib.py
--- a/image_restoration_sde_amd/_lib.py
+++ b/image_restoration_sde_amd/_lib.py
@@ -39,7 +39,7 @@
     "irsde_last_error", "irsde_version", "irsde_create", "irsde_create_nafnet", "irsde_destroy", "irsde_num_weights",
     "irsde_weight_name", "irsde_weight_shape", "irsde_load_weight", "irsde_finalize_weights",
     "irsde_set_schedule", "irsde_unet_forward", "irsde_sample", "irsde_sde_step", "irsde_philox_normal",
-    "irsde_get_profile", "irsde_debug_tap", "irsde_work_model", "irsde_debug_conv", "irsde_debug_conv_choice", "irsde_debug_conv_halo_choice", "irsde_debug_conv_features", "irsde_plan_describe", "irsde_bench_conv", "irsde_op_profile", "irsde_debug_split_gemm", "irsde_bench_naf_chain", "irsde_debug_force_subbatches", "irsde_debug_force_chain_groups", "irsde_debug_force_wino_poly", "irsde_debug_force_split3", "irsde_debug_force_split3_blocks", "irsde_debug_scam", "irsde_debug_scam_full",
+    "irsde_get_profile", "irsde_debug_tap", "irsde_work_model", "irsde_debug_conv", "irsde_debug_conv_choice", "irsde_debug_conv_halo_choice", "irsde_debug_conv_features", "irsde_plan_describe", "irsde_bench_conv", "irsde_op_profile", "irsde_debug_split_gemm", "irsde_bench_naf_chain", "irsde_debug_force_subbatches", "irsde_debug_force_chain_groups", "irsde_debug_force_wino_poly", "irsde_debug_force_split3", "irsde_debug_force_split3_attn", "irsde_debug_force_split3_blocks", "irsde_debug_scam", "irsde_debug_scam_full",
     "irsde_debug_scam_stream", "irsde_debug_scam_full_stream", "irsde_debug_force_scam_stream",
     "irsde_debug_naf_gate_sca", "irsde_debug_tlsc", "irsde_debug_ln_film", "irsde_debug_naf_lnconv", "irsde_debug_naf_chain", "irsde_debug_naf_chain_split_order",
     "irsde_debug_full_attention16",
@@ -132,6 +132,7 @@
     lib.irsde_debug_force_chain_groups.argtypes = [c.c_int]
     lib.irsde_debug_force_wino_poly.argtypes = [c.c_int]
     lib.irsde_debug_force_split3.argtypes = [c.c_int]
+    lib.irsde_debug_force_split3_attn.argtypes = [c.c_int]
     lib.irsde_debug_force_split3_blocks.argtypes = [c.c_int]
     lib.irsde_debug_scam.argtypes = [P, c.c_int, c.c_int, c.c_int, c.c_int] + [P] * 12 + [P, P]
     lib.irsde_debug_scam_full.argtypes = [P, c.c_int, c.c_int, c.c_int, c.c_int] + [P] * 12 + [P, P]
diff --git a/image_restoration_sde_amd/csrc/common.h b/image_restoration_sde_amd/csrc/common.h
--- a/image_restoration_sde_amd/csrc/common.h
+++ b/image_restoration_sde_amd/csrc/common.h
@@ -291,6 +291,11 @@
 void launch_attention_kv_context(const float* xn, const float* wkv, int B, int N, int C, const AttnWorkspace& ws, hipStream_t s,
                                  const float* ln_g = nullptr, float ln_eps = 1e-5f, const unsigned short* wkv_pair = nullptr,
                                  float w_inv_scale = 1.f, int op16 = 0, bool act_bf16 = false);
+inline bool attn_split3_has_instance(int C) { return C == 64 || C == 128 || C == 256; }
+__host__ __device__ inline size_t attn_frag3_index(size_t row, int k, int K) {
+    return ((((row >> 5) * (size_t)(K >> 4) + (size_t)(k >> 4)) * 2 + (size_t)((k >> 3) & 1)) * 32 + (row & 31)) * 8 + (size_t)(k & 7);
+}
+void launch_split_frag3(const float* in, unsigned short* out, size_t rows, int K, hipStream_t s);
 void launch_attention_q_out(const float* q, float* out, int B, int N, const AttnWorkspace& ws, hipStream_t s);
 void launch_attention_q_out_fused(const float* xn, const float* x, const float* wq, const float* wout, const float* bias,
                                   const float* g2, float* y, int B, int N, int C, float eps, const AttnWorkspace& ws, hipStream_t s,
diff --git a/image_restoration_sde_amd/csrc/engine.h b/image_restoration_sde_amd/csrc/engine.h
--- a/image_restoration_sde_amd/csrc/engine.h
+++ b/image_restoration_sde_amd/csrc/engine.h
@@ -39,6 +39,8 @@
 constexpr int kSplit3NotExactF32 = IRSDE_FLAG_NO_WINOGRAD | IRSDE_FLAG_NAIVE_CONV | IRSDE_FLAG_BF16 | IRSDE_FLAG_BF16_ACT | IRSDE_FLAG_FP16 | IRSDE_FLAG_F16_ACT |
                                    IRSDE_FLAG_SPLIT_BF16X2 | IRSDE_FLAG_SPLIT_F16X2 | IRSDE_FLAG_NO_SPLIT3;
 inline bool split3_wants_weights(int flags) { return !(flags & kSplit3NotExactF32) && split3_mode() > 0; }
+int split3_attn_mode();
+void set_force_split3_attn(int mode);
 
 inline int wino_min_c(int tile) {
     return tuning_env_int(tile == 4 ? "IRSDE_WINO4_MINC" : "IRSDE_WINO2_MINC", tile == 4 ? 64 : 256);
@@ -431,6 +433,19 @@
     PairCopy pair_copy(const float* w, size_t n) {
         return make_pair_copy(pair_copies, w, n, [&](unsigned short* d, bool f16, float sc) { launch_split_planes(w, d, n, n, 2, stream, f16, sc); });
     }
+    std::map<const float*, unsigned short*> triple_copies;
+    const unsigned short* triple_copy(const float* w, size_t rows, int K) {
+        const size_t n = rows * (size_t)K;
+        auto it = triple_copies.find(w);
+        if (it != triple_copies.end()) return it->second;
+        unsigned short* d = nullptr;
+        IRSDE_HIP_CHECK(hipMalloc(&d, 3 * n * sizeof(unsigned short)));
+        dev_allocs.push_back(reinterpret_cast<float*>(d));
+        launch_split_frag3(w, d, rows, K, stream);
+        IRSDE_HIP_CHECK(hipStreamSynchronize(stream));
+        triple_copies[w] = d;
+        return d;
+    }
     std::map<const float*, PairCopy> pair_copies_il;
     PairCopy pair_copy_il(const float* w, size_t rows, int K) {
         return make_pair_copy(pair_copies_il, w, rows * (size_t)K, [&](unsigned short* d, bool f16, float sc) { launch_split_pairs(w, d, rows, K, stream, f16, sc); });
diff --git a/image_restoration_sde_amd/csrc/engine_debug.hip b/image_restoration_sde_amd/csrc/engine_debug.hip
--- a/image_restoration_sde_amd/csrc/engine_debug.hip
+++ b/image_restoration_sde_amd/csrc/engine_debug.hip
@@ -944,6 +944,10 @@
     return IRSDE_OK;
 }
 
+int irsde_debug_force_split3_attn(int mode) {
+    set_force_split3_attn(mode >= 0 && mode <= 2 ? mode : -1);
+    return IRSDE_OK;
+}
 int irsde_debug_force_split3_blocks(int n) {
     if (n >= 0 && n < 8) return guard([&] { throw HipError("debug_force_split3_blocks: n must be at least 8 (one block per XCD), or negative for the default"); });
     set_force_split3_blocks(n);
diff --git a/image_restoration_sde_amd/csrc/engine_plan.hip b/image_restoration_sde_amd/csrc/engine_plan.hip
--- a/image_restoration_sde_amd/csrc/engine_plan.hip
+++ b/image_restoration_sde_amd/csrc/engine_plan.hip
@@ -202,6 +202,15 @@
         if (!w.wino_u4t || p.C0 + p.C1 > 512 || !wino_shape_ok(p, 4)) return false;
         const long long T = (long long)p.B * (p.Ho / 4) * (p.Wo / 4);
         return T >= split3_fused_min_tiles() && split3_rule(T, p.C0 + p.C1, p.Cout, 36) && split3_adopts(w.wino_u4t, T, p.C0 + p.C1, p.Cout, 36);
+    }
+    static bool split3_attn_rule(int C, int N, int B) {
+        (void)N; (void)B;
+        return attn_split3_has_instance(C);
+    }
+    bool split3_attn_adopts(int C, int N, int B) const {
+        if ((e->cfg.flags & kSplit3NotExactF32) || split3_mode() == 0 || !attn_split3_has_instance(C)) return false;
+        const int mode = split3_attn_mode();
+        return mode >= 2 || (mode == 1 && split3_attn_rule(C, N, B));
     }
     float* alloc_triples(int ncomp, long long rows, int K) { return pl->alloc(((size_t)ncomp * split3_comp_elems((size_t)rows, (size_t)K) + 1) / 2, true); }
 
@@ -748,6 +757,18 @@
             float* yp = y.p;
             const int B = x.B, C = x.C;
             if (!bo) throw HipError("attention: to_out.0.bias missing");
+            if (split3_attn_adopts(C, N, B)) {
+                const unsigned short* wkv3 = e->triple_copy(wkv, 256, C);
+                const unsigned short* wq3 = e->triple_copy(wq, 128, C);
+                const unsigned short* wo3 = e->triple_copy(wo, (size_t)C, 128);
+                push_other(OP_ATTN, [=](hipStream_t s) { launch_attention_kv_context(xp, wkv, B, N, C, ws, s, g1, 1e-5f, wkv3, 1.f, 4); });
+                pl->net_ops.back().desc = "linear_attention LayerNorm + k,v projection (bf16x3) + context (fused) C=" + std::to_string(C);
+                push_other(OP_ATTN, [=](hipStream_t s) {
+                    launch_attention_q_out_fused(xp, xp, wq, wo, bo, g2, yp, B, N, C, 1e-5f, ws, s, g1, wq3, wo3, 1.f, 1.f, 4);
+                });
+                pl->net_ops.back().desc = "linear_attention LayerNorm + q projection (bf16x3) + softmax + context + to_out + LayerNorm + residual (fused) C=" + std::to_string(C);
+                return y;
+            }
             const unsigned short* wkv_pair = nullptr;
             float kv_inv = 1.f;
             if (e->cfg.flags & IRSDE_FLAG_SPLIT_F16X2) {
@@ -966,6 +987,12 @@
     const int f = g_force_split3.load(std::memory_order_relaxed);
     return f >= 0 ? f : tuning_env_int("IRSDE_SPLIT3", 1);
 }
+static std::atomic<int> g_force_split3_attn{-1};
+void set_force_split3_attn(int mode) { g_force_split3_attn.store(mode, std::memory_order_relaxed); }
+int split3_attn_mode() {
+    const int f = g_force_split3_attn.load(std::memory_order_relaxed);
+    return f >= 0 ? f : tuning_env_int("IRSDE_SPLIT3_ATTN", 1);
+}
 static std::atomic<int> g_force_wino_poly{-1};
 void set_force_wino_poly(int mode) { g_force_wino_poly.store(mode, std::memory_order_relaxed); }
 int wino_poly_mode() {
diff --git a/image_restoration_sde_amd/csrc/gemm_split.hip b/image_restoration_sde_amd/csrc/gemm_split.hip
--- a/image_restoration_sde_amd/csrc/gemm_split.hip
+++ b/image_restoration_sde_amd/csrc/gemm_split.hip
@@ -429,6 +429,28 @@
     }
 }
 
+__global__ __launch_bounds__(256) void split_frag3_kernel(const float* __restrict__ in, unsigned short* __restrict__ out, const size_t n, const int K) {
+    const size_t i = (size_t)blockIdx.x * blockDim.x + threadIdx.x;
+    if (i >= n) return;
+    const size_t row = i / K;
+    const int k = (int)(i - row * K);
+    float r = in[i];
+    const size_t o = attn_frag3_index(row, k, K);
+#pragma unroll
+    for (int p = 0; p < 3; ++p) {
+        const __bf16 hb = (__bf16)r;
+        out[p * n + o] = __builtin_bit_cast(unsigned short, hb);
+        r -= (float)hb;
+    }
+}
+
+}
+
+void launch_split_frag3(const float* in, unsigned short* out, size_t rows, int K, hipStream_t s) {
+    if (rows % 32 || K % 16) throw HipError("split_frag3: rows must be a multiple of 32, K of 16");
+    const size_t n = rows * (size_t)K;
+    hipLaunchKernelGGL(split_frag3_kernel, dim3((unsigned)((n + 255) / 256)), dim3(256), 0, s, in, out, n, K);
+    IRSDE_HIP_CHECK(hipGetLastError());
 }
 
 void gemm_split_global_init() {
diff --git a/image_restoration_sde_amd/csrc/kernels_misc.hip b/image_restoration_sde_amd/csrc/kernels_misc.hip
--- a/image_restoration_sde_amd/csrc/kernels_misc.hip
+++ b/image_restoration_sde_amd/csrc/kernels_misc.hip
@@ -311,6 +311,7 @@
 }
 
 constexpr int kKvTile = 128;
+constexpr int kKvTileTri = 64;
 template <int C, int MODE = 0, bool ABF = false>
 __global__ __launch_bounds__(256, 2) void attn_kv_ctx_kernel(const float* __restrict__ xn, const float* __restrict__ wkv,
                                                              float* __restrict__ pmax, float* __restrict__ pctx,
@@ -318,9 +319,10 @@
                                                              const int nch, const float* __restrict__ ln_g, const float ln_eps,
                                                              const unsigned short* __restrict__ wkv_pair = nullptr, const float w_inv_scale = 1.f) {
     extern __shared__ __attribute__((aligned(16))) float kv_smem[];
-    constexpr bool PAIR = MODE == 1, P16 = MODE != 0;
+    constexpr bool PAIR = MODE == 1, TRI = MODE == 4, P16 = MODE != 0;
     using M16 = Mf16<MODE == 1 || MODE == 3>;
     static_assert(!ABF || MODE == 2, "bf16 activation storage goes with the bf16 operand mode");
+    constexpr int TP = TRI ? kKvTileTri : kKvTile, NRT = TP / 32;
     constexpr int RB = 2 * C + 16;
     const int ch = blockIdx.x, b = blockIdx.y;
     const int tid = threadIdx.x, lane = tid & 63, head = tid >> 6;
@@ -335,11 +337,11 @@
 #pragma unroll
     for (int r = 0; r < 16; ++r) ctx[r] = 0.f;
     float ssum = 0.f, mrun = -INFINITY;
-    for (int t0 = n0; t0 < n1; t0 += kKvTile) {
+    for (int t0 = n0; t0 < n1; t0 += TP) {
         auto stage_tile = [&](auto full_tag) {
             constexpr bool FULL = decltype(full_tag)::value;
             const float* tile = xn + ((size_t)b * N + t0) * C;
-            constexpr int NP = kKvTile * c4n / 256;
+            constexpr int NP = TP * c4n / 256;
             constexpr int NB = NP % 8 == 0 ? 8 : 4;
 #pragma unroll
             for (int j0 = 0; j0 < NP; j0 += NB) {
@@ -364,7 +366,16 @@
                         const f16x4 lo = __builtin_convertvector(st[j] - __builtin_convertvector(hi, floatx4), f16x4);
                         char* dst = reinterpret_cast<char*>(kv_smem) + row * RB + 8 * c4;
                         *reinterpret_cast<f16x4*>(dst) = hi;
-                        *reinterpret_cast<f16x4*>(dst + kKvTile * RB) = lo;
+                        *reinterpret_cast<f16x4*>(dst + TP * RB) = lo;
+                    } else if constexpr (TRI) {
+                        const bf16x4 p0 = __builtin_convertvector(st[j], bf16x4);
+                        const floatx4 r1 = st[j] - __builtin_convertvector(p0, floatx4);
+                        const bf16x4 p1 = __builtin_convertvector(r1, bf16x4);
+                        const bf16x4 p2 = __builtin_convertvector(r1 - __builtin_convertvector(p1, floatx4), bf16x4);
+                        char* dst = reinterpret_cast<char*>(kv_smem) + row * RB + 8 * c4;
+                        *reinterpret_cast<bf16x4*>(dst) = p0;
+                        *reinterpret_cast<bf16x4*>(dst + TP * RB) = p1;
+                        *reinterpret_cast<bf16x4*>(dst + 2 * TP * RB) = p2;
                     } else if constexpr (P16) {
                         *reinterpret_cast<typename M16::x4*>(reinterpret_cast<char*>(kv_smem) + row * RB + 8 * c4) = __builtin_convertvector(st[j], typename M16::x4);
                     } else {
@@ -378,7 +389,7 @@
             constexpr int c8n = C >> 3;
             const char* xb = reinterpret_cast<const char*>(xn);
             const char* tile = xb + ((size_t)b * N + t0) * C * 2;
-            constexpr int NP = kKvTile * c8n / 256;
+            constexpr int NP = TP * c8n / 256;
             constexpr int NB = NP % 8 == 0 ? 8 : 4;
             static_assert(256 % c8n == 0 && NP % NB == 0, "piece / thread mapping");
 #pragma unroll
@@ -398,15 +409,27 @@
                 }
             }
         };
+        [[maybe_unused]] bf16x8 wk3[2][3], wv3[2][3];
+        [[maybe_unused]] const char* wkp3 = TRI ? reinterpret_cast<const char*>(wkv_pair) + ((size_t)head * (C / 16) * 64 + 32 * h + l31) * 16 : nullptr;
+        [[maybe_unused]] const char* wvp3 = TRI ? reinterpret_cast<const char*>(wkv_pair) + ((size_t)(kHeads + head) * (C / 16) * 64 + 32 * h + l31) * 16 : nullptr;
+        constexpr size_t WPL3 = (size_t)2 * kHid * C * 2;
+        if constexpr (TRI) {
+#pragma unroll
+            for (int p = 0; p < 3; ++p) {
+                wk3[0][p] = *reinterpret_cast<const bf16x8*>(wkp3 + p * WPL3);
+                wv3[0][p] = *reinterpret_cast<const bf16x8*>(wvp3 + p * WPL3);
+            }
+            __builtin_amdgcn_sched_barrier(0);
+        }
         if constexpr (ABF) {
-            if (t0 + kKvTile <= n1) stage_tile_bf(std::true_type{}); else stage_tile_bf(std::false_type{});
+            if (t0 + TP <= n1) stage_tile_bf(std::true_type{}); else stage_tile_bf(std::false_type{});
         } else {
-            if (t0 + kKvTile <= n1) stage_tile(std::true_type{}); else stage_tile(std::false_type{});
+            if (t0 + TP <= n1) stage_tile(std::true_type{}); else stage_tile(std::false_type{});
         }
         __syncthreads();
-        floatx16 ak[4], av[4];
-#pragma unroll
-        for (int rt = 0; rt < 4; ++rt)
+        floatx16 ak[NRT], av[NRT];
+#pragma unroll
+        for (int rt = 0; rt < NRT; ++rt)
 #pragma unroll
             for (int r = 0; r < 16; ++r) { ak[rt][r] = 0.f; av[rt][r] = 0.f; }
         if constexpr (PAIR) {
@@ -428,9 +451,9 @@
                 wv2[nxt][0] = *reinterpret_cast<const f16x8*>(wvp + kp);
                 wv2[nxt][1] = *reinterpret_cast<const f16x8*>(wvp + WPL + kp);
 #pragma unroll
-                for (int rt = 0; rt < 4; ++rt) {
+                for (int rt = 0; rt < NRT; ++rt) {
                     const f16x8 ah = *reinterpret_cast<const f16x8*>(arow + rt * 32 * RB + 32 * ks);
-                    const f16x8 al = *reinterpret_cast<const f16x8*>(arow + kKvTile * RB + rt * 32 * RB + 32 * ks);
+                    const f16x8 al = *reinterpret_cast<const f16x8*>(arow + TP * RB + rt * 32 * RB + 32 * ks);
                     ak[rt] = __builtin_amdgcn_mfma_f32_32x32x16_f16(ah, wk2[cur][1], ak[rt], 0, 0, 0);
                     av[rt] = __builtin_amdgcn_mfma_f32_32x32x16_f16(ah, wv2[cur][1], av[rt], 0, 0, 0);
                     ak[rt] = __builtin_amdgcn_mfma_f32_32x32x16_f16(al, wk2[cur][0], ak[rt], 0, 0, 0);
@@ -447,9 +470,46 @@
                 for (int ks = 0; ks < NK16; ++ks) kstep(ks);
             }
 #pragma unroll
-            for (int rt = 0; rt < 4; ++rt)
+            for (int rt = 0; rt < NRT; ++rt)
 #pragma unroll
                 for (int r = 0; r < 16; ++r) { ak[rt][r] *= w_inv_scale; av[rt][r] *= w_inv_scale; }
+        } else if constexpr (TRI) {
+            const char* arow = reinterpret_cast<const char*>(kv_smem) + l31 * RB + 16 * h;
+            constexpr int NK16 = C / 16;
+            auto kstep = [&](const int ks) {
+                const int cur = ks & 1, nxt = cur ^ 1;
+                const int kp = (ks + 1 < NK16 ? ks + 1 : ks) * 1024;
+#pragma unroll
+                for (int p = 0; p < 3; ++p) {
+                    wk3[nxt][p] = *reinterpret_cast<const bf16x8*>(wkp3 + p * WPL3 + kp);
+                    wv3[nxt][p] = *reinterpret_cast<const bf16x8*>(wvp3 + p * WPL3 + kp);
+                }
+#pragma unroll
+                for (int rt = 0; rt < NRT; ++rt) {
+                    const bf16x8 a0 = *reinterpret_cast<const bf16x8*>(arow + rt * 32 * RB + 32 * ks);
+                    const bf16x8 a1 = *reinterpret_cast<const bf16x8*>(arow + TP * RB + rt * 32 * RB + 32 * ks);
+                    const bf16x8 a2 = *reinterpret_cast<const bf16x8*>(arow + 2 * TP * RB + rt * 32 * RB + 32 * ks);
+                    ak[rt] = M16::mfma(a0, wk3[cur][2], ak[rt]);
+                    av[rt] = M16::mfma(a0, wv3[cur][2], av[rt]);
+                    ak[rt] = M16::mfma(a1, wk3[cur][1], ak[rt]);
+                    av[rt] = M16::mfma(a1, wv3[cur][1], av[rt]);
+                    ak[rt] = M16::mfma(a2, wk3[cur][0], ak[rt]);
+                    av[rt] = M16::mfma(a2, wv3[cur][0], av[rt]);
+                    ak[rt] = M16::mfma(a0, wk3[cur][1], ak[rt]);
+                    av[rt] = M16::mfma(a0, wv3[cur][1], av[rt]);
+                    ak[rt] = M16::mfma(a1, wk3[cur][0], ak[rt]);
+                    av[rt] = M16::mfma(a1, wv3[cur][0], av[rt]);
+                    ak[rt] = M16::mfma(a0, wk3[cur][0], ak[rt]);
+                    av[rt] = M16::mfma(a0, wv3[cur][0], av[rt]);
+                }
+            };
+            if constexpr (C > 64) {
+#pragma unroll 2
+                for (int ks = 0; ks < NK16; ++ks) kstep(ks);
+            } else {
+#pragma unroll
+                for (int ks = 0; ks < NK16; ++ks) kstep(ks);
+            }
         } else if constexpr (P16) {
             using x8 = typename M16::x8;
             const char* arow = reinterpret_cast<const char*>(kv_smem) + l31 * RB + 16 * h;
@@ -466,7 +526,7 @@
                 wk1[nxt] = *reinterpret_cast<const x8*>(wkp + kp);
                 wv1[nxt] = *reinterpret_cast<const x8*>(wvp + kp);
 #pragma unroll
-                for (int rt = 0; rt < 4; ++rt) {
+                for (int rt = 0; rt < NRT; ++rt) {
                     const x8 a = *reinterpret_cast<const x8*>(arow + rt * 32 * RB + 32 * ks);
                     ak[rt] = M16::mfma(a, wk1[cur], ak[rt]);
                     av[rt] = M16::mfma(a, wv1[cur], av[rt]);
@@ -493,7 +553,7 @@
                 __builtin_amdgcn_sched_barrier(0);
                 const floatx4 bk = wkr[u], bv = wvr[u];
 #pragma unroll
-                for (int rt = 0; rt < 4; ++rt) {
+                for (int rt = 0; rt < NRT; ++rt) {
                     const floatx4 a = *reinterpret_cast<const floatx4*>(arow + rt * 32 * LDA + k8);
                     ak[rt] = __builtin_amdgcn_mfma_f32_32x32x2f32(a.x, bk.x, ak[rt], 0, 0, 0);
                     av[rt] = __builtin_amdgcn_mfma_f32_32x32x2f32(a.x, bv.x, av[rt], 0, 0, 0);
@@ -507,9 +567,9 @@
             }
         }
         float mit = -INFINITY;
-        if (t0 + kKvTile > n1) {
-#pragma unroll
-            for (int rt = 0; rt < 4; ++rt)
+        if (t0 + TP > n1) {
+#pragma unroll
+            for (int rt = 0; rt < NRT; ++rt)
 #pragma unroll
                 for (int r = 0; r < 16; ++r) {
                     const int n = t0 + 32 * rt + (r & 3) + 8 * (r >> 2) + 4 * h;
@@ -517,7 +577,7 @@
                 }
         }
 #pragma unroll
-        for (int rt = 0; rt < 4; ++rt)
+        for (int rt = 0; rt < NRT; ++rt)
 #pragma unroll
             for (int r = 0; r < 16; ++r) mit = fmaxf(mit, ak[rt][r]);
         mit = half_max(mit);
@@ -532,7 +592,7 @@
         {
             const float ml = mrun * 1.44269504088896341f;
 #pragma unroll
-            for (int rt = 0; rt < 4; ++rt)
+            for (int rt = 0; rt < NRT; ++rt)
 #pragma unroll
                 for (int r = 0; r < 16; ++r) {
                     ak[rt][r] = __builtin_amdgcn_exp2f(__builtin_fmaf(ak[rt][r], 1.44269504088896341f, -ml));
@@ -540,10 +600,10 @@
                 }
         }
         __builtin_amdgcn_sched_barrier(0);
-        if constexpr (MODE >= 2) {
+        if constexpr (MODE == 2 || MODE == 3) {
             using x8 = typename M16::x8;
 #pragma unroll
-            for (int rt = 0; rt < 4; ++rt)
+            for (int rt = 0; rt < NRT; ++rt)
 #pragma unroll
                 for (int sh = 0; sh < 2; ++sh) {
                     const floatx8 ka = {ak[rt][8 * sh], ak[rt][8 * sh + 1], ak[rt][8 * sh + 2], ak[rt][8 * sh + 3],
@@ -554,7 +614,7 @@
                 }
         } else {
 #pragma unroll
-            for (int rt = 0; rt < 4; ++rt)
+            for (int rt = 0; rt < NRT; ++rt)
 #pragma unroll
                 for (int r = 0; r < 16; ++r) ctx = __builtin_amdgcn_mfma_f32_32x32x2f32(ak[rt][r], av[rt][r], ctx, 0, 0, 0);
         }
@@ -666,6 +726,11 @@
     }
 }
 
+constexpr int kQoTileTri = 64;
+constexpr size_t qo_tri_main_bytes(const int C) {
+    const size_t px = (size_t)3 * kQoTileTri * (2 * C + 16), po = (size_t)3 * kQoTileTri * (2 * kHid + 16), ys = (size_t)kQoTileTri * ((C > kHid ? C : kHid) + 4) * 4;
+    return px > po ? (px > ys ? px : ys) : (po > ys ? po : ys);
+}
 template <int C, int MODE = 0, bool ABF = false>
 __global__ __launch_bounds__(256, 2) void attn_q_out_fused_kernel(const float* __restrict__ xn, const float* __restrict__ xres,
                                                                const float* __restrict__ wq, const float* __restrict__ ctx,
@@ -675,8 +740,9 @@
                                                                const unsigned short* __restrict__ wq_pair = nullptr,
                                                                const unsigned short* __restrict__ wout_pair = nullptr, const float wq_inv = 1.f,
                                                                const float wout_inv = 1.f) {
-    constexpr int TP = 128, LDA = C + 4, LDO = kHid + 4, RT = C / 32;
-    constexpr bool PAIR = MODE == 1, P16 = MODE != 0;
+    constexpr bool PAIR = MODE == 1, TRI = MODE == 4, P16 = MODE != 0;
+    constexpr int TP = TRI ? kQoTileTri : 128, LDA = C + 4, LDO = kHid + 4, RT = C / 32;
+    constexpr int NCT = TP / 32, SL = TP / 4;
     using M16 = Mf16<MODE == 1 || MODE == 3>;
     static_assert(!ABF || MODE == 2, "bf16 activation storage goes with the bf16 operand mode");
     constexpr int RBX = 2 * C + 16, RBO = 2 * kHid + 16;
@@ -691,7 +757,7 @@
 
     constexpr int C4 = C / 4;
     const bool full_tile = t0 + TP <= N;
-    constexpr int NQ = 32 * C4 / 64;
+    constexpr int NQ = SL * C4 / 64;
     constexpr bool KEEP = !PAIR && !ABF && C <= 128;
     floatx4 xkeep[KEEP ? NQ : 1];
     constexpr int C8 = C / 8, NQ8 = 32 * C8 / 64;
@@ -700,20 +766,21 @@
     bf16x8 xkeep8[KEEP8 ? NQ8 : 1];
     auto stage_tile = [&](auto full_tag) {
         constexpr bool FULL = decltype(full_tag)::value;
-        const float* slab_in = xn + (img + t0 + wave * 32) * C;
-#pragma unroll
-        for (int j0 = 0; j0 < NQ; j0 += 8) {
-            floatx4 st[8];
-#pragma unroll
-            for (int j = 0; j < 8; ++j) {
-                const int i = lane + 64 * (j0 + j), row = wave * 32 + lane / C4 + (64 / C4) * (j0 + j), c4 = lane % C4;
+        const float* slab_in = xn + (img + t0 + wave * SL) * C;
+        constexpr int NB = NQ < 8 ? NQ : 8;
+#pragma unroll
+        for (int j0 = 0; j0 < NQ; j0 += NB) {
+            floatx4 st[NB];
+#pragma unroll
+            for (int j = 0; j < NB; ++j) {
+                const int i = lane + 64 * (j0 + j), row = wave * SL + lane / C4 + (64 / C4) * (j0 + j), c4 = lane % C4;
                 if constexpr (FULL) st[j] = *reinterpret_cast<const floatx4*>(slab_in + 4 * i);
                 else st[j] = *reinterpret_cast<const floatx4*>(xn + (img + min(t0 + row, N - 1)) * C + 4 * c4);
                 if constexpr (FULL && KEEP) xkeep[j0 + j] = st[j];
             }
 #pragma unroll
-            for (int j = 0; j < 8; ++j) {
-                const int row = wave * 32 + lane / C4 + (64 / C4) * (j0 + j), c4 = lane % C4;
+            for (int j = 0; j < NB; ++j) {
+                const int row = wave * SL + lane / C4 + (64 / C4) * (j0 + j), c4 = lane % C4;
                 if (ln_g) st[j] = ln_piece<C4>(st[j], *reinterpret_cast<const floatx4*>(ln_g + 4 * c4), eps);
                 if constexpr (PAIR) {
                     const f16x4 hi = __builtin_convertvector(st[j], f16x4);
@@ -721,6 +788,15 @@
                     char* dst = reinterpret_cast<char*>(qo_smem) + row * RBX + 8 * c4;
                     *reinterpret_cast<f16x4*>(dst) = hi;
                     *reinterpret_cast<f16x4*>(dst + TP * RBX) = lo;
+                } else if constexpr (TRI) {
+                    const bf16x4 p0 = __builtin_convertvector(st[j], bf16x4);
+                    const floatx4 r1 = st[j] - __builtin_convertvector(p0, floatx4);
+                    const bf16x4 p1 = __builtin_convertvector(r1, bf16x4);
+                    const bf16x4 p2 = __builtin_convertvector(r1 - __builtin_convertvector(p1, floatx4), bf16x4);
+                    char* dst = reinterpret_cast<char*>(qo_smem) + row * RBX + 8 * c4;
+                    *reinterpret_cast<bf16x4*>(dst) = p0;
+                    *reinterpret_cast<bf16x4*>(dst + TP * RBX) = p1;
+                    *reinterpret_cast<bf16x4*>(dst + 2 * TP * RBX) = p2;
                 } else if constexpr (P16) {
                     *reinterpret_cast<typename M16::x4*>(reinterpret_cast<char*>(qo_smem) + row * RBX + 8 * c4) = __builtin_convertvector(st[j], typename M16::x4);
                 } else {
@@ -752,6 +828,17 @@
             }
         }
     };
+    constexpr int NKB = C / 16, DB = TRI ? (NKB - 1 < 3 ? NKB - 1 : 3) : 0;
+    [[maybe_unused]] bf16x8 wq3[DB + 1][3];
+    [[maybe_unused]] const char* wq3row = TRI ? reinterpret_cast<const char*>(wq_pair) + ((size_t)wave * (C / 16) * 64 + 32 * h + l31) * 16 : nullptr;
+    constexpr size_t WQPL = (size_t)kHid * C * 2;
+    if constexpr (TRI) {
+#pragma unroll
+        for (int pf = 0; pf < DB; ++pf)
+#pragma unroll
+            for (int p = 0; p < 3; ++p) wq3[pf][p] = *reinterpret_cast<const bf16x8*>(wq3row + p * WQPL + 1024 * pf);
+        __builtin_amdgcn_sched_barrier(0);
+    }
     if constexpr (ABF) {
         if (full_tile) stage_tile_bf(std::true_type{}); else stage_tile_bf(std::false_type{});
     } else {
@@ -771,9 +858,9 @@
     }
     __syncthreads();
 
-    floatx16 q[4];
-#pragma unroll
-    for (int ct = 0; ct < 4; ++ct)
+    floatx16 q[NCT];
+#pragma unroll
+    for (int ct = 0; ct < NCT; ++ct)
 #pragma unroll
         for (int r = 0; r < 16; ++r) q[ct][r] = 0.f;
     if constexpr (PAIR) {
@@ -791,7 +878,7 @@
             wa2[nxt][0] = *reinterpret_cast<const f16x8*>(wrow + kp);
             wa2[nxt][1] = *reinterpret_cast<const f16x8*>(wrow + WPL + kp);
 #pragma unroll
-            for (int ct = 0; ct < 4; ++ct) {
+            for (int ct = 0; ct < NCT; ++ct) {
                 const f16x8 bh = *reinterpret_cast<const f16x8*>(brow + ct * 32 * RBX + 32 * ks);
                 const f16x8 bl = *reinterpret_cast<const f16x8*>(brow + TP * RBX + ct * 32 * RBX + 32 * ks);
                 q[ct] = __builtin_amdgcn_mfma_f32_32x32x16_f16(wa2[cur][0], bl, q[ct], 0, 0, 0);
@@ -800,9 +887,32 @@
             }
         }
 #pragma unroll
-        for (int ct = 0; ct < 4; ++ct)
+        for (int ct = 0; ct < NCT; ++ct)
 #pragma unroll
             for (int r = 0; r < 16; ++r) q[ct][r] *= wq_inv;
+    } else if constexpr (TRI) {
+        const char* brow = reinterpret_cast<const char*>(qo_smem) + l31 * RBX + 16 * h;
+#pragma unroll
+        for (int ks = 0; ks < NKB; ++ks) {
+            if (ks + DB < NKB) {
+#pragma unroll
+                for (int p = 0; p < 3; ++p) wq3[(ks + DB) % (DB + 1)][p] = *reinterpret_cast<const bf16x8*>(wq3row + p * WQPL + 1024 * (ks + DB));
+            }
+            __builtin_amdgcn_sched_barrier(0);
+            const bf16x8* wa3c = wq3[ks % (DB + 1)];
+#pragma unroll
+            for (int ct = 0; ct < NCT; ++ct) {
+                const bf16x8 b0 = *reinterpret_cast<const bf16x8*>(brow + ct * 32 * RBX + 32 * ks);
+                const bf16x8 b1 = *reinterpret_cast<const bf16x8*>(brow + TP * RBX + ct * 32 * RBX + 32 * ks);
+                const bf16x8 b2 = *reinterpret_cast<const bf16x8*>(brow + 2 * TP * RBX + ct * 32 * RBX + 32 * ks);
+                q[ct] = M16::mfma(wa3c[2], b0, q[ct]);
+                q[ct] = M16::mfma(wa3c[1], b1, q[ct]);
+                q[ct] = M16::mfma(wa3c[0], b2, q[ct]);
+                q[ct] = M16::mfma(wa3c[1], b0, q[ct]);
+                q[ct] = M16::mfma(wa3c[0], b1, q[ct]);
+                q[ct] = M16::mfma(wa3c[0], b0, q[ct]);
+            }
+        }
     } else if constexpr (P16) {
         using x8 = typename M16::x8;
         const char* wrow = reinterpret_cast<const char*>(wq_pair) + ((size_t)(wave * kDh + l31) * C + 8 * h) * 2;
@@ -815,7 +925,7 @@
             const int cur = ks & 1, nxt = cur ^ 1;
             wa1[nxt] = *reinterpret_cast<const x8*>(wrow + (ks + 1 < NK16 ? ks + 1 : ks) * 32);
 #pragma unroll
-            for (int ct = 0; ct < 4; ++ct)
+            for (int ct = 0; ct < NCT; ++ct)
                 q[ct] = M16::mfma(wa1[cur], *reinterpret_cast<const x8*>(brow + ct * 32 * RBX + 32 * ks), q[ct]);
         }
     } else
@@ -832,7 +942,7 @@
             __builtin_amdgcn_sched_barrier(0);
             const floatx4 a = wa[ks % 3];
 #pragma unroll
-            for (int ct = 0; ct < 4; ++ct) {
+            for (int ct = 0; ct < NCT; ++ct) {
                 const floatx4 bb = *reinterpret_cast<const floatx4*>(brow + ct * 32 * LDA + 8 * ks);
                 q[ct] = __builtin_amdgcn_mfma_f32_32x32x2f32(a.x, bb.x, q[ct], 0, 0, 0);
                 q[ct] = __builtin_amdgcn_mfma_f32_32x32x2f32(a.y, bb.y, q[ct], 0, 0, 0);
@@ -841,9 +951,25 @@
             }
         }
     }
+    constexpr int RTW = TRI ? RT / 2 : RT;
+    constexpr int NKF = kHid / 16, DF = !TRI ? 0 : RTW == 1 ? NKF - 1 : RTW == 2 ? 3 : 1;
+    const int rt0 = TRI ? (wave >> 1) * RTW : 0;
+    const int prow = TRI ? (wave & 1) * 32 : wave * 32;
+    [[maybe_unused]] bf16x8 wo3[DF + 1][3][TRI ? RTW : 1];
+    [[maybe_unused]] const char* wo3row = TRI ? reinterpret_cast<const char*>(wout_pair) + ((size_t)rt0 * (kHid / 16) * 64 + 32 * h + l31) * 16 : nullptr;
+    constexpr size_t WOPL = (size_t)C * kHid * 2;
+    if constexpr (TRI) {
+#pragma unroll
+        for (int pf = 0; pf < DF; ++pf)
+#pragma unroll
+            for (int p = 0; p < 3; ++p)
+#pragma unroll
+                for (int rt = 0; rt < RTW; ++rt) wo3[pf][p][rt] = *reinterpret_cast<const bf16x8*>(wo3row + p * WOPL + (size_t)rt * 32 * kHid * 2 + 1024 * pf);
+        __builtin_amdgcn_sched_barrier(0);
+    }
     __syncthreads();
 #pragma unroll
-    for (int ct = 0; ct < 4; ++ct) {
+    for (int ct = 0; ct < NCT; ++ct) {
         float m = q[ct][0];
 #pragma unroll
         for (int r = 1; r < 16; ++r) m = fmaxf(m, q[ct][r]);
@@ -860,7 +986,7 @@
         floatx16 o;
 #pragma unroll
         for (int r = 0; r < 16; ++r) o[r] = 0.f;
-        if constexpr (MODE >= 2) {
+        if constexpr (MODE == 2 || MODE == 3) {
             using x8 = typename M16::x8;
 #pragma unroll
             for (int sh = 0; sh < 2; ++sh) {
@@ -883,6 +1009,19 @@
                 *reinterpret_cast<f16x4*>(orow + 16 * gq) = hi;
                 *reinterpret_cast<f16x4*>(orow + TP * RBO + 16 * gq) = lo;
             }
+        } else if constexpr (TRI) {
+            char* orow = reinterpret_cast<char*>(qo_smem) + (ct * 32 + l31) * RBO + (wave * kDh + 4 * h) * 2;
+#pragma unroll
+            for (int gq = 0; gq < 4; ++gq) {
+                const floatx4 v = floatx4{o[4 * gq], o[4 * gq + 1], o[4 * gq + 2], o[4 * gq + 3]};
+                const bf16x4 p0 = __builtin_convertvector(v, bf16x4);
+                const floatx4 r1 = v - __builtin_convertvector(p0, floatx4);
+                const bf16x4 p1 = __builtin_convertvector(r1, bf16x4);
+                const bf16x4 p2 = __builtin_convertvector(r1 - __builtin_convertvector(p1, floatx4), bf16x4);
+                *reinterpret_cast<bf16x4*>(orow + 16 * gq) = p0;
+                *reinterpret_cast<bf16x4*>(orow + TP * RBO + 16 * gq) = p1;
+                *reinterpret_cast<bf16x4*>(orow + 2 * TP * RBO + 16 * gq) = p2;
+            }
         } else if constexpr (P16) {
             char* orow = reinterpret_cast<char*>(qo_smem) + (ct * 32 + l31) * RBO + (wave * kDh + 4 * h) * 2;
 #pragma unroll
@@ -898,12 +1037,41 @@
     }
     __syncthreads();
 
-    floatx16 yv[RT];
-#pragma unroll
-    for (int rt = 0; rt < RT; ++rt)
+    floatx16 yv[RTW];
+#pragma unroll
+    for (int rt = 0; rt < RTW; ++rt)
 #pragma unroll
         for (int r = 0; r < 16; ++r) yv[rt][r] = 0.f;
-    if constexpr (PAIR) {
+    if constexpr (TRI) {
+        const char* brow = reinterpret_cast<const char*>(qo_smem) + (prow + l31) * RBO + 16 * h;
+#pragma unroll
+        for (int ks = 0; ks < NKF; ++ks) {
+            if (ks + DF < NKF) {
+#pragma unroll
+                for (int p = 0; p < 3; ++p)
+#pragma unroll
+                    for (int rt = 0; rt < RTW; ++rt)
+                        wo3[(ks + DF) % (DF + 1)][p][rt] = *reinterpret_cast<const bf16x8*>(wo3row + p * WOPL + (size_t)rt * 32 * kHid * 2 + 1024 * (ks + DF));
+            }
+            __builtin_amdgcn_sched_barrier(0);
+            const auto& wa3c = wo3[ks % (DF + 1)];
+            const bf16x8 b0 = *reinterpret_cast<const bf16x8*>(brow + 32 * ks);
+            const bf16x8 b1 = *reinterpret_cast<const bf16x8*>(brow + TP * RBO + 32 * ks);
+            const bf16x8 b2 = *reinterpret_cast<const bf16x8*>(brow + 2 * TP * RBO + 32 * ks);
+#pragma unroll
+            for (int rt = 0; rt < RTW; ++rt) yv[rt] = M16::mfma(wa3c[2][rt], b0, yv[rt]);
+#pragma unroll
+            for (int rt = 0; rt < RTW; ++rt) yv[rt] = M16::mfma(wa3c[1][rt], b1, yv[rt]);
+#pragma unroll
+            for (int rt = 0; rt < RTW; ++rt) yv[rt] = M16::mfma(wa3c[0][rt], b2, yv[rt]);
+#pragma unroll
+            for (int rt = 0; rt < RTW; ++rt) yv[rt] = M16::mfma(wa3c[1][rt], b0, yv[rt]);
+#pragma unroll
+            for (int rt = 0; rt < RTW; ++rt) yv[rt] = M16::mfma(wa3c[0][rt], b1, yv[rt]);
+#pragma unroll
+            for (int rt = 0; rt < RTW; ++rt) yv[rt] = M16::mfma(wa3c[0][rt], b0, yv[rt]);
+        }
+    } else if constexpr (PAIR) {
         const char* wrow = reinterpret_cast<const char*>(wout_pair) + ((size_t)l31 * kHid + 8 * h) * 2;
         constexpr size_t WPL = (size_t)C * kHid * 2;
         const char* brow = reinterpret_cast<const char*>(qo_smem) + (wave * 32 + l31) * RBO + 16 * h;
@@ -997,39 +1165,51 @@
     }
     float sum = 0.f;
 #pragma unroll
-    for (int rt = 0; rt < RT; ++rt)
+    for (int rt = 0; rt < RTW; ++rt)
 #pragma unroll
         for (int r = 0; r < 16; ++r) {
-            yv[rt][r] += bias[32 * rt + (r & 3) + 8 * (r >> 2) + 4 * h];
+            yv[rt][r] += bias[32 * (rt0 + rt) + (r & 3) + 8 * (r >> 2) + 4 * h];
             sum += yv[rt][r];
         }
     sum = half_sum(sum);
+    [[maybe_unused]] float* red = reinterpret_cast<float*>(reinterpret_cast<char*>(qo_smem) + qo_tri_main_bytes(C));
+    if constexpr (TRI) {
+        if (h == 0) red[(wave >> 1) * TP + prow + l31] = sum;
+        __syncthreads();
+        sum = red[prow + l31] + red[TP + prow + l31];
+    }
     const float mean = sum * (1.0f / (float)C);
     float sq = 0.f;
 #pragma unroll
-    for (int rt = 0; rt < RT; ++rt)
+    for (int rt = 0; rt < RTW; ++rt)
 #pragma unroll
         for (int r = 0; r < 16; ++r) {
             yv[rt][r] -= mean;
             sq += yv[rt][r] * yv[rt][r];
         }
     sq = half_sum(sq);
+    if constexpr (TRI) {
+        if (h == 0) red[2 * TP + (wave >> 1) * TP + prow + l31] = sq;
+        __syncthreads();
+        sq = red[2 * TP + prow + l31] + red[3 * TP + prow + l31];
+    }
     const float rstd = __builtin_amdgcn_rsqf(sq * (1.0f / (float)C) + eps);
-    if constexpr (C > kHid || P16) __syncthreads();
-    float* yrow = Os + (wave * 32 + l31) * LDY + 4 * h;
-#pragma unroll
-    for (int rt = 0; rt < RT; ++rt)
+    if constexpr (!TRI && (C > kHid || P16)) __syncthreads();
+    float* yrow = Os + (prow + l31) * LDY + 32 * rt0 + 4 * h;
+#pragma unroll
+    for (int rt = 0; rt < RTW; ++rt)
 #pragma unroll
         for (int gq = 0; gq < 4; ++gq) {
-            const floatx4 g4 = *reinterpret_cast<const floatx4*>(g2 + 32 * rt + 8 * gq + 4 * h);
+            const floatx4 g4 = *reinterpret_cast<const floatx4*>(g2 + 32 * (rt0 + rt) + 8 * gq + 4 * h);
             *reinterpret_cast<floatx4*>(yrow + 32 * rt + 8 * gq) =
                 floatx4{yv[rt][4 * gq] * rstd * g4.x, yv[rt][4 * gq + 1] * rstd * g4.y, yv[rt][4 * gq + 2] * rstd * g4.z,
                         yv[rt][4 * gq + 3] * rstd * g4.w};
         }
-    __builtin_amdgcn_s_waitcnt(0xc07f);
+    if constexpr (TRI) __syncthreads();
+    else __builtin_amdgcn_s_waitcnt(0xc07f);
     auto residual_store = [&](auto full_tag) {
         constexpr bool FULL = decltype(full_tag)::value;
-        const size_t slab = (img + t0 + wave * 32) * C;
+        const size_t slab = (img + t0 + wave * SL) * C;
         floatx4 xr[NQ];
         if (FULL && KEEP && keep_res) {
 #pragma unroll
@@ -1039,14 +1219,14 @@
             for (int j = 0; j < NQ; ++j) {
                 const int i = lane + 64 * j, row = lane / C4 + (64 / C4) * j, c4 = lane % C4;
                 if constexpr (FULL) xr[j] = *reinterpret_cast<const floatx4*>(xres + slab + 4 * i);
-                else xr[j] = *reinterpret_cast<const floatx4*>(xres + (img + min(t0 + wave * 32 + row, N - 1)) * C + 4 * c4);
+                else xr[j] = *reinterpret_cast<const floatx4*>(xres + (img + min(t0 + wave * SL + row, N - 1)) * C + 4 * c4);
             }
         }
 #pragma unroll
         for (int j = 0; j < NQ; ++j) {
             const int i = lane + 64 * j, row = lane / C4 + (64 / C4) * j, c4 = lane % C4;
-            const int n = t0 + wave * 32 + row;
-            const floatx4 v = *reinterpret_cast<const floatx4*>(Os + (wave * 32 + row) * LDY + 4 * c4);
+            const int n = t0 + wave * SL + row;
+            const floatx4 v = *reinterpret_cast<const floatx4*>(Os + (wave * SL + row) * LDY + 4 * c4);
             if constexpr (FULL) *reinterpret_cast<floatx4*>(y + slab + 4 * i) = v + xr[j];
             else if (n < N) *reinterpret_cast<floatx4*>(y + (img + n) * C + 4 * c4) = v + xr[j];
         }
@@ -1880,6 +2060,7 @@
     IRSDE_A16_ATTR(64, 2, false); IRSDE_A16_ATTR(128, 2, false); IRSDE_A16_ATTR(256, 2, false);
     IRSDE_A16_ATTR(64, 2, true); IRSDE_A16_ATTR(128, 2, true); IRSDE_A16_ATTR(256, 2, true);
     IRSDE_A16_ATTR(64, 3, false); IRSDE_A16_ATTR(128, 3, false); IRSDE_A16_ATTR(256, 3, false);
+    IRSDE_A16_ATTR(64, 4, false); IRSDE_A16_ATTR(128, 4, false); IRSDE_A16_ATTR(256, 4, false);
 #undef IRSDE_A16_ATTR
     IRSDE_HIP_CHECK(hipFuncSetAttribute(reinterpret_cast<const void*>(attn_q_out_fused_kernel<64>),
                                         hipFuncAttributeMaxDynamicSharedMemorySize, 160 * 1024));
@@ -1895,6 +2076,17 @@
     const int len = attn_chunk_len(N, B);
     const int nch = attn_num_chunks(N, B);
     if (nch != ws.nch) throw HipError("attention workspace chunk mismatch");
+    if (op16 == 4) {
+        if (!wkv_pair || act_bf16 || !attn_split3_has_instance(C)) throw HipError("attention_kv_context: the three-piece mode needs its weight planes, fp32 tensors, C = 64 / 128 / 256");
+        const size_t lds3 = (size_t)3 * kKvTileTri * (2 * C + 16);
+#define IRSDE_KV3_LAUNCH(CC) hipLaunchKernelGGL((attn_kv_ctx_kernel<CC, 4>), dim3(nch, B), dim3(256), lds3, s, xn, wkv, ws.pmax, ws.pctx, ws.psum, N, len, nch, ln_g, ln_eps, wkv_pair, 1.f)
+        if (C == 64) IRSDE_KV3_LAUNCH(64); else if (C == 128) IRSDE_KV3_LAUNCH(128); else IRSDE_KV3_LAUNCH(256);
+#undef IRSDE_KV3_LAUNCH
+        hipLaunchKernelGGL(attn_ctx_finalize_kernel, dim3(B * kHeads, 4), dim3(1024), 0, s, ws.pctx, ws.psum, ws.pmax, ws.ctx, nch,
+                           1.0f / (float)N, 1.0f / sqrtf((float)kDh));
+        IRSDE_HIP_CHECK(hipGetLastError());
+        return;
+    }
     if (op16) {
         if (!wkv_pair || (op16 != 2 && op16 != 3) || (act_bf16 && op16 != 2) || (C != 64 && C != 128 && C != 256))
             throw HipError("attention_kv_context: the 16-bit operand modes need their weight plane, C = 64 / 128 / 256; bf16 storage goes with bf16 operands");
@@ -1954,6 +2146,16 @@
                                   const float* ln_g, const unsigned short* wq_pair, const unsigned short* wout_pair, float wq_inv,
                                   float wout_inv, int op16, bool act_bf16) {
     if (C != 64 && C != 128 && C != 256) throw HipError("attention_q_out_fused: C must be 64, 128 or 256");
+    if (op16 == 4) {
+        if (!wq_pair || !wout_pair || act_bf16) throw HipError("attention_q_out_fused: the three-piece mode needs its weight planes and fp32 tensors");
+        const size_t lds3 = qo_tri_main_bytes(C) + (size_t)4 * kQoTileTri * sizeof(float);
+        const dim3 grid3((N + kQoTileTri - 1) / kQoTileTri, B);
+#define IRSDE_QO3_LAUNCH(CC) hipLaunchKernelGGL((attn_q_out_fused_kernel<CC, 4>), grid3, dim3(256), lds3, s, xn, x, wq, ws.ctx, wout, bias, g2, y, N, eps, ln_g, wq_pair, wout_pair, 1.f, 1.f)
+        if (C == 64) IRSDE_QO3_LAUNCH(64); else if (C == 128) IRSDE_QO3_LAUNCH(128); else IRSDE_QO3_LAUNCH(256);
+#undef IRSDE_QO3_LAUNCH
+        IRSDE_HIP_CHECK(hipGetLastError());
+        return;
+    }
     if (op16) {
         if (!wq_pair || !wout_pair || (op16 != 2 && op16 != 3) || (act_bf16 && op16 != 2))
             throw HipError("attention_q_out_fused: the 16-bit operand modes need their weight planes; bf16 storage goes with bf16 operands");
diff --git a/include/irsde_hip_debug.h b/include/irsde_hip_debug.h
--- a/include/irsde_hip_debug.h
+++ b/include/irsde_hip_debug.h
@@ -33,6 +33,7 @@
 int irsde_debug_force_chain_groups(int g);
 int irsde_debug_force_wino_poly(int mode);
 int irsde_debug_force_split3(int mode);
+int irsde_debug_force_split3_attn(int mode);
 int irsde_debug_force_split3_blocks(int n);
 
 int irsde_debug_scam(const float* x, int B_pairs, int H, int W, int C, const float* norm_l_g, const float* norm_r_g, const float* l_proj1_w,
```

New measurement: 4.893 images/s (median of 6 runs). 1.03x the previous value.
